# wpeebles/gangealing

Hardware: NVIDIA H100
Metric: gangealing_train_images_per_sec_256 (higher is better)
Workload: dtype f32

## Files before the change

### gangealing_b200/_lib.py

```python
import ctypes
import os

import torch

_HERE = os.path.dirname(os.path.abspath(__file__))
LIB_PATH = os.path.join(_HERE, "libgg_b200.so")

GG_F32, GG_F16, GG_BF16 = 0, 1, 2
PAD_MODES = {"zeros": 0, "border": 1, "reflection": 2}

_c = ctypes
_P, _I, _L, _F = _c.c_void_p, _c.c_int, _c.c_int64, _c.c_float

SIGNATURES = {
    "gg_version": (_I, []),
    "gg_last_error": (_c.c_char_p, []),
    "gg_sm_count": (_I, []),
    "gg_fused_bias_act": (_I, [_P, _P, _P, _P, _I, _I, _I, _F, _F, _L, _L, _L, _P]),
    "gg_noise_bias_act": (_I, [_P, _P, _P, _P, _P, _P, _I, _F, _F, _L, _L, _L, _P]),
    "gg_channel_scale_workspace": (_L, [_L, _L]),
    "gg_channel_scale": (_I, [_P, _P, _P, _P, _P, _P, _I, _L, _L, _P]),
    "gg_bias_act_backward_workspace": (_L, [_L, _L, _L]),
    "gg_bias_act_backward": (_I, [_P, _P, _P, _P, _P, _I, _F, _F, _L, _L, _L, _P]),
    "gg_upfirdn2d": (_I, [_P, _P, _P, _I, _L] + [_I] * 12 + [_P]),
    "gg_blur_noise_bias_act": (_I, [_P] * 7 + [_I, _L, _L] + [_I] * 9 + [_F, _F, _P]),
    "gg_mipmap_pyramid_elems": (_L, [_L, _I, _I, _I]),
    "gg_mipmap_build": (_I, [_P, _P, _I, _L, _I, _I, _I, _P]),
    "gg_mipmap_build_backward": (_I, [_P, _P, _L, _I, _I, _I, _P]),
    "gg_mipmap_warp_forward": (_I, [_P] * 5 + [_I, _L] + [_I] * 6 + [_F, _F, _I, _P]),
    "gg_warp_sample_indices": (_I, [_P, _P, _L, _I, _I, _I, _I, _F, _F, _I, _P]),
    "gg_stn_sample_forward": (_I, [_P] * 11 + [_I, _I, _L] + [_I] * 9 + [_F, _F, _I, _P]),
    "gg_mipmap_warp_lerp_forward": (_I, [_P] * 5 + [_L, _P, _P, _I, _I, _L] + [_I] * 6 + [_F, _F, _I, _P]),
    "gg_mipmap_warp_lerp_mean": (_I, [_P] * 4 + [_L, _P, _P, _I, _I, _L] + [_I] * 6 + [_F, _F, _I, _I, _P]),
    "gg_track_points_lerp": (_I, [_P] * 6 + [_I, _L, _L, _I, _I, _I, _P]),
    "gg_modconv_wsq": (_I, [_P, _P, _I, _I, _I, _P]),
    "gg_modconv_demod": (_I, [_P, _P, _P, _F, _F, _I, _I, _I, _P]),
    "gg_modconv_demod_batched": (_I, [_I, _P, _P, _P, _P, _P, _P, _F, _I, _P]),
    "gg_modconv_modulate": (_I, [_P, _P, _P, _P, _F, _I, _I, _I, _I, _I, _P]),
    "gg_noise_bias_act_nhwc": (_I, [_P] * 6 + [_I, _F, _F, _L, _I, _L, _P]),
    "gg_nhwc_rowwise_workspace": (_L, [_L, _I, _L]),
    "gg_channel_scale_nhwc": (_I, [_P] * 6 + [_I, _L, _I, _L, _P]),
    "gg_bias_act_backward_nhwc": (_I, [_P] * 5 + [_I, _F, _F, _L, _I, _L, _P]),
    "gg_blur_nhwc_workspace": (_L, [_I, _L] + [_I] * 9),
    "gg_blur_nhwc": (_I, [_P] * 12 + [_I, _L] + [_I] * 12 + [_F, _F, _P]),
    "gg_styled_tail_nhwc": (_I, [_P] * 12 + [_I, _I, _F, _F, _L, _I, _L, _P]),
    "gg_styled_tail_backward_workspace": (_L, [_I, _L, _I, _L]),
    "gg_styled_tail_backward_nhwc": (_I, [_P] * 12 + [_I, _F, _F, _L, _I, _L, _L, _P]),
    "gg_tent_downsample_forward": (_I, [_P] * 4 + [_L, _I, _I, _I, _I, _P]),
    "gg_tent_downsample_backward": (_I, [_P] * 4 + [_L, _I, _I, _I, _I, _P]),
    "gg_feature_distance_workspace": (_L, [_L, _I, _L]),
    "gg_feature_distance_forward": (_I, [_P] * 5 + [_I, _L, _I, _L, _F, _P]),
    "gg_feature_distance_backward": (_I, [_P] * 6 + [_I, _L, _I, _L, _F, _P]),
    "gg_bias_relu_pool_nhwc_forward": (_I, [_P, _P, _P, _P, _I, _L, _I, _I, _I, _P]),
    "gg_bias_relu_pool_nhwc_backward": (_I, [_P, _P, _P, _P, _I, _L, _I, _I, _I, _P]),
    "gg_to_rgb_nhwc_workspace": (_L, [_L, _I, _L]),
    "gg_to_rgb_nhwc_forward": (_I, [_P] * 5 + [_L, _I, _L, _P]),
    "gg_to_rgb_nhwc_backward": (_I, [_P] * 6 + [_L, _I, _L, _P]),
    "gg_nn_argmin_workspace": (_L, [_L, _L]),
    "gg_nn_argmin": (_I, [_P, _P, _P, _P, _L, _L, _I, _P]),
    "gg_splat2d_lookup_forward": (_I, [_P] * 8 + [_L, _L, _I, _I, _I, _I, _I, _F, _F, _I, _P]),
    "gg_scale_cast_multi": (_I, [_P, _P, _P, _I, _I, _P]),
    "gg_adam_ema_step": (_I, [_P, _P, _P, _I, _I, _P, _c.c_double, _c.c_double, _c.c_double, _c.c_double, _P]),
    "gg_tv_loss_workspace": (_L, [_L, _I, _I]),
    "gg_tv_loss_forward": (_I, [_P, _P, _P, _L, _I, _I, _P]),
    "gg_tv_loss_backward": (_I, [_P, _P, _P, _L, _I, _I, _P]),
    "gg_splat2d_workspace": (_L, [_L, _I, _I, _I]),
    "gg_splat2d_forward": (_I, [_P] * 6 + [_L, _L, _I, _I, _I, _I, _P]),
    "gg_flow_compose_forward": (_I, [_P] * 7 + [_L, _I, _I, _I, _P]),
    "gg_flow_compose_backward": (_I, [_P] * 10 + [_L, _I, _I, _I, _P]),
    "gg_mipmap_warp_backward": (_I, [_P] * 7 + [_I, _L] + [_I] * 6 + [_F, _F, _I, _P]),
    "gg_laplacian_blend_workspace": (_L, [_L, _I, _I, _I, _I, _I]),
    "gg_laplacian_blend_forward": (_I, [_P] * 6 + [_L, _I, _I, _I, _I, _I, _P]),
    "gg_laplacian_blend_backward": (_I, [_P] * 9 + [_L, _I, _I, _I, _I, _I, _P]),
    "gg_tv_per_sample": (_I, [_P, _P, _L, _I, _I, _P]),
    "gg_pck_transfer_workspace": (_L, [_L, _L, _I]),
    "gg_pck_transfer": (_I, [_P] * 14 + [_L, _L, _I, _I, _I, _I, _I, _P]),
    "gg_batch_gram": (_I, [_P, _P, _P, _P, _L, _I, _P]),
}

_dll = None
CALLS = 0


def load():
    global _dll
    if _dll is None:
        if not os.path.exists(LIB_PATH):
            raise RuntimeError(
                "libgg_b200.so is missing (%s): build it with `python -m gangealing_b200.build` "
                "(there is no CPU/PyTorch fallback for these ops)" % LIB_PATH)
        dll = ctypes.CDLL(LIB_PATH)
        for name, (res, args) in SIGNATURES.items():
            fn = getattr(dll, name)
            fn.restype = res
            fn.argtypes = args
        _dll = dll
    return _dll


def check(rc, what):
    global CALLS
    CALLS += 1
    if rc != 0:
        msg = load().gg_last_error().decode("utf-8", "replace")
        raise RuntimeError("%s failed (%d): %s" % (what, rc, msg))


def dtype_code(t):
    d = t.dtype
    if d == torch.float32:
        return GG_F32
    if d == torch.float16:
        return GG_F16
    if d == torch.bfloat16:
        return GG_BF16
    raise RuntimeError("gangealing_b200: dtype %s is not supported (float32/float16/bfloat16)" % d)


def require_cuda(*tensors):
    for t in tensors:
        if t is None:
            continue
        if not t.is_cuda:
            raise RuntimeError("gangealing_b200 ops run on CUDA tensors only (got a %s tensor); "
                               "the CPU restatement lives in oracle/ and is test infrastructure" % t.device.type)
        if t.device.index != torch.cuda.current_device():
            raise RuntimeError("gangealing_b200: tensor lives on %s but the current device is cuda:%d; wrap the call in "
                               "`with torch.cuda.device(tensor.device):`" % (t.device, torch.cuda.current_device()))


def ptr(t):
    return None if t is None else t.data_ptr()


def is_nhwc(t):
    return (t.dim() == 4 and t.dtype in (torch.float32, torch.bfloat16) and t.shape[1] > 1 and t.shape[2] * t.shape[3] > 1
            and t.is_contiguous(memory_format=torch.channels_last) and not t.is_contiguous())


def nhwc_vec(t):
    return 8 if t.dtype == torch.bfloat16 else 4


def aligned16(t):
    return t.data_ptr() % 16 == 0


def dense_f32(t):
    if t.dtype != torch.float32 or not t.is_contiguous():
        t = t.float().contiguous()
    return t if aligned16(t) else t.clone()


def tensor_cache(t):
    stamp = (t._version, t.data_ptr(), t.device, t.dtype)
    ent = getattr(t, "_gg_cache", None)
    if ent is None or ent[0] != stamp:
        ent = (stamp, {})
        try:
            t._gg_cache = ent
        except Exception:
            pass
    return ent[1]


def filter_is_separable(kernel):
    memo = tensor_cache(kernel)
    v = memo.get("separable")
    if v is None:
        k = kernel.detach().float().cpu()
        big = k.abs().max()
        if big == 0:
            v = True
        else:
            i0, j0 = divmod(int(k.abs().argmax()), k.shape[1])
            v = bool((k - torch.outer(k[:, j0], k[i0, :]) / k[i0, j0]).abs().max() <= 1e-6 * big)
        memo["separable"] = v
    return v


def flipped_filter(kernel):
    memo = tensor_cache(kernel)
    f = memo.get("flipped")
    if f is None:
        f = torch.flip(kernel.detach(), [0, 1])
        fm = tensor_cache(f)
        fm["flipped"] = kernel.detach()
        if "separable" in memo:
            fm["separable"] = memo["separable"]
        memo["flipped"] = f
    return f


def invalidate(t):
    try:
        t._gg_cache = None
    except Exception:
        pass


def stream():
    return torch.cuda.current_stream().cuda_stream


def sm_count():
    return load().gg_sm_count()


def ship_table(slot, payload):
    capturing = torch.cuda.is_current_stream_capturing()
    ev = slot.get("event")
    if ev is not None and not capturing:
        ev.synchronize()
    slot["host"].copy_(payload)
    slot["dev"].copy_(slot["host"], non_blocking=True)
    if capturing:
        slot["event"] = None
    else:
        ev = torch.cuda.Event()
        ev.record()
        slot["event"] = ev
```

### gangealing_b200/csrc/common.cuh

```cuda
#pragma once
#include <cuda_bf16.h>
#include <cuda_fp16.h>
#include <cuda_runtime.h>
#include <stdint.h>

#include <cstdarg>
#include <cstdio>

#include "../../include/gg_b200.h"

namespace gg {

inline char* err_buf() {
  static thread_local char buf[512] = {0};
  return buf;
}
inline int fail(int code, const char* fmt, ...) {
  va_list ap;
  va_start(ap, fmt);
  vsnprintf(err_buf(), 512, fmt, ap);
  va_end(ap);
  return code;
}
inline int cuda_fail(cudaError_t e, const char* what) {
  return fail(GG_ERR_CUDA, "%s: %s", what, cudaGetErrorString(e));
}
#define GG_CHECK_LAUNCH(what)                               \
  do {                                                      \
    cudaError_t e__ = cudaPeekAtLastError();                \
    if (e__ != cudaSuccess) {                               \
      (void)cudaGetLastError();                             \
      return ::gg::cuda_fail(e__, what);                    \
    }                                                       \
  } while (0)

#define GG_DISPATCH_CASE_(code_, type_, ...) \
  case code_: { using T_ = type_; __VA_ARGS__; break; }
#define GG_DISPATCH_T(dtype_, who_, ...)                                                                             \
  switch (dtype_) {                                                                                                  \
    GG_DISPATCH_CASE_(GG_F32, float, __VA_ARGS__)                                                                    \
    GG_DISPATCH_CASE_(GG_BF16, __nv_bfloat16, __VA_ARGS__)                                                           \
    default: return ::gg::fail(GG_ERR_UNSUPPORTED, "%s: dtype %d not supported (fp32 or bf16)", who_, dtype_);       \
  }
#define GG_DISPATCH_T16(dtype_, who_, ...)                                                                           \
  switch (dtype_) {                                                                                                  \
    GG_DISPATCH_CASE_(GG_F32, float, __VA_ARGS__)                                                                    \
    GG_DISPATCH_CASE_(GG_F16, __half, __VA_ARGS__)                                                                   \
    GG_DISPATCH_CASE_(GG_BF16, __nv_bfloat16, __VA_ARGS__)                                                           \
    default: return ::gg::fail(GG_ERR_UNSUPPORTED, "%s: dtype %d not supported (fp32, fp16 or bf16)", who_, dtype_); \
  }

int sm_count();

inline bool aligned16(const void* p) { return (reinterpret_cast<uintptr_t>(p) & 15u) == 0; }

struct DeviceOnce {
  unsigned long long mask[2] = {0ull, 0ull};
  int dev = 0;
  bool needed() {
    if (cudaGetDevice(&dev) != cudaSuccess || dev < 0 || dev >= 128) return true;
    return ((__atomic_load_n(&mask[dev >> 6], __ATOMIC_ACQUIRE) >> (dev & 63)) & 1ull) == 0ull;
  }
  void done() {
    if (dev >= 0 && dev < 128) __atomic_fetch_or(&mask[dev >> 6], 1ull << (dev & 63), __ATOMIC_RELEASE);
  }
};

template <typename T> struct Cvt;
template <> struct Cvt<float> {
  static __device__ __forceinline__ float to_f(float v) { return v; }
  static __device__ __forceinline__ float from_f(float v) { return v; }
};
template <> struct Cvt<__half> {
  static __device__ __forceinline__ float to_f(__half v) { return __half2float(v); }
  static __device__ __forceinline__ __half from_f(float v) { return __float2half_rn(v); }
};
template <> struct Cvt<__nv_bfloat16> {
  static __device__ __forceinline__ float to_f(__nv_bfloat16 v) { return __bfloat162float(v); }
  static __device__ __forceinline__ __nv_bfloat16 from_f(float v) { return __float2bfloat16_rn(v); }
};

template <typename T> struct alignas(16) Vec16 {
  static constexpr int N = 16 / sizeof(T);
  T v[N];
};

template <typename T>
__device__ __forceinline__ Vec16<T> ld_vec_stream(const T* p) {
  Vec16<T> r;
  uint4 u;
  asm volatile("ld.global.nc.L1::no_allocate.v4.u32 {%0,%1,%2,%3}, [%4];"
               : "=r"(u.x), "=r"(u.y), "=r"(u.z), "=r"(u.w)
               : "l"(p));
  *reinterpret_cast<uint4*>(&r) = u;
  return r;
}
template <typename T>
__device__ __forceinline__ void st_vec_stream(T* p, const Vec16<T>& r) {
  const uint4 u = *reinterpret_cast<const uint4*>(&r);
  asm volatile("st.global.L1::no_allocate.v4.u32 [%0], {%1,%2,%3,%4};" ::"l"(p), "r"(u.x), "r"(u.y),
               "r"(u.z), "r"(u.w)
               : "memory");
}

template <typename T> struct ChanVec;
template <> struct ChanVec<float> {
  static constexpr int V = 4;
  static __device__ __forceinline__ void unpack(const uint4& u, float (&f)[4]) {
    f[0] = __uint_as_float(u.x); f[1] = __uint_as_float(u.y); f[2] = __uint_as_float(u.z); f[3] = __uint_as_float(u.w);
  }
  static __device__ __forceinline__ uint4 pack(const float (&f)[4]) {
    return make_uint4(__float_as_uint(f[0]), __float_as_uint(f[1]), __float_as_uint(f[2]), __float_as_uint(f[3]));
  }
};
template <> struct ChanVec<__nv_bfloat16> {
  static constexpr int V = 8;
  static __device__ __forceinline__ void unpack(const uint4& u, float (&f)[8]) {
    f[0] = __uint_as_float(u.x << 16); f[1] = __uint_as_float(u.x & 0xffff0000u);
    f[2] = __uint_as_float(u.y << 16); f[3] = __uint_as_float(u.y & 0xffff0000u);
    f[4] = __uint_as_float(u.z << 16); f[5] = __uint_as_float(u.z & 0xffff0000u);
    f[6] = __uint_as_float(u.w << 16); f[7] = __uint_as_float(u.w & 0xffff0000u);
  }
  static __device__ __forceinline__ uint32_t pack2(float lo, float hi) {
    const __nv_bfloat162 h = __floats2bfloat162_rn(lo, hi);
    return *reinterpret_cast<const uint32_t*>(&h);
  }
  static __device__ __forceinline__ uint4 pack(const float (&f)[8]) {
    return make_uint4(pack2(f[0], f[1]), pack2(f[2], f[3]), pack2(f[4], f[5]), pack2(f[6], f[7]));
  }
};
__device__ __forceinline__ uint4 ldg_stream16(const void* p) {
  uint4 u;
  asm volatile("ld.global.nc.L1::no_allocate.v4.u32 {%0,%1,%2,%3}, [%4];" : "=r"(u.x), "=r"(u.y), "=r"(u.z), "=r"(u.w) : "l"(p));
  return u;
}
__device__ __forceinline__ void stg_stream16(void* p, const uint4& u) {
  asm volatile("st.global.L1::no_allocate.v4.u32 [%0], {%1,%2,%3,%4};" ::"l"(p), "r"(u.x), "r"(u.y), "r"(u.z), "r"(u.w) : "memory");
}

__device__ __forceinline__ float warp_sum(float v) {
#pragma unroll
  for (int o = 16; o > 0; o >>= 1) v += __shfl_xor_sync(0xffffffffu, v, o);
  return v;
}

__device__ __forceinline__ uint32_t smem_u32(const void* p) {
  return static_cast<uint32_t>(__cvta_generic_to_shared(p));
}
__device__ __forceinline__ void mbar_init(uint64_t* bar, uint32_t count) {
  asm volatile("mbarrier.init.shared::cta.b64 [%0], %1;" ::"r"(smem_u32(bar)), "r"(count));
}
__device__ __forceinline__ void mbar_fence_init() {
  asm volatile("fence.mbarrier_init.release.cluster;" ::: "memory");
}
__device__ __forceinline__ void mbar_expect_tx(uint64_t* bar, uint32_t bytes) {
  asm volatile("mbarrier.arrive.expect_tx.shared::cta.b64 _, [%0], %1;" ::"r"(smem_u32(bar)),
               "r"(bytes)
               : "memory");
}
__device__ __forceinline__ void mbar_wait(uint64_t* bar, uint32_t parity) {
  uint32_t done;
  uint32_t spins = 0;
  do {
    if (++spins == (1u << 28)) __trap();
    asm volatile(
        "{\n\t"
        ".reg .pred p;\n\t"
        "mbarrier.try_wait.parity.shared::cta.b64 p, [%1], %2;\n\t"
        "selp.u32 %0, 1, 0, p;\n\t"
        "}"
        : "=r"(done)
        : "r"(smem_u32(bar)), "r"(parity)
        : "memory");
  } while (!done);
}
__device__ __forceinline__ void tma_bulk_g2s(void* dst_smem, const void* src_gmem, uint32_t bytes,
                                             uint64_t* bar) {
  asm volatile(
      "cp.async.bulk.shared::cluster.global.mbarrier::complete_tx::bytes [%0], [%1], %2, [%3];" ::"r"(
          smem_u32(dst_smem)),
      "l"(src_gmem), "r"(bytes), "r"(smem_u32(bar))
      : "memory");
}

}
```

### gangealing_b200/csrc/nhwc.cu

```cuda
#include <cuda.h>

#include "common.cuh"
#include "nhwc_reduce.cuh"

namespace gg {
namespace {

constexpr int kT = 256;

template <typename T>
__global__ void __launch_bounds__(kT)
noise_bias_act_nhwc_kernel(T* __restrict__ out, const T* __restrict__ x, const float* __restrict__ noise,
                           const float* __restrict__ noise_weight, const float* __restrict__ bias,
                           const float* __restrict__ row_scale, float alpha, float gain, int64_t n_vec, int cv,
                           int64_t hw) {
  constexpr int V = ChanVec<T>::V;
  const float nw = noise ? (noise_weight ? __ldg(noise_weight) : 1.f) : 0.f;
  const int64_t base = (static_cast<int64_t>(blockIdx.x) * 4) * kT + threadIdx.x;
  uint4 xv[4];
#pragma unroll
  for (int u = 0; u < 4; ++u) {
    const int64_t v = base + static_cast<int64_t>(u) * kT;
    if (v < n_vec) xv[u] = ldg_stream16(x + v * V);
  }
#pragma unroll
  for (int u = 0; u < 4; ++u) {
    const int64_t v = base + static_cast<int64_t>(u) * kT;
    if (v < n_vec) {
      int64_t pix, n = 0;
      int cq;
      if (n_vec <= 0xffffffffLL) {
        const unsigned v32 = static_cast<unsigned>(v), p32 = v32 / static_cast<unsigned>(cv);
        cq = static_cast<int>(v32 - p32 * static_cast<unsigned>(cv));
        pix = p32;
        if (row_scale) n = p32 / static_cast<unsigned>(hw);
      } else {
        pix = v / cv;
        cq = static_cast<int>(v - pix * cv);
        if (row_scale) n = pix / hw;
      }
      const float nz = noise ? nw * __ldg(noise + pix) : 0.f;
      float xf[V], o[V];
      ChanVec<T>::unpack(xv[u], xf);
#pragma unroll
      for (int q = 0; q < V / 4; ++q) {
        const float4 b = bias ? __ldg(reinterpret_cast<const float4*>(bias) + cq * (V / 4) + q) : make_float4(0.f, 0.f, 0.f, 0.f);
        const float4 r = row_scale ? __ldg(reinterpret_cast<const float4*>(row_scale + n * cv * V) + cq * (V / 4) + q)
                                   : make_float4(1.f, 1.f, 1.f, 1.f);
        const float bb[4] = {b.x, b.y, b.z, b.w}, rr[4] = {r.x, r.y, r.z, r.w};
#pragma unroll
        for (int k = 0; k < 4; ++k) {
          const float t = fmaf(xf[4 * q + k], rr[k], bb[k]) + nz;
          o[4 * q + k] = (t > 0.f ? t : t * alpha) * gain;
        }
      }
      stg_stream16(out + v * V, ChanVec<T>::pack(o));
    }
  }
}

template <typename T, int MODE>
__global__ void __launch_bounds__(kT)
rowwise_nhwc_kernel(T* __restrict__ out, float* __restrict__ partial, const T* __restrict__ x,
                    const T* __restrict__ y, const float* __restrict__ s, float alpha, float gain, int cv,
                    int64_t hw, int chunk, int chunks_per_sample) {
  constexpr int V = ChanVec<T>::V;
  extern __shared__ float red[];
  const int64_t n = blockIdx.x / chunks_per_sample;
  const int ck = blockIdx.x - n * chunks_per_sample;
  const int64_t p0 = static_cast<int64_t>(ck) * chunk, p1 = min(p0 + chunk, hw);
  const int lanes_p = kT / cv > 0 ? kT / cv : 1;
  float acc[V];
#pragma unroll
  for (int k = 0; k < V; ++k) acc[k] = 0.f;
  const int cq = threadIdx.x % cv;
  const int pl = threadIdx.x / cv;
  if (pl < lanes_p) {
    float sv[V];
#pragma unroll
    for (int k = 0; k < V; ++k) sv[k] = (MODE == 0) ? __ldg(s + n * cv * V + cq * V + k) : 1.f;
    const bool has_y = (MODE == 1) || y != nullptr;
    auto body = [&](const uint4 xr, const uint4 yr, int64_t off) {
      float xf[V], yf[V], o[V];
      ChanVec<T>::unpack(xr, xf);
      ChanVec<T>::unpack(yr, yf);
#pragma unroll
      for (int k = 0; k < V; ++k) {
        if (MODE == 0) {
          o[k] = xf[k] * sv[k];
          if (has_y) acc[k] = fmaf(xf[k], yf[k], acc[k]);
        } else {
          o[k] = (yf[k] > 0.f ? xf[k] : xf[k] * alpha) * gain;
          acc[k] += o[k];
        }
      }
      *reinterpret_cast<uint4*>(out + off) = ChanVec<T>::pack(o);
    };
    const uint4 zero = make_uint4(0u, 0u, 0u, 0u);
    int64_t p = p0 + pl;
    for (; p + 3 * lanes_p < p1; p += 4 * lanes_p) {
      uint4 xv[4], yv[4];
      int64_t off[4];
#pragma unroll
      for (int u = 0; u < 4; ++u) {
        off[u] = ((n * hw + p + u * lanes_p) * cv + cq) * V;
        xv[u] = ldg_stream16(x + off[u]);
      }
#pragma unroll
      for (int u = 0; u < 4; ++u) yv[u] = has_y ? ldg_stream16(y + off[u]) : zero;
#pragma unroll
      for (int u = 0; u < 4; ++u) body(xv[u], yv[u], off[u]);
    }
    for (; p < p1; p += lanes_p) {
      const int64_t off = ((n * hw + p) * cv + cq) * V;
      const uint4 xv = ldg_stream16(x + off);
      const uint4 yv = has_y ? ldg_stream16(y + off) : zero;
      body(xv, yv, off);
    }
  }
  if (partial) {
    const int C = cv * V;
    if (pl < lanes_p) {
#pragma unroll
      for (int q = 0; q < V / 4; ++q)
        reinterpret_cast<float4*>(red + pl * C + cq * V)[q] = make_float4(acc[4 * q], acc[4 * q + 1], acc[4 * q + 2], acc[4 * q + 3]);
    }
    __syncthreads();
    for (int c = threadIdx.x; c < C; c += kT) {
      float t = 0.f;
      for (int l = 0; l < lanes_p; ++l) t += red[l * C + c];
      partial[static_cast<int64_t>(blockIdx.x) * C + c] = t;
    }
  }
}

__global__ void __launch_bounds__(kT)
to_rgb_nhwc_fwd_kernel(float* __restrict__ out, const float* __restrict__ x, const float* __restrict__ wm,
                       const float* __restrict__ bias, const float* __restrict__ skip, int c4, int64_t hw, int chunk,
                       int chunks_per_sample) {
  extern __shared__ __align__(16) float wsm[];
  const int64_t n = blockIdx.x / chunks_per_sample;
  const int ck = blockIdx.x - n * chunks_per_sample;
  const int64_t p0 = static_cast<int64_t>(ck) * chunk, p1 = min(p0 + chunk, hw);
  {
    const float4* src = reinterpret_cast<const float4*>(wm + n * 3 * c4 * 4);
    float4* dst = reinterpret_cast<float4*>(wsm);
    for (int i = threadIdx.x; i < 3 * c4; i += kT) dst[i] = __ldg(src + i);
  }
  __syncthreads();
  const float4* w4 = reinterpret_cast<const float4*>(wsm);
  const int l = threadIdx.x & 7, grp = threadIdx.x >> 3;
  const bool vec_ok = (hw & 3) == 0;
  const unsigned gmask = 0xffu << (threadIdx.x & 24);
  for (int64_t pb = p0 + grp * 4; pb < p1; pb += (kT / 8) * 4) {
    float acc[4][3];
#pragma unroll
    for (int u = 0; u < 4; ++u) acc[u][0] = acc[u][1] = acc[u][2] = 0.f;
    const float4* xp[4];
#pragma unroll
    for (int u = 0; u < 4; ++u) {
      const int64_t pu = min(pb + u, p1 - 1);
      xp[u] = reinterpret_cast<const float4*>(x + (n * hw + pu) * c4 * 4);
    }
    for (int q = l; q < c4; q += 8) {
      float4 xv[4];
#pragma unroll
      for (int u = 0; u < 4; ++u) xv[u] = __ldcs(xp[u] + q);
      const float4 w0 = w4[q], w1 = w4[c4 + q], w2 = w4[2 * c4 + q];
#pragma unroll
      for (int u = 0; u < 4; ++u) {
        acc[u][0] = fmaf(xv[u].x, w0.x, fmaf(xv[u].y, w0.y, fmaf(xv[u].z, w0.z, fmaf(xv[u].w, w0.w, acc[u][0]))));
        acc[u][1] = fmaf(xv[u].x, w1.x, fmaf(xv[u].y, w1.y, fmaf(xv[u].z, w1.z, fmaf(xv[u].w, w1.w, acc[u][1]))));
        acc[u][2] = fmaf(xv[u].x, w2.x, fmaf(xv[u].y, w2.y, fmaf(xv[u].z, w2.z, fmaf(xv[u].w, w2.w, acc[u][2]))));
      }
    }
#pragma unroll
    for (int m = 4; m >= 1; m >>= 1)
#pragma unroll
      for (int u = 0; u < 4; ++u)
#pragma unroll
        for (int o = 0; o < 3; ++o) acc[u][o] += __shfl_xor_sync(gmask, acc[u][o], m);
    if (l < 3) {
      const int o = l;
      float r[4];
#pragma unroll
      for (int u = 0; u < 4; ++u) r[u] = (o == 0 ? acc[u][0] : o == 1 ? acc[u][1] : acc[u][2]) + (bias ? __ldg(bias + o) : 0.f);
      const int64_t off = (n * 3 + o) * hw + pb;
      if (vec_ok && pb + 3 < p1) {
        if (skip) {
          const float4 sk = __ldg(reinterpret_cast<const float4*>(skip + off));
          r[0] += sk.x; r[1] += sk.y; r[2] += sk.z; r[3] += sk.w;
        }
        *reinterpret_cast<float4*>(out + off) = make_float4(r[0], r[1], r[2], r[3]);
      } else {
#pragma unroll
        for (int u = 0; u < 4; ++u)
          if (pb + u < p1) out[off + u] = r[u] + (skip ? __ldg(skip + off + u) : 0.f);
      }
    }
  }
}

__global__ void __launch_bounds__(kT)
to_rgb_nhwc_bwd_kernel(float* __restrict__ gx, float* __restrict__ partial, const float* __restrict__ g,
                       const float* __restrict__ x, const float* __restrict__ wm, int c4, int64_t hw, int chunk,
                       int chunks_per_sample) {
  extern __shared__ float red[];
  const int64_t n = blockIdx.x / chunks_per_sample;
  const int ck = blockIdx.x - n * chunks_per_sample;
  const int64_t p0 = static_cast<int64_t>(ck) * chunk, p1 = min(p0 + chunk, hw);
  const int lanes_p = kT / c4 > 0 ? kT / c4 : 1;
  const int cq = threadIdx.x % c4, pl = threadIdx.x / c4;
  float4 a0 = make_float4(0.f, 0.f, 0.f, 0.f), a1 = a0, a2 = a0;
  if (pl < lanes_p) {
    const float4* wp = reinterpret_cast<const float4*>(wm + n * 3 * c4 * 4);
    const float4 w0 = __ldg(wp + cq), w1 = __ldg(wp + c4 + cq), w2 = __ldg(wp + 2 * c4 + cq);
    const float* g0 = g + n * 3 * hw;
    auto body = [&](int64_t p, const float4 xv, float s0, float s1, float s2) {
      float4 o;
      o.x = fmaf(w2.x, s2, fmaf(w1.x, s1, w0.x * s0)); o.y = fmaf(w2.y, s2, fmaf(w1.y, s1, w0.y * s0));
      o.z = fmaf(w2.z, s2, fmaf(w1.z, s1, w0.z * s0)); o.w = fmaf(w2.w, s2, fmaf(w1.w, s1, w0.w * s0));
      if (gx) *reinterpret_cast<float4*>(gx + ((n * hw + p) * c4 + cq) * 4) = o;
      a0.x = fmaf(s0, xv.x, a0.x); a0.y = fmaf(s0, xv.y, a0.y); a0.z = fmaf(s0, xv.z, a0.z); a0.w = fmaf(s0, xv.w, a0.w);
      a1.x = fmaf(s1, xv.x, a1.x); a1.y = fmaf(s1, xv.y, a1.y); a1.z = fmaf(s1, xv.z, a1.z); a1.w = fmaf(s1, xv.w, a1.w);
      a2.x = fmaf(s2, xv.x, a2.x); a2.y = fmaf(s2, xv.y, a2.y); a2.z = fmaf(s2, xv.z, a2.z); a2.w = fmaf(s2, xv.w, a2.w);
    };
    const float4 zero = make_float4(0.f, 0.f, 0.f, 0.f);
    int64_t p = p0 + pl;
    for (; p + 3 * lanes_p < p1; p += 4 * lanes_p) {
      float4 xv[4];
      float s[4][3];
#pragma unroll
      for (int u = 0; u < 4; ++u) {
        const int64_t pu = p + u * lanes_p;
        xv[u] = partial ? __ldcs(reinterpret_cast<const float4*>(x + ((n * hw + pu) * c4 + cq) * 4)) : zero;
        s[u][0] = __ldg(g0 + pu); s[u][1] = __ldg(g0 + hw + pu); s[u][2] = __ldg(g0 + 2 * hw + pu);
      }
#pragma unroll
      for (int u = 0; u < 4; ++u) body(p + u * lanes_p, xv[u], s[u][0], s[u][1], s[u][2]);
    }
    for (; p < p1; p += lanes_p) {
      const float4 xv = partial ? __ldcs(reinterpret_cast<const float4*>(x + ((n * hw + p) * c4 + cq) * 4)) : zero;
      body(p, xv, __ldg(g0 + p), __ldg(g0 + hw + p), __ldg(g0 + 2 * hw + p));
    }
  }
  if (partial) {
    float4* r4 = reinterpret_cast<float4*>(red);
    if (pl < lanes_p) {
      r4[(pl * 3 + 0) * c4 + cq] = a0; r4[(pl * 3 + 1) * c4 + cq] = a1; r4[(pl * 3 + 2) * c4 + cq] = a2;
    }
    __syncthreads();
    for (int i = threadIdx.x; i < 3 * c4; i += kT) {
      float4 t = make_float4(0.f, 0.f, 0.f, 0.f);
      for (int q = 0; q < lanes_p; ++q) {
        const float4 v = r4[q * 3 * c4 + i];
        t.x += v.x; t.y += v.y; t.z += v.z; t.w += v.w;
      }
      reinterpret_cast<float4*>(partial + static_cast<int64_t>(blockIdx.x) * 3 * c4 * 4)[i] = t;
    }
  }
}

template <typename T> struct BlurGeom {
  static constexpr int V = ChanVec<T>::V;
  static constexpr int CB = 8 * V;
  static constexpr int COLS = (V == 4) ? 2 : 1;
  static constexpr int BX = 32 * COLS;
  static constexpr int TW = BX + 3;
  static constexpr int STAGE_ELEMS = 4 * TW * CB;
};
constexpr int kRY = 4;
constexpr int kNS = 3;

struct BlurNhwcParams {
  int n, c, in_h, in_w, out_h, out_w;
  int pad_x0, pad_y0;
  int seg_rows;
  int act;
  float alpha, gain;
};

__device__ __forceinline__ void tma_load_4d(void* smem_dst, const CUtensorMap* tmap, int c0, int x0, int y0, int n0,
                                            uint64_t* bar) {
  asm volatile(
      "cp.async.bulk.tensor.4d.shared::cluster.global.tile.mbarrier::complete_tx::bytes [%0], [%1, {%2, %3, %4, %5}], [%6];"
      ::"r"(smem_u32(smem_dst)), "l"(tmap), "r"(c0), "r"(x0), "r"(y0), "r"(n0), "r"(smem_u32(bar))
      : "memory");
}

template <typename T, int MODE, bool SEP, bool FAST = false>
__global__ void __launch_bounds__(kT, 2)
blur_nhwc_kernel(T* __restrict__ out, T* __restrict__ out2, const __grid_constant__ CUtensorMap tmap,
                 const float* __restrict__ filt, int kh, int kw, const float* __restrict__ noise,
                 const float* __restrict__ noise_weight, const float* __restrict__ bias,
                 const float* __restrict__ row_scale, const float* __restrict__ scale2, const T* __restrict__ mul,
                 float* __restrict__ partial, BlurNhwcParams p) {
  using G = BlurGeom<T>;
  constexpr int V = G::V, CB = G::CB, COLS = G::COLS, BX = G::BX, TW = G::TW;
  constexpr bool FUSED = MODE == 1;
  extern __shared__ __align__(128) unsigned char tiles_raw[];
  T* tiles = reinterpret_cast<T*>(tiles_raw);
  __shared__ uint64_t full_bar[kNS];
  const int tid = threadIdx.x;
  const int cq = tid & 7;
  const int xg = tid >> 3;
  const int chunks = p.c / CB;
  const int bx = blockIdx.x / chunks, cc = blockIdx.x - bx * chunks;
  const int n = blockIdx.z;
  const int oy0 = blockIdx.y * p.seg_rows;
  const int rows_out = min(p.seg_rows, p.out_h - oy0);
  const int x_out0 = bx * BX;
  const int c0 = cc * CB;
  const int iy0 = oy0 - p.pad_y0, ix0 = x_out0 - p.pad_x0;
  const int rows_in = rows_out + 3;
  const int n_stage_iters = (rows_in + kRY - 1) / kRY;
  constexpr uint32_t kStageBytes = G::STAGE_ELEMS * sizeof(T);

  if (tid == 0) {
#pragma unroll
    for (int s = 0; s < kNS; ++s) mbar_init(&full_bar[s], 1);
    mbar_fence_init();
  }
  __syncthreads();
  if (tid == 0) {
#pragma unroll
    for (int s = 0; s < kNS - 1; ++s)
      if (s < n_stage_iters) {
        mbar_expect_tx(&full_bar[s], kStageBytes);
        tma_load_4d(tiles + s * G::STAGE_ELEMS, &tmap, c0, ix0, iy0 + s * kRY, n, &full_bar[s]);
      }
  }

  float kf[4][4];
#pragma unroll
  for (int a = 0; a < 4; ++a)
#pragma unroll
    for (int b = 0; b < 4; ++b)
      kf[a][b] = (a < kh && b < kw) ? __ldg(filt + (kh - 1 - a) * kw + (kw - 1 - b)) : 0.f;
  float ku[4], kv[4];
  {
    int a0 = 0, b0 = 0;
    float big = 0.f;
#pragma unroll
    for (int a = 0; a < 4; ++a)
#pragma unroll
      for (int b = 0; b < 4; ++b)
        if (fabsf(kf[a][b]) > big) { big = fabsf(kf[a][b]); a0 = a; b0 = b; }
    float piv = 1.f;
#pragma unroll
    for (int a = 0; a < 4; ++a)
#pragma unroll
      for (int b = 0; b < 4; ++b)
        if (a == a0 && b == b0) piv = kf[a][b];
    const float inv = big > 0.f ? 1.f / piv : 0.f;
#pragma unroll
    for (int a = 0; a < 4; ++a) {
      float col = 0.f;
#pragma unroll
      for (int b = 0; b < 4; ++b) if (b == b0) col = kf[a][b];
      ku[a] = col * inv;
    }
#pragma unroll
    for (int b = 0; b < 4; ++b) {
      float row = 0.f;
#pragma unroll
      for (int a = 0; a < 4; ++a) if (a == a0) row = kf[a][b];
      kv[b] = row;
    }
  }

  float bq[V], rq[V], sq[V], dacc[V];
#pragma unroll
  for (int k = 0; k < V; ++k) { bq[k] = 0.f; rq[k] = 1.f; sq[k] = 1.f; dacc[k] = 0.f; }
  float nw = 0.f;
  const int64_t nc0 = static_cast<int64_t>(n) * p.c + c0 + cq * V;
  if (MODE != 0) {
    if (row_scale) {
#pragma unroll
      for (int k = 0; k < V; ++k) rq[k] = __ldg(row_scale + nc0 + k);
    }
  }
  if (FUSED) {
    if (bias) {
#pragma unroll
      for (int k = 0; k < V; ++k) bq[k] = __ldg(bias + c0 + cq * V + k);
    }
    if (scale2) {
#pragma unroll
      for (int k = 0; k < V; ++k) sq[k] = __ldg(scale2 + nc0 + k);
    }
    nw = noise ? (noise_weight ? __ldg(noise_weight) : 1.f) : 0.f;
  }
  constexpr bool fast = FUSED && FAST;
  const float neg = (p.act == 3) ? p.alpha : 1.f;
  if (fast) {
#pragma unroll
    for (int k = 0; k < V; ++k) { rq[k] *= p.gain; bq[k] *= p.gain; }
    nw *= p.gain;
  }
  const int xo = x_out0 + COLS * xg;
  const int64_t row_stride = static_cast<int64_t>(p.out_w) * p.c;
  const int64_t obase = ((static_cast<int64_t>(n) * p.out_h + oy0) * p.out_w + xo) * p.c + c0 + cq * V;
  int64_t ocur = obase - 3 * row_stride;
  bool okc[COLS];
#pragma unroll
  for (int j = 0; j < COLS; ++j) okc[j] = xo + j < p.out_w;
  float nzn[kRY][COLS];
#pragma unroll
  for (int rr = 0; rr < kRY; ++rr)
#pragma unroll
    for (int j = 0; j < COLS; ++j) nzn[rr][j] = 0.f;
  const float* noise_base = noise ? noise + (static_cast<int64_t>(n) * p.out_h + oy0) * p.out_w + xo : nullptr;
  auto fetch_noise = [&](int it_) {
#pragma unroll
    for (int rr = 0; rr < kRY; ++rr) {
      const int ro = it_ * kRY + rr - 3;
#pragma unroll
      for (int j = 0; j < COLS; ++j) nzn[rr][j] = 0.f;
      if (ro >= 0 && ro < rows_out) {
        const float* np_ = noise_base + static_cast<int64_t>(ro) * p.out_w;
#pragma unroll
        for (int j = 0; j < COLS; ++j)
          if (okc[j]) nzn[rr][j] = __ldg(np_ + j);
      }
    }
  };
  if (FUSED && noise) fetch_noise(0);

  uint4 mcur[COLS], mnext[COLS];
#pragma unroll
  for (int j = 0; j < COLS; ++j) mcur[j] = mnext[j] = make_uint4(0u, 0u, 0u, 0u);
  auto fetch_mul = [&](int ro_) {
    if (ro_ >= 0 && ro_ < rows_out) {
      const int64_t mo = obase + ro_ * row_stride;
#pragma unroll
      for (int j = 0; j < COLS; ++j)
        if (okc[j]) mnext[j] = __ldg(reinterpret_cast<const uint4*>(mul + mo + static_cast<int64_t>(j) * p.c));
    }
  };
  if (MODE == 2 && mul) { fetch_mul(-3 + 3); }

  float hwin[SEP ? 4 : 1][COLS][V];
  float rwin[SEP ? 1 : 4][COLS + 3][V];
  int r_in = 0;
  for (int it = 0; it < n_stage_iters; ++it) {
    const int stage = it % kNS;
    if (tid == 0) {
      const int nxt = it + kNS - 1;
      if (nxt < n_stage_iters) {
        const int ns = nxt % kNS;
        asm volatile("fence.proxy.async.shared::cta;" ::: "memory");
        mbar_expect_tx(&full_bar[ns], kStageBytes);
        tma_load_4d(tiles + ns * G::STAGE_ELEMS, &tmap, c0, ix0, iy0 + nxt * kRY, n, &full_bar[ns]);
      }
    }
    float nzc[kRY][COLS];
#pragma unroll
    for (int rr = 0; rr < kRY; ++rr)
#pragma unroll
      for (int j = 0; j < COLS; ++j) nzc[rr][j] = nzn[rr][j];
    if (FUSED && noise && it + 1 < n_stage_iters) fetch_noise(it + 1);
    if (MODE == 2 && mul && it + 1 < n_stage_iters) {
#pragma unroll
      for (int rr = 0; rr < kRY; ++rr) {
        const int ro = (it + 1) * kRY + rr - 3;
        if (ro >= 0 && ro < rows_out) {
          const T* mp = mul + obase + ro * row_stride;
#pragma unroll
          for (int j = 0; j < COLS; ++j)
            if (okc[j]) asm volatile("prefetch.global.L2 [%0];" ::"l"(mp + static_cast<int64_t>(j) * p.c));
        }
      }
    }
    mbar_wait(&full_bar[stage], static_cast<uint32_t>((it / kNS) & 1));
    const T* st = tiles + stage * G::STAGE_ELEMS;
#pragma unroll
    for (int rr = 0; rr < kRY; ++rr, ++r_in, ocur += row_stride) {
      if (MODE == 2 && mul) {
#pragma unroll
        for (int j = 0; j < COLS; ++j) mcur[j] = mnext[j];
        fetch_mul(r_in - 3 + 1);
      }
      const uint4* rowp = reinterpret_cast<const uint4*>(st + (rr * TW + COLS * xg) * CB) + cq;
      float q[COLS + 3][V];
#pragma unroll
      for (int i = 0; i < COLS + 3; ++i) ChanVec<T>::unpack(rowp[i * 8], q[i]);
      if constexpr (SEP) {
#pragma unroll
        for (int j = 0; j < COLS; ++j)
#pragma unroll
          for (int k = 0; k < V; ++k) {
            float h = __fmul_rn(kv[0], q[j][k]);
            h = __fmaf_rn(kv[1], q[j + 1][k], h);
            h = __fmaf_rn(kv[2], q[j + 2][k], h);
            h = __fmaf_rn(kv[3], q[j + 3][k], h);
            hwin[rr][j][k] = h;
          }
      } else {
#pragma unroll
        for (int i = 0; i < COLS + 3; ++i)
#pragma unroll
          for (int k = 0; k < V; ++k) rwin[rr][i][k] = q[i][k];
      }
      const int ro = r_in - 3;
      if (ro >= 0 && ro < rows_out) {
#pragma unroll
        for (int j = 0; j < COLS; ++j) {
          float a4[V];
          if constexpr (SEP) {
#pragma unroll
            for (int k = 0; k < V; ++k) {
              float a = __fmul_rn(ku[0], hwin[(rr + 1) & 3][j][k]);
              a = __fmaf_rn(ku[1], hwin[(rr + 2) & 3][j][k], a);
              a = __fmaf_rn(ku[2], hwin[(rr + 3) & 3][j][k], a);
              a = __fmaf_rn(ku[3], hwin[rr][j][k], a);
              a4[k] = a;
            }
          } else {
#pragma unroll
            for (int k = 0; k < V; ++k) a4[k] = 0.f;
#pragma unroll
            for (int a = 0; a < 4; ++a)
#pragma unroll
              for (int b = 0; b < 4; ++b)
#pragma unroll
                for (int k = 0; k < V; ++k) a4[k] = fmaf(kf[a][b], rwin[(rr + 1 + a) & 3][j + b][k], a4[k]);
          }
          const int64_t ooff = ocur + j * p.c;
          if (FUSED) {
            const float nzj = nw * nzc[rr][j];
            float o2[V];
#pragma unroll
            for (int k = 0; k < V; ++k) {
              float t = __fmaf_rn(a4[k], rq[k], __fadd_rn(bq[k], nzj));
              const float tn = __fmul_rn(t, neg);
              if (fast) t = fmaxf(t, tn);
              else t = (t > 0.f ? t : tn) * p.gain;
              a4[k] = t;
              o2[k] = __fmul_rn(t, sq[k]);
            }
            if (okc[j]) {
              if (out) *reinterpret_cast<uint4*>(out + ooff) = ChanVec<T>::pack(a4);
              if (out2) *reinterpret_cast<uint4*>(out2 + ooff) = ChanVec<T>::pack(o2);
            }
          } else if (MODE == 2) {
            if (okc[j]) {
              if (mul) {
                float mf[V];
                ChanVec<T>::unpack(mcur[j], mf);
#pragma unroll
                for (int k = 0; k < V; ++k) dacc[k] = fmaf(a4[k], mf[k], dacc[k]);
              }
#pragma unroll
              for (int k = 0; k < V; ++k) a4[k] *= rq[k];
              *reinterpret_cast<uint4*>(out + ooff) = ChanVec<T>::pack(a4);
            }
          } else {
            if (okc[j]) *reinterpret_cast<uint4*>(out + ooff) = ChanVec<T>::pack(a4);
          }
        }
      }
    }
    __syncthreads();
  }
  if (MODE == 2 && partial) {
    float* red = reinterpret_cast<float*>(tiles_raw);
#pragma unroll
    for (int k = 0; k < V; ++k) red[xg * CB + cq * V + k] = dacc[k];
    __syncthreads();
    if (tid < CB) {
      float t = 0.f;
#pragma unroll 8
      for (int g = 0; g < 32; ++g) t += red[g * CB + tid];
      const int64_t K = static_cast<int64_t>(gridDim.x / chunks) * gridDim.y;
      const int64_t kidx = static_cast<int64_t>(bx) * gridDim.y + blockIdx.y;
      partial[(static_cast<int64_t>(n) * K + kidx) * p.c + c0 + tid] = t;
    }
  }
}

typedef CUresult (*EncodeTiledFn)(CUtensorMap*, CUtensorMapDataType, cuuint32_t, void*, const cuuint64_t*, const cuuint64_t*,
                                  const cuuint32_t*, const cuuint32_t*, CUtensorMapInterleave, CUtensorMapSwizzle,
                                  CUtensorMapL2promotion, CUtensorMapFloatOOBfill);

inline EncodeTiledFn encode_fn() {
  static EncodeTiledFn fn = nullptr;
  if (!fn) {
    void* p = nullptr;
    cudaDriverEntryPointQueryResult q;
    if (cudaGetDriverEntryPoint("cuTensorMapEncodeTiled", &p, cudaEnableDefault, &q) == cudaSuccess &&
        q == cudaDriverEntryPointSuccess)
      fn = reinterpret_cast<EncodeTiledFn>(p);
  }
  return fn;
}

inline int grid1(int64_t total, int per_cta) {
  int64_t g = (total + per_cta - 1) / per_cta;
  return static_cast<int>(g > 0 ? g : 1);
}

}
}

using namespace gg;

extern "C" {

static inline int vec_of(int dtype) { return dtype == GG_BF16 ? 8 : 4; }

int gg_noise_bias_act_nhwc(void* out, const void* x, const float* noise, const float* noise_weight, const float* bias,
                           const float* row_scale, int dtype, float alpha, float scale, int64_t N, int C, int64_t HW,
                           void* stream) {
  if (N < 0 || C < 0 || HW < 0) return fail(GG_ERR_BAD_ARG, "noise_bias_act_nhwc: negative size");
  if (dtype != GG_F32 && dtype != GG_BF16) return fail(GG_ERR_UNSUPPORTED, "noise_bias_act_nhwc: dtype %d not supported", dtype);
  const int64_t numel = N * HW * C;
  if (numel == 0) return GG_OK;
  const int V = vec_of(dtype);
  if (C % V != 0) return fail(GG_ERR_UNSUPPORTED, "noise_bias_act_nhwc: C must be a multiple of %d", V);
  if (!out || !x) return fail(GG_ERR_BAD_ARG, "noise_bias_act_nhwc: null tensor");
  if (!aligned16(bias) || !aligned16(row_scale))
    return fail(GG_ERR_BAD_ARG, "noise_bias_act_nhwc: bias and row_scale must be 16-byte aligned");
  const int64_t n_vec = numel / V;
  const int64_t grid = (n_vec + 4 * kT - 1) / (4 * kT);
  if (grid > 0x7fffffffLL) return fail(GG_ERR_BAD_ARG, "noise_bias_act_nhwc: tensor too large");
  GG_DISPATCH_T(dtype, "noise_bias_act_nhwc",
                (noise_bias_act_nhwc_kernel<T_><<<static_cast<unsigned>(grid), kT, 0, static_cast<cudaStream_t>(stream)>>>(
                    static_cast<T_*>(out), static_cast<const T_*>(x), noise, noise_weight, bias, row_scale, alpha, scale,
                    n_vec, C / V, HW)));
  GG_CHECK_LAUNCH("noise_bias_act_nhwc launch");
  return GG_OK;
}

static int64_t rowwise_chunk(int64_t N, int cv, int64_t HW) {
  const int lanes_p = kT / cv > 0 ? kT / cv : 1;
  const int64_t target = 8LL * sm_count();
  int64_t k = (target + N - 1) / N;
  const int64_t kmax = (HW + 4 * lanes_p - 1) / (4 * lanes_p);
  if (k > kmax) k = kmax;
  if (k < 1) k = 1;
  return (HW + k - 1) / k;
}

int64_t gg_nhwc_rowwise_workspace(int64_t N, int C, int64_t HW) {
  if (N <= 0 || C <= 0 || HW <= 0 || C % 4 != 0) return 0;
  const int64_t chunk = rowwise_chunk(N, C / 4, HW);
  const int64_t chunk8 = (C % 8 == 0) ? rowwise_chunk(N, C / 8, HW) : chunk;
  const int64_t k = (HW + (chunk < chunk8 ? chunk : chunk8) - 1) / (chunk < chunk8 ? chunk : chunk8);
  return N * k * C * static_cast<int64_t>(sizeof(float));
}

static int launch_rowwise(int mode, void* out, float* dst, void* workspace, const void* x, const void* y, const float* s,
                          int dtype, float alpha, float gain, int64_t N, int C, int64_t HW, bool per_sample, void* stream) {
  if (N < 0 || C < 0 || HW < 0) return fail(GG_ERR_BAD_ARG, "nhwc rowwise: negative size");
  if (dtype != GG_F32 && dtype != GG_BF16) return fail(GG_ERR_UNSUPPORTED, "nhwc rowwise: dtype %d not supported", dtype);
  if (N * HW * C == 0) {
    const int64_t sums = (per_sample ? N : 1) * C;
    if (dst && sums > 0) {
      cudaError_t e = cudaMemsetAsync(dst, 0, sums * sizeof(float), static_cast<cudaStream_t>(stream));
      if (e != cudaSuccess) return cuda_fail(e, "nhwc rowwise memset");
    }
    return GG_OK;
  }
  const int V = vec_of(dtype);
  if (C % V != 0 || C / V > kT) return fail(GG_ERR_UNSUPPORTED, "nhwc rowwise: C must be a multiple of %d and <= %d", V, V * kT);
  if (!out || !x) return fail(GG_ERR_BAD_ARG, "nhwc rowwise: null tensor");
  if (dst && !workspace) return fail(GG_ERR_BAD_ARG, "nhwc rowwise: reduction needs a workspace");
  const int cv = C / V;
  const int64_t chunk64 = rowwise_chunk(N, cv, HW);
  if (chunk64 > 0x7fffffffLL) return fail(GG_ERR_BAD_ARG, "nhwc rowwise: plane too large");
  const int chunk = static_cast<int>(chunk64);
  const int K = static_cast<int>((HW + chunk - 1) / chunk);
  const int64_t grid = N * K;
  if (grid > 0x7fffffffLL) return fail(GG_ERR_BAD_ARG, "nhwc rowwise: too many CTAs");
  const int lanes_p = kT / cv > 0 ? kT / cv : 1;
  const size_t smem = static_cast<size_t>(lanes_p) * C * sizeof(float);
  float* partial = dst ? static_cast<float*>(workspace) : nullptr;
  auto st = static_cast<cudaStream_t>(stream);
  const unsigned g = static_cast<unsigned>(grid);
  if (mode == 0) {
    GG_DISPATCH_T(dtype, "nhwc rowwise",
                  (rowwise_nhwc_kernel<T_, 0><<<g, kT, smem, st>>>(static_cast<T_*>(out), partial, static_cast<const T_*>(x),
                                                                 dst ? static_cast<const T_*>(y) : nullptr, s, alpha, gain,
                                                                 cv, HW, chunk, K)));
  } else {
    GG_DISPATCH_T(dtype, "nhwc rowwise",
                  (rowwise_nhwc_kernel<T_, 1><<<g, kT, smem, st>>>(static_cast<T_*>(out), partial, static_cast<const T_*>(x),
                                                                 static_cast<const T_*>(y), s, alpha, gain, cv, HW, chunk, K)));
  }
  GG_CHECK_LAUNCH("nhwc rowwise launch");
  if (dst) {
    const int64_t rows = per_sample ? N : 1;
    const int kk = per_sample ? K : static_cast<int>(N * K);
    nhwc_finish_kernel<<<static_cast<unsigned>(rows * ((C + 31) / 32)), dim3(32, 32), 0, st>>>(dst, partial, rows, kk, C);
    GG_CHECK_LAUNCH("nhwc finish launch");
  }
  return GG_OK;
}

int gg_channel_scale_nhwc(void* out, float* row_dot, void* workspace, const void* x, const void* y, const float* s,
                          int dtype, int64_t N, int C, int64_t HW, void* stream) {
  if (!s) return fail(GG_ERR_BAD_ARG, "channel_scale_nhwc: null scale");
  if (row_dot && !y) return fail(GG_ERR_BAD_ARG, "channel_scale_nhwc: row_dot needs y");
  return launch_rowwise(0, out, row_dot, workspace, x, y, s, dtype, 0.f, 1.f, N, C, HW, true, stream);
}

int gg_bias_act_backward_nhwc(void* gx, float* grad_bias, void* workspace, const void* g, const void* out_saved,
                              int dtype, float alpha, float scale, int64_t N, int C, int64_t HW, void* stream) {
  if (!out_saved) return fail(GG_ERR_BAD_ARG, "bias_act_backward_nhwc: null saved output");
  return launch_rowwise(1, gx, grad_bias, workspace, g, out_saved, nullptr, dtype, alpha, scale, N, C, HW, false, stream);
}

int64_t gg_to_rgb_nhwc_workspace(int64_t N, int C, int64_t HW) { return 3 * gg_nhwc_rowwise_workspace(N, C, HW); }

int gg_to_rgb_nhwc_forward(float* out, const float* x, const float* wm, const float* bias, const float* skip, int64_t N,
                           int C, int64_t HW, void* stream) {
  if (N < 0 || C < 0 || HW < 0) return fail(GG_ERR_BAD_ARG, "to_rgb_nhwc: negative size");
  if (N * HW == 0) return GG_OK;
  if (C < 32 || C % 32 != 0 || C > 1024) return fail(GG_ERR_UNSUPPORTED, "to_rgb_nhwc: C must be a multiple of 32, <= 1024");
  if (!out || !x || !wm) return fail(GG_ERR_BAD_ARG, "to_rgb_nhwc: null tensor");
  if (!aligned16(wm) || (HW % 4 == 0 && (!aligned16(skip) || !aligned16(out))))
    return fail(GG_ERR_BAD_ARG, "to_rgb_nhwc: wm (and skip, out when HW %% 4 == 0) must be 16-byte aligned");
  const int64_t target = 8LL * sm_count();
  int64_t k = (target + N - 1) / N;
  const int64_t kmax = (HW + 127) / 128;
  if (k > kmax) k = kmax;
  if (k < 1) k = 1;
  int64_t chunk = ((HW + k - 1) / k + 127) / 128 * 128;
  if (chunk > 0x7fffff00LL) return fail(GG_ERR_BAD_ARG, "to_rgb_nhwc: plane too large");
  const int K = static_cast<int>((HW + chunk - 1) / chunk);
  const int64_t grid = N * K;
  if (grid > 0x7fffffffLL) return fail(GG_ERR_BAD_ARG, "to_rgb_nhwc: too many CTAs");
  to_rgb_nhwc_fwd_kernel<<<static_cast<unsigned>(grid), kT, static_cast<size_t>(3) * C * sizeof(float),
                           static_cast<cudaStream_t>(stream)>>>(out, x, wm, bias, skip, C / 4, HW, static_cast<int>(chunk), K);
  GG_CHECK_LAUNCH("to_rgb_nhwc forward launch");
  return GG_OK;
}

int gg_to_rgb_nhwc_backward(float* gx, float* gwm, void* workspace, const float* g, const float* x, const float* wm,
                            int64_t N, int C, int64_t HW, void* stream) {
  if (N < 0 || C < 0 || HW < 0) return fail(GG_ERR_BAD_ARG, "to_rgb_nhwc backward: negative size");
  if (N * HW == 0 || C == 0) {
    if (gwm && N * C > 0) {
      cudaError_t e = cudaMemsetAsync(gwm, 0, N * 3 * C * sizeof(float), static_cast<cudaStream_t>(stream));
      if (e != cudaSuccess) return cuda_fail(e, "to_rgb_nhwc backward memset");
    }
    return GG_OK;
  }
  if (C % 4 != 0 || C > 1024) return fail(GG_ERR_UNSUPPORTED, "to_rgb_nhwc backward: C must be a multiple of 4, <= 1024");
  if (!g || !wm || (!gx && !gwm)) return fail(GG_ERR_BAD_ARG, "to_rgb_nhwc backward: null tensor");
  if (gwm && (!x || !workspace)) return fail(GG_ERR_BAD_ARG, "to_rgb_nhwc backward: gwm needs x and a workspace");
  if (!aligned16(wm)) return fail(GG_ERR_BAD_ARG, "to_rgb_nhwc backward: wm must be 16-byte aligned");
  const int c4 = C / 4;
  const int64_t chunk64 = rowwise_chunk(N, c4, HW);
  if (chunk64 > 0x7fffffffLL) return fail(GG_ERR_BAD_ARG, "to_rgb_nhwc backward: plane too large");
  const int chunk = static_cast<int>(chunk64);
  const int K = static_cast<int>((HW + chunk - 1) / chunk);
  const int64_t grid = N * K;
  if (grid > 0x7fffffffLL) return fail(GG_ERR_BAD_ARG, "to_rgb_nhwc backward: too many CTAs");
  const int lanes_p = kT / c4 > 0 ? kT / c4 : 1;
  const size_t smem = static_cast<size_t>(lanes_p) * 3 * C * sizeof(float);
  auto st = static_cast<cudaStream_t>(stream);
  float* partial = gwm ? static_cast<float*>(workspace) : nullptr;
  to_rgb_nhwc_bwd_kernel<<<static_cast<unsigned>(grid), kT, smem, st>>>(gx, partial, g, x, wm, c4, HW, chunk, K);
  GG_CHECK_LAUNCH("to_rgb_nhwc backward launch");
  if (gwm) {
    nhwc_finish_kernel<<<static_cast<unsigned>(N * ((3 * C + 31) / 32)), dim3(32, 32), 0, st>>>(gwm, partial, N, K, 3 * C);
    GG_CHECK_LAUNCH("to_rgb_nhwc finish launch");
  }
  return GG_OK;
}

struct BlurPlan {
  int out_h, out_w, xblocks, chunks, segs, seg_rows;
};
static int blur_plan(BlurPlan* pl, int dtype, int64_t N, int C, int in_h, int in_w, int kernel_h, int kernel_w, int pad_x0,
                     int pad_x1, int pad_y0, int pad_y1) {
  const int V = vec_of(dtype);
  const int CB = 8 * V, BX = (V == 4) ? 64 : 32;
  if (C % CB != 0) return fail(GG_ERR_UNSUPPORTED, "blur_nhwc: C must be a multiple of %d", CB);
  pl->out_h = in_h + pad_y0 + pad_y1 - kernel_h + 1;
  pl->out_w = in_w + pad_x0 + pad_x1 - kernel_w + 1;
  if (pl->out_h < 1 || pl->out_w < 1) return fail(GG_ERR_BAD_ARG, "blur_nhwc: empty output");
  pl->xblocks = (pl->out_w + BX - 1) / BX;
  pl->chunks = C / CB;
  const int64_t base_ctas = static_cast<int64_t>(pl->xblocks) * pl->chunks * (N > 0 ? N : 1);
  int segs = static_cast<int>((2LL * 2 * sm_count() + base_ctas - 1) / base_ctas);
  int seg_rows = (pl->out_h + segs - 1) / segs;
  if (seg_rows < 16) seg_rows = pl->out_h < 16 ? pl->out_h : 16;
  seg_rows = (seg_rows + 3) / 4 * 4;
  pl->seg_rows = seg_rows;
  pl->segs = (pl->out_h + seg_rows - 1) / seg_rows;
  return GG_OK;
}

int64_t gg_blur_nhwc_workspace(int dtype, int64_t N, int C, int in_h, int in_w, int kernel_h, int kernel_w, int pad_x0,
                               int pad_x1, int pad_y0, int pad_y1) {
  BlurPlan pl;
  if (N <= 0 || C <= 0 || (dtype != GG_F32 && dtype != GG_BF16)) return 0;
  if (blur_plan(&pl, dtype, N, C, in_h, in_w, kernel_h, kernel_w, pad_x0, pad_x1, pad_y0, pad_y1) != GG_OK) return 0;
  return N * static_cast<int64_t>(pl.xblocks) * pl.segs * C * static_cast<int64_t>(sizeof(float));
}

}

template <typename T>
static int launch_blur(void* out, void* out2, const void* in, const float* kernel, const float* noise,
                       const float* noise_weight, const float* bias, const float* row_scale, const float* scale2,
                       const void* mul, float* row_dot, void* workspace, int64_t N, int C, int in_h, int in_w, int kernel_h,
                       int kernel_w, int separable, int pad_x0, int pad_x1, int pad_y0, int pad_y1, int mode, int act,
                       float alpha, float scale, void* stream, int dtype) {
  using G = BlurGeom<T>;
  BlurPlan pl;
  int rc = blur_plan(&pl, dtype, N, C, in_h, in_w, kernel_h, kernel_w, pad_x0, pad_x1, pad_y0, pad_y1);
  if (rc != GG_OK) return rc;
  EncodeTiledFn enc = encode_fn();
  if (!enc) return fail(GG_ERR_CUDA, "blur_nhwc: cuTensorMapEncodeTiled is not available from this driver");
  struct MapKey { const void* ptr; int64_t n; int c, h, w, es; };
  struct MapEnt { MapKey key; CUtensorMap map; bool valid; };
  static thread_local MapEnt cache[16] = {};
  static thread_local unsigned cache_next = 0;
  const MapKey key = {in, N, C, in_h, in_w, static_cast<int>(sizeof(T))};
  const CUtensorMap* cached = nullptr;
  for (int i = 0; i < 16 && !cached; ++i)
    if (cache[i].valid && cache[i].key.ptr == key.ptr && cache[i].key.n == key.n && cache[i].key.c == key.c &&
        cache[i].key.h == key.h && cache[i].key.w == key.w && cache[i].key.es == key.es)
      cached = &cache[i].map;
  CUtensorMap tmap;
  if (cached) tmap = *cached;
  const cuuint64_t es = sizeof(T);
  const cuuint64_t gdim[4] = {static_cast<cuuint64_t>(C), static_cast<cuuint64_t>(in_w), static_cast<cuuint64_t>(in_h),
                              static_cast<cuuint64_t>(N)};
  const cuuint64_t gstr[3] = {static_cast<cuuint64_t>(C) * es, static_cast<cuuint64_t>(in_w) * C * es,
                              static_cast<cuuint64_t>(in_h) * in_w * C * es};
  const cuuint32_t box[4] = {G::CB, G::TW, kRY, 1};
  const cuuint32_t estr[4] = {1, 1, 1, 1};
  if (!cached) {
    const CUresult r = enc(&tmap, sizeof(T) == 4 ? CU_TENSOR_MAP_DATA_TYPE_FLOAT32 : CU_TENSOR_MAP_DATA_TYPE_BFLOAT16, 4,
                           const_cast<void*>(in), gdim, gstr, box, estr, CU_TENSOR_MAP_INTERLEAVE_NONE,
                           CU_TENSOR_MAP_SWIZZLE_NONE, CU_TENSOR_MAP_L2_PROMOTION_L2_128B, CU_TENSOR_MAP_FLOAT_OOB_FILL_NONE);
    if (r != CUDA_SUCCESS) return fail(GG_ERR_CUDA, "blur_nhwc: cuTensorMapEncodeTiled failed (%d)", static_cast<int>(r));
    MapEnt& e = cache[cache_next++ % 16];
    e.key = key; e.map = tmap; e.valid = true;
  }
  BlurNhwcParams p;
  p.n = static_cast<int>(N); p.c = C; p.in_h = in_h; p.in_w = in_w; p.out_h = pl.out_h; p.out_w = pl.out_w;
  p.pad_x0 = pad_x0; p.pad_y0 = pad_y0;
  p.act = act; p.alpha = alpha; p.gain = scale;
  p.seg_rows = pl.seg_rows;
  const dim3 grid(static_cast<unsigned>(pl.xblocks * pl.chunks), static_cast<unsigned>(pl.segs), static_cast<unsigned>(N));
  const size_t smem = static_cast<size_t>(kNS) * G::STAGE_ELEMS * sizeof(T);
  static DeviceOnce configured;
  if (configured.needed()) {
    cudaError_t e = cudaSuccess;
    const void* kernels[8] = {reinterpret_cast<const void*>(blur_nhwc_kernel<T, 0, true>),
                              reinterpret_cast<const void*>(blur_nhwc_kernel<T, 0, false>),
                              reinterpret_cast<const void*>(blur_nhwc_kernel<T, 1, true, false>),
                              reinterpret_cast<const void*>(blur_nhwc_kernel<T, 1, false, false>),
                              reinterpret_cast<const void*>(blur_nhwc_kernel<T, 1, true, true>),
                              reinterpret_cast<const void*>(blur_nhwc_kernel<T, 1, false, true>),
                              reinterpret_cast<const void*>(blur_nhwc_kernel<T, 2, true>),
                              reinterpret_cast<const void*>(blur_nhwc_kernel<T, 2, false>)};
    for (int i = 0; i < 8 && e == cudaSuccess; ++i)
      e = cudaFuncSetAttribute(kernels[i], cudaFuncAttributeMaxDynamicSharedMemorySize, static_cast<int>(smem));
    if (e != cudaSuccess) return cuda_fail(e, "blur_nhwc smem opt-in");
    configured.done();
  }
  auto st = static_cast<cudaStream_t>(stream);
  float* partial = (mode == 2 && row_dot) ? static_cast<float*>(workspace) : nullptr;
  const bool fast = scale > 0.f && ((act == 3 && alpha >= 0.f && alpha <= 1.f) || act == 1);
#define GG_BLUR(M_, S_, F_)                                                                                          \
  blur_nhwc_kernel<T, M_, S_, F_><<<grid, kT, smem, st>>>(static_cast<T*>(out), static_cast<T*>(out2), tmap, kernel, kernel_h, \
                                                         kernel_w, noise, noise_weight, bias, row_scale, scale2,     \
                                                         static_cast<const T*>(mul), partial, p)
  if (mode == 1) {
    if (fast) { if (separable) GG_BLUR(1, true, true); else GG_BLUR(1, false, true); }
    else { if (separable) GG_BLUR(1, true, false); else GG_BLUR(1, false, false); }
  }
  else if (mode == 2) { if (separable) GG_BLUR(2, true, false); else GG_BLUR(2, false, false); }
  else { if (separable) GG_BLUR(0, true, false); else GG_BLUR(0, false, false); }
#undef GG_BLUR
  GG_CHECK_LAUNCH("blur_nhwc launch");
  if (partial) {
    const int K = pl.xblocks * pl.segs;
    nhwc_finish_kernel<<<static_cast<unsigned>(N * ((C + 31) / 32)), dim3(32, 32), 0, st>>>(row_dot, partial, N, K, C);
    GG_CHECK_LAUNCH("blur_nhwc finish launch");
  }
  return GG_OK;
}

extern "C" {

int gg_blur_nhwc(void* out, void* out2, const void* in, const float* kernel, const float* noise, const float* noise_weight,
                 const float* bias, const float* row_scale, const float* scale2, const void* mul, float* row_dot,
                 void* workspace, int dtype, int64_t N, int C, int in_h, int in_w, int kernel_h, int kernel_w, int separable,
                 int pad_x0, int pad_x1, int pad_y0, int pad_y1, int mode, int act, float alpha, float scale, void* stream) {
  if (N < 0 || C < 0 || in_h < 1 || in_w < 1) return fail(GG_ERR_BAD_ARG, "blur_nhwc: bad shape");
  if (kernel_h < 1 || kernel_w < 1 || kernel_h > 4 || kernel_w > 4) return fail(GG_ERR_UNSUPPORTED, "blur_nhwc: filter must be <= 4x4");
  if (mode < 0 || mode > 2) return fail(GG_ERR_BAD_ARG, "blur_nhwc: mode must be 0 (blur), 1 (fused tail) or 2 (adjoint epilogue)");
  if (act != 1 && act != 3) return fail(GG_ERR_UNSUPPORTED, "blur_nhwc: act must be 1 or 3");
  if (dtype != GG_F32 && dtype != GG_BF16) return fail(GG_ERR_UNSUPPORTED, "blur_nhwc: dtype %d not supported (fp32 or bf16)", dtype);
  if (N == 0 || C == 0) return GG_OK;
  if (!in || !kernel) return fail(GG_ERR_BAD_ARG, "blur_nhwc: null tensor");
  if (mode == 1 ? (!out && !out2) : !out) return fail(GG_ERR_BAD_ARG, "blur_nhwc: null output");
  if (mode != 1 && out2) return fail(GG_ERR_BAD_ARG, "blur_nhwc: out2 belongs to the fused tail (mode 1)");
  if (mode == 2 && row_dot && (!mul || !workspace)) return fail(GG_ERR_BAD_ARG, "blur_nhwc: row_dot needs `mul` and a workspace");
  if (N > 65535) return fail(GG_ERR_UNSUPPORTED, "blur_nhwc: batch > 65535");
  if (mode == 0) { noise = nullptr; noise_weight = nullptr; bias = nullptr; row_scale = nullptr; scale2 = nullptr; }
  GG_DISPATCH_T(dtype, "blur_nhwc",
                return launch_blur<T_>(out, out2, in, kernel, noise, noise_weight, bias, row_scale, scale2, mul, row_dot,
                                       workspace, N, C, in_h, in_w, kernel_h, kernel_w, separable, pad_x0, pad_x1, pad_y0,
                                       pad_y1, mode, act, alpha, scale, stream, dtype));
  return GG_OK;
}

}
```

### gangealing_b200/csrc/styled.cu

```cuda
#include "common.cuh"
#include "nhwc_reduce.cuh"

namespace gg {
namespace {

constexpr int kT = 256;
constexpr int kGroup = 8;
constexpr int kPix = 4;

struct TailFwdParams {
  const void* raw; void* out; void* xs; float* rgb; const float* skip;
  const float* noise; const float* noise_weight; const float* bias; const float* demod; const float* s_next;
  const float* wm; const float* rgb_bias;
  float alpha, gain;
  int act;
  int C;
  int64_t hw;
  int chunk, chunks_per_sample;
};

template <typename T, bool FAST>
__global__ void __launch_bounds__(kT, 2)
styled_tail_nhwc_kernel(const TailFwdParams p) {
  constexpr int V = ChanVec<T>::V;
  constexpr int Q = V / 4;
  extern __shared__ __align__(16) float cst[];
  const int C = p.C;
  const int nvec = C / V, J = nvec / kGroup;
  const int64_t n = blockIdx.x / p.chunks_per_sample;
  const int ck = blockIdx.x - n * p.chunks_per_sample;
  const int64_t p0 = static_cast<int64_t>(ck) * p.chunk, p1 = min(p0 + p.chunk, p.hw);
  constexpr bool fast = FAST;
  const float neg = (p.act == 3) ? p.alpha : 1.f;
  const float gfold = fast ? p.gain : 1.f;
  for (int c = threadIdx.x; c < C; c += kT) {
    const int v = c / V, r = c - v * V, q = r >> 2, e = r & 3;
    const int slot = (q * nvec + v) * 4 + e;
    cst[slot] = (p.demod ? __ldg(p.demod + n * C + c) : 1.f) * gfold;
    cst[C + slot] = (p.bias ? __ldg(p.bias + c) : 0.f) * gfold;
    cst[2 * C + slot] = p.s_next ? __ldg(p.s_next + n * C + c) : 1.f;
    if (p.rgb) {
      cst[3 * C + slot] = __ldg(p.wm + (n * 3 + 0) * C + c);
      cst[4 * C + slot] = __ldg(p.wm + (n * 3 + 1) * C + c);
      cst[5 * C + slot] = __ldg(p.wm + (n * 3 + 2) * C + c);
    }
  }
  const float nw = (p.noise ? (p.noise_weight ? __ldg(p.noise_weight) : 1.f) : 0.f) * gfold;
  __syncthreads();
  const float4* c4 = reinterpret_cast<const float4*>(cst);
  const int c4_plane = C / 4;
  const int l = threadIdx.x & (kGroup - 1), grp = threadIdx.x / kGroup;
  const unsigned gmask = 0xffu << (threadIdx.x & 24);
  const int hw = static_cast<int>(p.hw);
  const T* raw = static_cast<const T*>(p.raw) + n * hw * C;
  T* out = p.out ? static_cast<T*>(p.out) + n * hw * C : nullptr;
  T* xs = p.xs ? static_cast<T*>(p.xs) + n * hw * C : nullptr;
  const float* noise_n = p.noise ? p.noise + n * hw : nullptr;
  const int q0 = static_cast<int>(p0), q1 = static_cast<int>(p1);
  constexpr int kStride = (kT / kGroup) * kPix;
  auto pixel = [&](int pb_, int u) { return min(pb_ + u, q1 - 1); };
  uint4 xn[kPix];
  int pb = q0 + grp * kPix;
  if (pb < q1) {
#pragma unroll
    for (int u = 0; u < kPix; ++u) xn[u] = ldg_stream16(raw + static_cast<unsigned>(pixel(pb, u) * C + l * V));
  }
  for (; pb < q1; pb += kStride) {
    float nz[kPix];
    unsigned po[kPix];
#pragma unroll
    for (int u = 0; u < kPix; ++u) {
      const int px = pixel(pb, u);
      po[u] = static_cast<unsigned>(px) * static_cast<unsigned>(C);
      nz[u] = noise_n ? nw * __ldg(noise_n + px) : 0.f;
    }
    float acc[kPix][3];
#pragma unroll
    for (int u = 0; u < kPix; ++u) acc[u][0] = acc[u][1] = acc[u][2] = 0.f;
    for (int j = 0; j < J; ++j) {
      const int v = l + kGroup * j;
      uint4 xr[kPix];
#pragma unroll
      for (int u = 0; u < kPix; ++u) xr[u] = xn[u];
      {
        const bool wrap = (j + 1 == J);
        const int pbn = wrap ? pb + kStride : pb;
        const int vn = wrap ? l : v + kGroup;
        if (pbn < q1) {
#pragma unroll
          for (int u = 0; u < kPix; ++u) xn[u] = ldg_stream16(raw + static_cast<unsigned>(pixel(pbn, u) * C + vn * V));
        }
      }
      float d[V], b[V], s[V], w0[V], w1[V], w2[V];
#pragma unroll
      for (int q = 0; q < Q; ++q) {
        const float4 dv = c4[q * nvec + v], bv = c4[c4_plane + q * nvec + v], sv = c4[2 * c4_plane + q * nvec + v];
        d[4 * q] = dv.x; d[4 * q + 1] = dv.y; d[4 * q + 2] = dv.z; d[4 * q + 3] = dv.w;
        b[4 * q] = bv.x; b[4 * q + 1] = bv.y; b[4 * q + 2] = bv.z; b[4 * q + 3] = bv.w;
        s[4 * q] = sv.x; s[4 * q + 1] = sv.y; s[4 * q + 2] = sv.z; s[4 * q + 3] = sv.w;
        if (p.rgb) {
          const float4 a0 = c4[3 * c4_plane + q * nvec + v], a1 = c4[4 * c4_plane + q * nvec + v], a2 = c4[5 * c4_plane + q * nvec + v];
          w0[4 * q] = a0.x; w0[4 * q + 1] = a0.y; w0[4 * q + 2] = a0.z; w0[4 * q + 3] = a0.w;
          w1[4 * q] = a1.x; w1[4 * q + 1] = a1.y; w1[4 * q + 2] = a1.z; w1[4 * q + 3] = a1.w;
          w2[4 * q] = a2.x; w2[4 * q + 1] = a2.y; w2[4 * q + 2] = a2.z; w2[4 * q + 3] = a2.w;
        }
      }
#pragma unroll
      for (int u = 0; u < kPix; ++u) {
        float x[V], o[V], o2[V];
        ChanVec<T>::unpack(xr[u], x);
#pragma unroll
        for (int k = 0; k < V; ++k) {
          float t = fmaf(x[k], d[k], b[k] + nz[u]);
          t = fast ? fmaxf(t, t * neg) : (t > 0.f ? t : t * neg) * p.gain;
          o[k] = t;
          o2[k] = t * s[k];
        }
        if (p.rgb) {
#pragma unroll
          for (int k = 0; k < V; ++k) {
            acc[u][0] = fmaf(w0[k], o[k], acc[u][0]);
            acc[u][1] = fmaf(w1[k], o[k], acc[u][1]);
            acc[u][2] = fmaf(w2[k], o[k], acc[u][2]);
          }
        }
        if (pb + u < q1) {
          const unsigned off = po[u] + static_cast<unsigned>(v * V);
          if (out) stg_stream16(out + off, ChanVec<T>::pack(o));
          if (xs) stg_stream16(xs + off, ChanVec<T>::pack(o2));
        }
      }
    }
    if (p.rgb) {
#pragma unroll
      for (int m = kGroup / 2; m >= 1; m >>= 1)
#pragma unroll
        for (int u = 0; u < kPix; ++u)
#pragma unroll
          for (int o = 0; o < 3; ++o) acc[u][o] += __shfl_xor_sync(gmask, acc[u][o], m);
      if (l < 3) {
        const int o = l;
        const float rb = p.rgb_bias ? __ldg(p.rgb_bias + o) : 0.f;
        const int64_t off = (n * 3 + o) * p.hw + pb;
#pragma unroll
        for (int u = 0; u < kPix; ++u)
          if (pb + u < q1) {
            const float r = (o == 0 ? acc[u][0] : o == 1 ? acc[u][1] : acc[u][2]) + rb;
            p.rgb[off + u] = r + (p.skip ? __ldg(p.skip + off + u) : 0.f);
          }
      }
    }
  }
}

struct TailBwdParams {
  void* g_raw; float* partial;
  const void* g_xs; const void* out; const void* raw;
  const float* s_next; const float* demod; const float* g_rgb; const float* wm;
  float alpha, gain;
  int C;
  int64_t hw;
  int chunk, chunks_per_sample;
  int r_ds, r_dd, r_gw, n_red;
};

template <typename T>
__global__ void __launch_bounds__(kT, 2)
styled_tail_bwd_nhwc_kernel(const TailBwdParams p) {
  constexpr int V = ChanVec<T>::V;
  constexpr int U = (V == 4) ? 4 : 2;
  extern __shared__ float red[];
  const int C = p.C, cv = C / V;
  const int64_t n = blockIdx.x / p.chunks_per_sample;
  const int ck = blockIdx.x - n * p.chunks_per_sample;
  const int64_t p0 = static_cast<int64_t>(ck) * p.chunk, p1 = min(p0 + p.chunk, p.hw);
  const int lanes_p = kT / cv > 0 ? kT / cv : 1;
  const int cq = threadIdx.x % cv, pl = threadIdx.x / cv;
  float a_ds[V], a_dd[V], a_g0[V], a_g1[V], a_g2[V];
#pragma unroll
  for (int k = 0; k < V; ++k) a_ds[k] = a_dd[k] = a_g0[k] = a_g1[k] = a_g2[k] = 0.f;
  const T* gxs = static_cast<const T*>(p.g_xs);
  const T* outp = static_cast<const T*>(p.out);
  const T* rawp = static_cast<const T*>(p.raw);
  T* graw = static_cast<T*>(p.g_raw);
  if (pl < lanes_p) {
    float sv[V], dv[V], w0[V], w1[V], w2[V];
#pragma unroll
    for (int k = 0; k < V; ++k) {
      const int c = cq * V + k;
      sv[k] = p.s_next ? __ldg(p.s_next + n * C + c) : 1.f;
      dv[k] = p.demod ? __ldg(p.demod + n * C + c) : 1.f;
      w0[k] = p.g_rgb ? __ldg(p.wm + (n * 3 + 0) * C + c) : 0.f;
      w1[k] = p.g_rgb ? __ldg(p.wm + (n * 3 + 1) * C + c) : 0.f;
      w2[k] = p.g_rgb ? __ldg(p.wm + (n * 3 + 2) * C + c) : 0.f;
    }
    const float* g0 = p.g_rgb ? p.g_rgb + n * 3 * p.hw : nullptr;
    const uint4 zero = make_uint4(0u, 0u, 0u, 0u);
    auto body = [&](int64_t off, const uint4 gr, const uint4 orw, const uint4 rr, float s0, float s1, float s2) {
      float g[V], o[V], r[V], gt[V];
      ChanVec<T>::unpack(gr, g);
      ChanVec<T>::unpack(orw, o);
      ChanVec<T>::unpack(rr, r);
#pragma unroll
      for (int k = 0; k < V; ++k) {
        float go = g[k] * sv[k];
        if (p.g_rgb) go = fmaf(w2[k], s2, fmaf(w1[k], s1, fmaf(w0[k], s0, go)));
        const float t = (o[k] > 0.f ? go : go * p.alpha) * p.gain;
        a_ds[k] = fmaf(g[k], o[k], a_ds[k]);
        a_dd[k] = fmaf(t, r[k], a_dd[k]);
        a_g0[k] = fmaf(s0, o[k], a_g0[k]);
        a_g1[k] = fmaf(s1, o[k], a_g1[k]);
        a_g2[k] = fmaf(s2, o[k], a_g2[k]);
        gt[k] = t * dv[k];
      }
      *reinterpret_cast<uint4*>(graw + off) = ChanVec<T>::pack(gt);
    };
    int64_t pp = p0 + pl;
    for (; pp + (U - 1) * lanes_p < p1; pp += U * lanes_p) {
      uint4 gr[U], orw[U], rr[U];
      float s[U][3];
      int64_t off[U];
#pragma unroll
      for (int u = 0; u < U; ++u) {
        const int64_t pu = pp + u * lanes_p;
        off[u] = ((n * p.hw + pu) * cv + cq) * V;
        orw[u] = ldg_stream16(outp + off[u]);
        gr[u] = gxs ? ldg_stream16(gxs + off[u]) : zero;
      }
#pragma unroll
      for (int u = 0; u < U; ++u) {
        const int64_t pu = pp + u * lanes_p;
        rr[u] = rawp ? ldg_stream16(rawp + off[u]) : zero;
        s[u][0] = g0 ? __ldg(g0 + pu) : 0.f;
        s[u][1] = g0 ? __ldg(g0 + p.hw + pu) : 0.f;
        s[u][2] = g0 ? __ldg(g0 + 2 * p.hw + pu) : 0.f;
      }
#pragma unroll
      for (int u = 0; u < U; ++u) body(off[u], gr[u], orw[u], rr[u], s[u][0], s[u][1], s[u][2]);
    }
    for (; pp < p1; pp += lanes_p) {
      const int64_t off = ((n * p.hw + pp) * cv + cq) * V;
      body(off, gxs ? ldg_stream16(gxs + off) : zero, ldg_stream16(outp + off), rawp ? ldg_stream16(rawp + off) : zero,
           g0 ? __ldg(g0 + pp) : 0.f, g0 ? __ldg(g0 + p.hw + pp) : 0.f, g0 ? __ldg(g0 + 2 * p.hw + pp) : 0.f);
    }
  }
  if (p.partial && p.n_red > 0) {
    const int R = p.n_red;
    if (pl < lanes_p) {
      float* row = red + static_cast<int64_t>(pl) * R * C + cq * V;
#pragma unroll
      for (int k = 0; k < V; ++k) {
        if (p.r_ds >= 0) row[p.r_ds * C + k] = a_ds[k];
        if (p.r_dd >= 0) row[p.r_dd * C + k] = a_dd[k];
        if (p.r_gw >= 0) { row[p.r_gw * C + k] = a_g0[k]; row[(p.r_gw + 1) * C + k] = a_g1[k]; row[(p.r_gw + 2) * C + k] = a_g2[k]; }
      }
    }
    __syncthreads();
    for (int i = threadIdx.x; i < R * C; i += kT) {
      float t = 0.f;
      for (int q = 0; q < lanes_p; ++q) t += red[static_cast<int64_t>(q) * R * C + i];
      p.partial[static_cast<int64_t>(blockIdx.x) * R * C + i] = t;
    }
  }
}

int64_t fwd_chunk(int64_t N, int64_t HW) {
  const int64_t trip = (kT / kGroup) * kPix;
  const int64_t target = 8LL * sm_count();
  int64_t k = (target + N - 1) / N;
  const int64_t kmax = (HW + trip - 1) / trip;
  if (k > kmax) k = kmax;
  if (k < 1) k = 1;
  return ((HW + k - 1) / k + trip - 1) / trip * trip;
}

int64_t bwd_chunk(int64_t N, int cv, int64_t HW) {
  const int lanes_p = kT / cv > 0 ? kT / cv : 1;
  const int64_t target = 8LL * sm_count();
  int64_t k = (target + N - 1) / N;
  const int64_t kmax = (HW + 4 * lanes_p - 1) / (4 * lanes_p);
  if (k > kmax) k = kmax;
  if (k < 1) k = 1;
  return (HW + k - 1) / k;
}

}
}

using namespace gg;

extern "C" {

int gg_styled_tail_nhwc(void* out, void* xs, float* rgb, const void* raw, const float* noise, const float* noise_weight,
                        const float* bias, const float* demod, const float* s_next, const float* wm, const float* rgb_bias,
                        const float* skip, int dtype, int act, float alpha, float scale, int64_t N, int C, int64_t HW,
                        void* stream) {
  if (N < 0 || C < 0 || HW < 0) return fail(GG_ERR_BAD_ARG, "styled_tail_nhwc: negative size");
  if (dtype != GG_F32 && dtype != GG_BF16) return fail(GG_ERR_UNSUPPORTED, "styled_tail_nhwc: dtype %d not supported (fp32 or bf16)", dtype);
  if (act != 1 && act != 3) return fail(GG_ERR_UNSUPPORTED, "styled_tail_nhwc: act must be 1 (linear) or 3 (lrelu)");
  if (N * HW * C == 0) return GG_OK;
  const int V = dtype == GG_BF16 ? 8 : 4;
  if (C % (V * kGroup) != 0 || C > 2048) return fail(GG_ERR_UNSUPPORTED, "styled_tail_nhwc: C must be a multiple of %d, <= 2048", V * kGroup);
  if (!raw || (!out && !xs && !rgb)) return fail(GG_ERR_BAD_ARG, "styled_tail_nhwc: null tensor");
  if (xs && !s_next) return fail(GG_ERR_BAD_ARG, "styled_tail_nhwc: xs needs s_next");
  if (rgb && !wm) return fail(GG_ERR_BAD_ARG, "styled_tail_nhwc: rgb needs wm");
  const int64_t chunk = fwd_chunk(N, HW);
  if (chunk > 0x7fffff00LL || HW * C >= 0x7fffffffLL) return fail(GG_ERR_BAD_ARG, "styled_tail_nhwc: plane too large (H*W*C must be < 2^31)");
  const int K = static_cast<int>((HW + chunk - 1) / chunk);
  const int64_t grid = N * K;
  if (grid > 0x7fffffffLL) return fail(GG_ERR_BAD_ARG, "styled_tail_nhwc: too many CTAs");
  TailFwdParams p;
  p.raw = raw; p.out = out; p.xs = xs; p.rgb = rgb; p.skip = rgb ? skip : nullptr;
  p.noise = noise; p.noise_weight = noise_weight; p.bias = bias; p.demod = demod; p.s_next = s_next;
  p.wm = wm; p.rgb_bias = rgb_bias; p.alpha = alpha; p.gain = scale; p.act = act; p.C = C; p.hw = HW;
  p.chunk = static_cast<int>(chunk); p.chunks_per_sample = K;
  const size_t smem = static_cast<size_t>(6) * C * sizeof(float);
  auto st = static_cast<cudaStream_t>(stream);
  const bool fast = p.gain > 0.f && ((p.act == 3 && p.alpha >= 0.f && p.alpha <= 1.f) || p.act == 1);
  const unsigned g = static_cast<unsigned>(grid);
  if (dtype == GG_F32) {
    if (fast) styled_tail_nhwc_kernel<float, true><<<g, kT, smem, st>>>(p);
    else styled_tail_nhwc_kernel<float, false><<<g, kT, smem, st>>>(p);
  } else {
    if (fast) styled_tail_nhwc_kernel<__nv_bfloat16, true><<<g, kT, smem, st>>>(p);
    else styled_tail_nhwc_kernel<__nv_bfloat16, false><<<g, kT, smem, st>>>(p);
  }
  GG_CHECK_LAUNCH("styled_tail_nhwc launch");
  return GG_OK;
}

int64_t gg_styled_tail_backward_workspace(int dtype, int64_t N, int C, int64_t HW) {
  if (N <= 0 || C <= 0 || HW <= 0) return 0;
  const int V = dtype == GG_BF16 ? 8 : 4;
  if (C % V != 0) return 0;
  const int64_t chunk = bwd_chunk(N, C / V, HW);
  return N * ((HW + chunk - 1) / chunk) * 5 * C * static_cast<int64_t>(sizeof(float));
}

int gg_styled_tail_backward_nhwc(void* g_raw, float* d_s_next, float* d_demod, float* d_wm, void* workspace,
                                 const void* g_xs, const float* g_rgb, const void* out_saved, const void* raw,
                                 const float* s_next, const float* demod, const float* wm, int dtype, float alpha,
                                 float scale, int64_t N, int C, int64_t HW, int64_t reduce_pitch, void* stream) {
  if (N < 0 || C < 0 || HW < 0) return fail(GG_ERR_BAD_ARG, "styled_tail_backward_nhwc: negative size");
  if (dtype != GG_F32 && dtype != GG_BF16) return fail(GG_ERR_UNSUPPORTED, "styled_tail_backward_nhwc: dtype %d not supported", dtype);
  if (N * HW * C == 0) return GG_OK;
  const int V = dtype == GG_BF16 ? 8 : 4;
  if (C % V != 0 || C / V > kT) return fail(GG_ERR_UNSUPPORTED, "styled_tail_backward_nhwc: C must be a multiple of %d, <= %d", V, V * kT);
  if (!g_raw || !out_saved || (!g_xs && !g_rgb)) return fail(GG_ERR_BAD_ARG, "styled_tail_backward_nhwc: null tensor");
  if (g_xs && !s_next) return fail(GG_ERR_BAD_ARG, "styled_tail_backward_nhwc: g_xs needs s_next");
  if (g_rgb && !wm) return fail(GG_ERR_BAD_ARG, "styled_tail_backward_nhwc: g_rgb needs wm");
  if (d_s_next && !g_xs) return fail(GG_ERR_BAD_ARG, "styled_tail_backward_nhwc: d_s_next needs g_xs");
  if (d_demod && !raw) return fail(GG_ERR_BAD_ARG, "styled_tail_backward_nhwc: d_demod needs raw");
  if (d_wm && !g_rgb) return fail(GG_ERR_BAD_ARG, "styled_tail_backward_nhwc: d_wm needs g_rgb");
  if ((d_s_next || d_demod || d_wm) && !workspace) return fail(GG_ERR_BAD_ARG, "styled_tail_backward_nhwc: reductions need a workspace");
  const int cv = C / V;
  const int64_t chunk64 = bwd_chunk(N, cv, HW);
  if (chunk64 > 0x7fffffffLL) return fail(GG_ERR_BAD_ARG, "styled_tail_backward_nhwc: plane too large");
  const int K = static_cast<int>((HW + chunk64 - 1) / chunk64);
  const int64_t grid = N * K;
  if (grid > 0x7fffffffLL) return fail(GG_ERR_BAD_ARG, "styled_tail_backward_nhwc: too many CTAs");
  TailBwdParams p;
  p.g_raw = g_raw; p.partial = static_cast<float*>(workspace); p.g_xs = g_xs; p.out = out_saved;
  p.raw = d_demod ? raw : nullptr; p.s_next = s_next; p.demod = demod; p.g_rgb = g_rgb; p.wm = wm;
  p.alpha = alpha; p.gain = scale; p.C = C; p.hw = HW; p.chunk = static_cast<int>(chunk64); p.chunks_per_sample = K;
  int r = 0;
  p.r_ds = d_s_next ? r++ : -1;
  p.r_dd = d_demod ? r++ : -1;
  p.r_gw = d_wm ? r : -1;
  if (d_wm) r += 3;
  p.n_red = r;
  const int lanes_p = kT / cv > 0 ? kT / cv : 1;
  const size_t smem = static_cast<size_t>(lanes_p) * (r > 0 ? r : 1) * C * sizeof(float);
  auto st = static_cast<cudaStream_t>(stream);
  if (smem > 48 * 1024) {
    static DeviceOnce configured;
    if (configured.needed()) {
      cudaError_t e = cudaFuncSetAttribute(styled_tail_bwd_nhwc_kernel<float>, cudaFuncAttributeMaxDynamicSharedMemorySize, 100 * 1024);
      if (e == cudaSuccess)
        e = cudaFuncSetAttribute(styled_tail_bwd_nhwc_kernel<__nv_bfloat16>, cudaFuncAttributeMaxDynamicSharedMemorySize, 100 * 1024);
      if (e != cudaSuccess) return cuda_fail(e, "styled_tail_backward_nhwc smem opt-in");
      configured.done();
    }
    if (smem > 100 * 1024) return fail(GG_ERR_UNSUPPORTED, "styled_tail_backward_nhwc: C too large for the reduction stage");
  }
  if (dtype == GG_F32) styled_tail_bwd_nhwc_kernel<float><<<static_cast<unsigned>(grid), kT, smem, st>>>(p);
  else styled_tail_bwd_nhwc_kernel<__nv_bfloat16><<<static_cast<unsigned>(grid), kT, smem, st>>>(p);
  GG_CHECK_LAUNCH("styled_tail_backward_nhwc launch");
  if (r > 0) {
    float* first = d_s_next ? d_s_next : (d_demod ? d_demod : d_wm);
    const bool packed = (!d_s_next || d_s_next == first + static_cast<int64_t>(p.r_ds) * C) &&
                        (!d_demod || d_demod == first + static_cast<int64_t>(p.r_dd) * C) &&
                        (!d_wm || d_wm == first + static_cast<int64_t>(p.r_gw) * C) && reduce_pitch == r * C;
    if (packed) {
      nhwc_finish_kernel<<<static_cast<unsigned>(N * ((r * C + 31) / 32)), dim3(32, 32), 0, st>>>(
          first, static_cast<const float*>(workspace), N, K, r * C, r * C);
    } else {
      auto finish_row = [&](float* dst, int row, int rows_n) {
        nhwc_finish_kernel<<<static_cast<unsigned>(N * ((rows_n * C + 31) / 32)), dim3(32, 32), 0, st>>>(
            dst, static_cast<const float*>(workspace) + static_cast<int64_t>(row) * C, N, K, rows_n * C, r * C);
      };
      if (reduce_pitch != C && reduce_pitch != 0 && reduce_pitch != r * C)
        return fail(GG_ERR_BAD_ARG, "styled_tail_backward_nhwc: reduce_pitch must be C (separate dense outputs) or r*C (packed block)");
      if (d_s_next) finish_row(d_s_next, p.r_ds, 1);
      if (d_demod) finish_row(d_demod, p.r_dd, 1);
      if (d_wm) finish_row(d_wm, p.r_gw, 3);
    }
    GG_CHECK_LAUNCH("styled_tail_backward_nhwc finish launch");
  }
  return GG_OK;
}

}
```

### gangealing_b200/op/nhwc.py

```python
import torch

from .. import _lib

CL = torch.channels_last

TIMING = None


def elementwise_ok(t):
    return _lib.is_nhwc(t) and t.shape[1] % _lib.nhwc_vec(t) == 0 and _lib.aligned16(t)


def rowwise_ok(t):
    return elementwise_ok(t) and t.shape[1] // _lib.nhwc_vec(t) <= 256


def blur_ok(t, kh, kw, up=(1, 1), down=(1, 1)):
    return (_lib.is_nhwc(t) and t.shape[1] % (8 * _lib.nhwc_vec(t)) == 0 and kh <= 4 and kw <= 4
            and up == (1, 1) and down == (1, 1) and _lib.aligned16(t))


def _f32(t, numel=None):
    if t is None:
        return None
    t = _lib.dense_f32(t.detach())
    if numel is not None and t.numel() != numel:
        raise RuntimeError("channels-last op: expected %d fp32 values, got %d" % (numel, t.numel()))
    return t


def noise_plane(noise, n, h, w):
    if noise is None:
        return None
    noise = noise.detach()
    if noise.numel() != n * h * w:
        noise = noise.expand(n, 1, h, w)
    return noise.float().contiguous()


def blur(x, kernel, pad, mode=0, noise=None, noise_weight=None, bias=None, row_scale=None, scale2=None, want_out=True,
         want_out2=False, mul=None, want_dot=False, negative_slope=0.2, gain=1.0, act=3):
    n, c, in_h, in_w = x.shape
    taps = kernel.detach()
    if taps.dtype != torch.float32 or not taps.is_contiguous():
        taps = taps.float().contiguous()
    kh, kw = taps.shape
    out_h = in_h + pad[2] + pad[3] - kh + 1
    out_w = in_w + pad[0] + pad[1] - kw + 1
    if out_h < 1 or out_w < 1:
        raise RuntimeError("blur: empty output (%d x %d)" % (out_h, out_w))
    lib = _lib.load()
    code = _lib.dtype_code(x)

    def empty():
        return torch.empty((n, c, out_h, out_w), dtype=x.dtype, device=x.device, memory_format=CL)
    out = empty() if (want_out or mode != 1) else None
    out2 = empty() if (mode == 1 and want_out2) else None
    nz = noise_plane(noise, n, out_h, out_w) if mode == 1 else None
    dot = ws = None
    if mode == 2 and want_dot:
        if (mul is None or mul.shape != (n, c, out_h, out_w) or mul.dtype != x.dtype or not mul.is_contiguous(memory_format=CL)
                or not _lib.aligned16(mul)):
            raise RuntimeError("blur (adjoint epilogue): `mul` must be a 16-byte-aligned channels-last tensor of the output's "
                               "shape and dtype")
        dot = torch.empty((n, c), dtype=torch.float32, device=x.device)
        nbytes = lib.gg_blur_nhwc_workspace(code, n, c, in_h, in_w, kh, kw, pad[0], pad[1], pad[2], pad[3])
        ws = torch.empty(max(1, nbytes // 4), dtype=torch.float32, device=x.device)
    timed = TIMING is not None and mode == 1
    if timed:
        ev0, ev1 = torch.cuda.Event(enable_timing=True), torch.cuda.Event(enable_timing=True)
        ev0.record()
    nw, b, rs, s2 = _f32(noise_weight, 1), _f32(bias, c), _f32(row_scale, n * c), _f32(scale2, n * c)
    rc = lib.gg_blur_nhwc(_lib.ptr(out), _lib.ptr(out2), x.data_ptr(), taps.data_ptr(), _lib.ptr(nz),
                          _lib.ptr(nw), _lib.ptr(b), _lib.ptr(rs),
                          _lib.ptr(s2), _lib.ptr(mul if dot is not None else None), _lib.ptr(dot), _lib.ptr(ws),
                          code, n, c, in_h, in_w, kh, kw, 1 if _lib.filter_is_separable(kernel) else 0, pad[0], pad[1],
                          pad[2], pad[3], mode, act, negative_slope, gain, _lib.stream())
    _lib.check(rc, "gg_blur_nhwc")
    if timed:
        ev1.record()
        es = x.element_size()
        writes = (out is not None) + (out2 is not None)
        TIMING.append((ev0, ev1, es * n * c * (in_h * in_w + writes * out_h * out_w) + (4 * n * out_h * out_w if nz is not None else 0)
                       + 4 * ((2 + (scale2 is not None)) * c + 1 + kh * kw)))
    return out, out2, dot


def noise_bias_act(x, noise, noise_weight, bias, row_scale, negative_slope, gain):
    n, c, h, w = x.shape
    out = torch.empty_like(x)
    nz, nw, b, rs = noise_plane(noise, n, h, w), _f32(noise_weight, 1), _f32(bias, c), _f32(row_scale, n * c)
    rc = _lib.load().gg_noise_bias_act_nhwc(out.data_ptr(), x.data_ptr(), _lib.ptr(nz), _lib.ptr(nw), _lib.ptr(b),
                                            _lib.ptr(rs), _lib.dtype_code(x), negative_slope, gain, n, c, h * w,
                                            _lib.stream())
    _lib.check(rc, "gg_noise_bias_act_nhwc")
    return out


def bias_act_backward(g, out_saved, negative_slope, gain, want_bias_grad):
    n, c, h, w = out_saved.shape
    lib = _lib.load()
    gx = torch.empty_like(out_saved)
    grad_bias = ws = None
    if want_bias_grad:
        grad_bias = torch.empty(c, dtype=torch.float32, device=g.device)
        ws = torch.empty(max(1, lib.gg_nhwc_rowwise_workspace(n, c, h * w) // 4), dtype=torch.float32, device=g.device)
    rc = lib.gg_bias_act_backward_nhwc(gx.data_ptr(), _lib.ptr(grad_bias), _lib.ptr(ws), g.data_ptr(), out_saved.data_ptr(),
                                       _lib.dtype_code(out_saved), negative_slope, gain, n, c, h * w, _lib.stream())
    _lib.check(rc, "gg_bias_act_backward_nhwc")
    return gx, grad_bias


def channel_scale(x, s, y=None):
    n, c, h, w = x.shape
    lib = _lib.load()
    out = torch.empty_like(x)
    dot = ws = None
    if y is not None:
        dot = torch.empty((n, c), dtype=torch.float32, device=x.device)
        ws = torch.empty(max(1, lib.gg_nhwc_rowwise_workspace(n, c, h * w) // 4), dtype=torch.float32, device=x.device)
    sc = _f32(s, n * c)
    rc = lib.gg_channel_scale_nhwc(out.data_ptr(), _lib.ptr(dot), _lib.ptr(ws), x.data_ptr(), _lib.ptr(y), sc.data_ptr(),
                                   _lib.dtype_code(x), n, c, h * w, _lib.stream())
    _lib.check(rc, "gg_channel_scale_nhwc")
    return out, dot


def styled_tail(raw, noise, noise_weight, bias, demod, s_next, wm, rgb_bias, skip, want_out, negative_slope, gain, act=3):
    n, c, h, w = raw.shape
    out = torch.empty_like(raw) if want_out else None
    xs = torch.empty_like(raw) if s_next is not None else None
    rgb = torch.empty((n, 3, h, w), dtype=torch.float32, device=raw.device) if wm is not None else None
    sk = None
    if skip is not None and rgb is not None:
        sk = skip.detach()
        if sk.dtype != torch.float32 or not sk.is_contiguous():
            sk = sk.float().contiguous()
        if sk.shape != rgb.shape:
            raise RuntimeError("styled_tail: skip must be (N, 3, H, W)")
    consts = [noise_plane(noise, n, h, w), _f32(noise_weight, 1), _f32(bias, c), _f32(demod, n * c), _f32(s_next, n * c),
              _f32(wm, n * 3 * c), _f32(rgb_bias, 3)]
    rc = _lib.load().gg_styled_tail_nhwc(_lib.ptr(out), _lib.ptr(xs), _lib.ptr(rgb), raw.data_ptr(),
                                         *[_lib.ptr(t) for t in consts], _lib.ptr(sk),
                                         _lib.dtype_code(raw), act, negative_slope, gain, n, c, h * w, _lib.stream())
    _lib.check(rc, "gg_styled_tail_nhwc")
    return out, xs, rgb


def styled_tail_backward(g_xs, g_rgb, out_saved, raw, s_next, demod, wm, want_ds, want_dd, want_dwm, negative_slope, gain):
    n, c, h, w = out_saved.shape
    lib = _lib.load()
    dev = out_saved.device
    g_raw = torch.empty_like(out_saved)
    want_ds = want_ds and g_xs is not None
    want_dd = want_dd and raw is not None
    want_dwm = want_dwm and g_rgb is not None
    rows = int(want_ds) + int(want_dd) + 3 * int(want_dwm)
    block = torch.empty((n, rows, c), dtype=torch.float32, device=dev) if rows else None
    r = 0
    d_s = d_d = d_w = None
    if want_ds:
        d_s = block[:, r]; r += 1
    if want_dd:
        d_d = block[:, r]; r += 1
    if want_dwm:
        d_w = block[:, r:r + 3]
    code = _lib.dtype_code(out_saved)
    ws = None
    if rows:
        ws = torch.empty(max(1, lib.gg_styled_tail_backward_workspace(code, n, c, h * w) // 4), dtype=torch.float32, device=dev)
    consts = [_f32(s_next, n * c), _f32(demod, n * c), _f32(wm, n * 3 * c)]
    rc = lib.gg_styled_tail_backward_nhwc(g_raw.data_ptr(), _lib.ptr(d_s), _lib.ptr(d_d), _lib.ptr(d_w), _lib.ptr(ws),
                                          _lib.ptr(g_xs), _lib.ptr(g_rgb), out_saved.data_ptr(),
                                          _lib.ptr(raw if want_dd else None),
                                          *[_lib.ptr(t) for t in consts],
                                          code, negative_slope, gain, n, c, h * w, rows * c, _lib.stream())
    _lib.check(rc, "gg_styled_tail_backward_nhwc")
    return g_raw, d_s, d_d, d_w
```

### gangealing_b200/op/style_path.py

```python
import ctypes

import torch
from torch.autograd import Function
from torch.autograd.function import once_differentiable

from .. import _lib
from .modconv import _derived


class _Plan:

    def __init__(self, convs, rgbs, conv_idx, rgb_idx):
        mods = [(("conv", i), m.conv.modulation, conv_idx[i]) for i, m in enumerate(convs)] + \
               [(("rgb", i), m.conv.modulation, rgb_idx[i]) for i, m in enumerate(rgbs)]
        groups = {}
        for key, lin, li in mods:
            groups.setdefault(lin.weight.shape[0], []).append((key, lin, li))
        self.groups = []
        for c, members in sorted(groups.items(), reverse=True):
            w = torch.stack([(lin.weight.detach() * lin.scale).t().contiguous() for _, lin, _ in members])
            b = torch.stack([(lin.bias.detach() * lin.lr_mul) for _, lin, _ in members]).unsqueeze(1)
            idx = torch.tensor([li for _, _, li in members], device=w.device)
            self.groups.append((w, b, idx, [key for key, _, _ in members]))
        self.stamp = tuple((lin.weight._version, lin.weight.data_ptr(), lin.bias._version) for _, lin, _ in mods)

    def valid(self, convs, rgbs):
        mods = [m.conv.modulation for m in convs] + [m.conv.modulation for m in rgbs]
        return self.stamp == tuple((lin.weight._version, lin.weight.data_ptr(), lin.bias._version) for lin in mods)


def all_styles(generator, latent, convs, rgbs, conv_idx, rgb_idx):
    plan = getattr(generator, "_gg_style_plan", None)
    if plan is None or not plan.valid(convs, rgbs):
        plan = _Plan(convs, rgbs, conv_idx, rgb_idx)
        generator._gg_style_plan = plan
    out = {}
    for w, b, idx, keys in plan.groups:
        lat = latent.index_select(1, idx).transpose(0, 1)
        s = torch.baddbmm(b, lat, w)
        for j, key in enumerate(keys):
            out[key] = s[j]
    return [out[("conv", i)] for i in range(len(convs))], [out[("rgb", i)] for i in range(len(rgbs))]


class _DemodAll(Function):

    @staticmethod
    def forward(ctx, meta, *styles):
        weights, scales, eps = meta
        lib = _lib.load()
        n = len(styles)
        b = styles[0].shape[0]
        if b > 256:
            raise RuntimeError("batched demodulation: batch %d > 256" % b)
        ss, wsqs, outs = [], [], []
        for w, s in zip(weights, styles):
            s = s.detach()
            if s.dtype != torch.float32 or not s.is_contiguous():
                s = s.float().contiguous()
            ss.append(s)
            wsqs.append(_derived(w, False)[1])
            outs.append(torch.empty((b, w.shape[1]), dtype=torch.float32, device=s.device))
        P, F, I = ctypes.c_void_p * n, ctypes.c_float * n, ctypes.c_int * n
        rc = lib.gg_modconv_demod_batched(n, P(*[o.data_ptr() for o in outs]), P(*[w.data_ptr() for w in wsqs]),
                                          P(*[s.data_ptr() for s in ss]), F(*[float(x) for x in scales]),
                                          I(*[w.shape[1] for w in weights]), I(*[w.shape[2] for w in weights]), float(eps), b,
                                          _lib.stream())
        _lib.check(rc, "gg_modconv_demod_batched")
        ctx.save_for_backward(*ss, *outs, *wsqs)
        ctx.cfg = (n, tuple(float(x) for x in scales), tuple(s.dtype for s in styles))
        return tuple(outs)

    @staticmethod
    @once_differentiable
    def backward(ctx, *gds):
        n, scales, dtypes = ctx.cfg
        saved = ctx.saved_tensors
        ss, ds, wsqs = saved[:n], saved[n:2 * n], saved[2 * n:]
        grads = [None] * n
        groups = {}
        for l in range(n):
            if gds[l] is not None and ctx.needs_input_grad[1 + l]:
                groups.setdefault(tuple(wsqs[l].shape), []).append(l)
        for _, members in groups.items():
            t = torch.stack([gds[l].float() * ds[l].pow(3) * (-(scales[l] ** 2)) for l in members])
            w = torch.stack([wsqs[l] for l in members])
            gs = torch.bmm(t, w)
            for j, l in enumerate(members):
                grads[l] = (gs[j] * ss[l]).to(dtypes[l])
        return (None,) + tuple(grads)


def all_demod(weights, styles, scales, eps=1e-8):
    for w in weights:
        if w.requires_grad:
            raise RuntimeError("batched demodulation serves frozen filter banks only")
    _lib.require_cuda(*weights, *styles)
    return list(_DemodAll.apply((tuple(weights), tuple(scales), eps), *styles))
```

### gangealing_b200/op/styled_fused.py

```python
import torch
from torch.autograd import Function
from torch.autograd.function import once_differentiable

from .. import _lib
from . import conv2d_gradfix, nhwc, style_path
from .modconv import channel_scale, shared_conv_weight
from .upfirdn2d import grad_pad, upfirdn2d

CL = torch.channels_last


class _FusedTail(Function):

    @staticmethod
    def forward(ctx, raw, demod, s_next, wm, skip, noise, noise_weight, bias, rgb_bias, kernel, pad, negative_slope, gain):
        _lib.require_cuda(raw, demod, s_next, wm, skip, noise)
        needs = ctx.needs_input_grad
        save = needs[0] or needs[1] or needs[2] or needs[3]
        if kernel is None:
            out, xs, rgb = nhwc.styled_tail(raw, noise, noise_weight, bias, demod, s_next, wm, rgb_bias, skip, save,
                                            negative_slope, gain)
        else:
            if wm is not None:
                raise RuntimeError("fused tail: the blur (up-sampling) layers carry no to-RGB branch")
            pad4 = (pad[0], pad[1], pad[0], pad[1])
            out, xs, _ = nhwc.blur(raw, kernel, pad4, mode=1, noise=noise, noise_weight=noise_weight, bias=bias,
                                   row_scale=demod, scale2=s_next, want_out=save or s_next is None,
                                   want_out2=s_next is not None, negative_slope=negative_slope, gain=gain)
            rgb = None
        ctx.cfg = (kernel is not None, pad, negative_slope, gain, tuple(raw.shape))
        if save:
            ctx.save_for_backward(raw if (needs[1] and demod is not None) else None, out,
                                  demod.detach() if demod is not None else None,
                                  s_next.detach() if s_next is not None else None,
                                  wm.detach() if wm is not None else None, kernel)
        if skip is not None and rgb is None:
            raise RuntimeError("fused tail: skip without a to-RGB branch")
        return xs, rgb

    @staticmethod
    @once_differentiable
    def backward(ctx, g_xs, g_rgb):
        raw, out, demod, s_next, wm, kernel = ctx.saved_tensors
        is_blur, pad, negative_slope, gain, raw_shape = ctx.cfg
        need_raw, need_d, need_s, need_w, need_skip = ctx.needs_input_grad[:5]
        if g_xs is not None:
            g_xs = g_xs.contiguous(memory_format=CL)
            if g_xs.dtype != out.dtype:
                g_xs = g_xs.to(out.dtype)
        if g_rgb is not None:
            g_rgb = g_rgb.float().contiguous()
        g_raw = d_s = d_d = d_w = None
        if g_xs is None and g_rgb is None:
            return (None,) * 13
        if not is_blur:
            g_raw, d_s, d_d, d_w = nhwc.styled_tail_backward(
                g_xs, g_rgb, out, raw, s_next, demod, wm, need_s, need_d and demod is not None, need_w,
                negative_slope, gain)
        else:
            g_t, d_s, _, _ = nhwc.styled_tail_backward(g_xs, None, out, None, s_next, None, None, need_s, False, False,
                                                       negative_slope, gain)
            kh, kw = kernel.shape
            pad4 = (pad[0], pad[1], pad[0], pad[1])
            gp = grad_pad(raw_shape[2], raw_shape[3], out.shape[2], out.shape[3], kh, kw, (1, 1), (1, 1), pad4)
            want_dot = need_d and demod is not None
            g_raw, _, d_d = nhwc.blur(g_t, _lib.flipped_filter(kernel), gp, mode=2, row_scale=demod, mul=raw if want_dot else None,
                                      want_dot=want_dot)
            if tuple(g_raw.shape) != raw_shape:
                raise RuntimeError("fused tail backward: adjoint produced %s, expected %s" % (tuple(g_raw.shape), raw_shape))
        return (g_raw if need_raw else None, d_d if need_d else None, d_s if need_s else None, d_w if need_w else None,
                g_rgb if need_skip else None, None, None, None, None, None, None, None, None)


def fused_tail(raw, demod, s_next, wm, skip, noise, noise_weight, bias, rgb_bias, kernel=None, pad=None, negative_slope=0.2,
               gain=2 ** 0.5):
    return _FusedTail.apply(raw, demod, s_next, wm, skip, noise, noise_weight, bias, rgb_bias, kernel, pad, negative_slope, gain)


def fusable(generator, latent, act_dtype):
    if not latent.is_cuda or getattr(generator, "num_fp16_res", 0) != 0 and not generator.run_fp32:
        return False
    vec = 8 if act_dtype == torch.bfloat16 else 4
    layers = [generator.conv1] + list(generator.convs)
    for layer in layers:
        conv = layer.conv
        if conv.normalize or conv.downsample or not conv.demodulate or conv.out_channel % (8 * vec) or conv.in_channel % vec:
            return False
        if conv.kernel_size != 3 or layer.activate.scale <= 0:
            return False
    for m in list(generator.to_rgbs) + [generator.to_rgb1]:
        if m.conv.normalize or m.conv.demodulate or m.conv.out_channel != 3:
            return False
    return not any(p.requires_grad for p in generator.parameters())


def synthesis(generator, latent, noise, act_dtype=torch.float32):
    layers = [generator.conv1] + list(generator.convs)
    rgbs = [generator.to_rgb1] + list(generator.to_rgbs)
    b = latent.shape[0]
    styles, rgb_styles = style_path.all_styles(generator, latent, layers, rgbs, list(range(len(layers))),
                                               [2 * r + 1 for r in range(len(rgbs))])
    demods = style_path.all_demod([layer.conv.weight for layer in layers], styles, [layer.conv.scale for layer in layers],
                                  layers[0].conv.eps)
    x0 = generator.input(latent).to(act_dtype).contiguous(memory_format=CL)
    xs = channel_scale(x0, styles[0])
    rgb = None
    for i, layer in enumerate(layers):
        conv, act = layer.conv, layer.activate
        w = shared_conv_weight(conv.weight, conv.scale, transposed=conv.upsample, channels_last=True, dtype=act_dtype)
        if conv.upsample:
            raw = conv2d_gradfix.conv_transpose2d(xs, w, padding=0, stride=2)
            blur = conv.blur
            out_h = raw.shape[2] + blur.pad[0] + blur.pad[1] - blur.kernel.shape[0] + 1
            out_w = raw.shape[3] + blur.pad[0] + blur.pad[1] - blur.kernel.shape[1] + 1
        else:
            raw = conv2d_gradfix.conv2d(xs, w, padding=conv.padding)
            blur = None
            out_h, out_w = raw.shape[2], raw.shape[3]
        nz = noise[i]
        if nz is None:
            nz = type(layer.noise).sample(b, out_h, out_w, styles[0])
        demod = demods[i]
        s_next = styles[i + 1] if i + 1 < len(layers) else None
        wm = rgb_bias = skip = None
        if not conv.upsample:
            to_rgb = rgbs[i // 2]
            rconv = to_rgb.conv
            s_rgb = rgb_styles[i // 2]
            wm = (rconv.scale * rconv.weight[0, :, :, 0, 0]).unsqueeze(0) * s_rgb.unsqueeze(1)
            rgb_bias = to_rgb.bias
            if rgb is not None:
                skip = upfirdn2d(rgb, to_rgb.upsample.kernel, up=to_rgb.upsample.up, down=1, pad=to_rgb.upsample.pad)
        xs, new_rgb = fused_tail(raw, demod, s_next, wm, skip, nz, layer.noise.weight, act.bias, rgb_bias,
                                 kernel=blur.kernel if blur is not None else None, pad=blur.pad if blur is not None else None,
                                 negative_slope=act.negative_slope, gain=act.scale)
        if new_rgb is not None:
            rgb = new_rgb
    return rgb
```

### gangealing_b200/stylegan2/networks.py

```python
import math
import random

import torch
from torch import nn
from torch.nn import functional as F

from ..opset import cuda_ops


def make_kernel(k):
    k = torch.tensor(k, dtype=torch.float32)
    if k.ndim == 1:
        k = k[None, :] * k[:, None]
    return k / k.sum()


class PixelNorm(nn.Module):
    def forward(self, input):
        return input * torch.rsqrt(torch.mean(input ** 2, dim=1, keepdim=True) + 1e-8)


class _FirModule(nn.Module):

    def __init__(self, kernel, up, down, pad, ops):
        super().__init__()
        self.register_buffer("kernel", kernel)
        self.up, self.down, self.pad = up, down, pad
        self.ops = ops if ops is not None else cuda_ops()

    def forward(self, input):
        return self.ops.upfirdn2d(input, self.kernel, up=self.up, down=self.down, pad=self.pad)


class Upsample(_FirModule):
    def __init__(self, kernel, factor=2, ops=None):
        k = make_kernel(kernel) * (factor ** 2)
        p = k.shape[0] - factor
        super().__init__(k, factor, 1, ((p + 1) // 2 + factor - 1, p // 2), ops)
        self.factor = factor


class Downsample(_FirModule):
    def __init__(self, kernel, factor=2, ops=None):
        k = make_kernel(kernel)
        p = k.shape[0] - factor
        super().__init__(k, 1, factor, ((p + 1) // 2, p // 2), ops)
        self.factor = factor


class Blur(_FirModule):
    def __init__(self, kernel, pad, upsample_factor=1, ops=None):
        k = make_kernel(kernel)
        if upsample_factor > 1:
            k = k * (upsample_factor ** 2)
        super().__init__(k, 1, 1, pad, ops)


class EqualConv2d(nn.Module):
    def __init__(self, in_channel, out_channel, kernel_size, stride=1, padding=0, bias=True, ops=None):
        super().__init__()
        self.weight = nn.Parameter(torch.randn(out_channel, in_channel, kernel_size, kernel_size))
        self.scale = 1 / math.sqrt(in_channel * kernel_size ** 2)
        self.stride, self.padding = stride, padding
        self.bias = nn.Parameter(torch.zeros(out_channel)) if bias else None
        self.ops = ops if ops is not None else cuda_ops()

    scaler = None

    def forward(self, input, gain=1.0):
        w = self.scaler.get(self, input.dtype, gain) if self.scaler is not None and input.is_cuda else None
        if w is None:
            w = self.weight * (self.scale * gain)
        b = self.bias
        if w.dtype != input.dtype:
            w = w.to(input.dtype)
        if b is not None and b.dtype != input.dtype:
            b = b.to(input.dtype)
        return self.ops.conv2d(input, w, bias=b, stride=self.stride, padding=self.padding)

    def __repr__(self):
        return (f"{self.__class__.__name__}({self.weight.shape[1]}, {self.weight.shape[0]},"
                f" {self.weight.shape[2]}, stride={self.stride}, padding={self.padding})")


class EqualLinear(nn.Module):
    def __init__(self, in_dim, out_dim, bias=True, bias_init=0, lr_mul=1, activation=None, ops=None):
        super().__init__()
        self.weight = nn.Parameter(torch.randn(out_dim, in_dim).div_(lr_mul))
        self.bias = nn.Parameter(torch.zeros(out_dim).fill_(bias_init)) if bias else None
        self.activation = activation
        self.scale = (1 / math.sqrt(in_dim)) * lr_mul
        self.lr_mul = lr_mul
        self.ops = ops if ops is not None else cuda_ops()

    scaler = None

    def forward(self, input):
        w = self.scaler.get(self, input.dtype) if self.scaler is not None and input.is_cuda else None
        if w is None:
            w = self.weight * self.scale
        if self.activation:
            out = F.linear(input, w)
            return self.ops.fused_leaky_relu(out, self.bias * self.lr_mul)
        return F.linear(input, w, bias=self.bias * self.lr_mul)

    def __repr__(self):
        return f"{self.__class__.__name__}({self.weight.shape[1]}, {self.weight.shape[0]})"


class ScaledLeakyReLU(nn.Module):
    def __init__(self, negative_slope=0.2):
        super().__init__()
        self.negative_slope = negative_slope

    def forward(self, input):
        return F.leaky_relu(input, negative_slope=self.negative_slope) * math.sqrt(2)


class FusedLeakyReLU(nn.Module):

    def __init__(self, channel, negative_slope=0.2, scale=2 ** 0.5, ops=None):
        super().__init__()
        self.bias = nn.Parameter(torch.zeros(channel))
        self.negative_slope, self.scale = negative_slope, scale
        self.ops = ops if ops is not None else cuda_ops()

    def forward(self, input):
        bias = self.bias if input.dtype == torch.bfloat16 else self.bias.type(input.dtype)
        return self.ops.fused_leaky_relu(input, bias, self.negative_slope, self.scale)


class ModulatedConv2d(nn.Module):

    def __init__(self, in_channel, out_channel, kernel_size, style_dim, demodulate=True, upsample=False,
                 downsample=False, blur_kernel=[1, 3, 3, 1], normalize=False, ops=None):
        super().__init__()
        self.eps = 1e-8
        self.kernel_size, self.in_channel, self.out_channel = kernel_size, in_channel, out_channel
        self.upsample, self.downsample, self.normalize = upsample, downsample, normalize
        self.ops = ops if ops is not None else cuda_ops()
        if upsample:
            factor = 2
            p = (len(blur_kernel) - factor) - (kernel_size - 1)
            self.blur = Blur(blur_kernel, pad=((p + 1) // 2 + factor - 1, p // 2 + 1), upsample_factor=factor, ops=ops)
        if downsample:
            factor = 2
            p = (len(blur_kernel) - factor) + (kernel_size - 1)
            self.blur = Blur(blur_kernel, pad=((p + 1) // 2, p // 2), ops=ops)
        self.scale = 1 / math.sqrt(in_channel * kernel_size ** 2)
        self.padding = kernel_size // 2
        self.weight = nn.Parameter(torch.randn(1, out_channel, in_channel, kernel_size, kernel_size))
        self.modulation = EqualLinear(style_dim, in_channel, bias_init=1, ops=ops)
        self.demodulate = demodulate

    def __repr__(self):
        return (f"{self.__class__.__name__}({self.in_channel}, {self.out_channel}, {self.kernel_size}, "
                f"upsample={self.upsample}, downsample={self.downsample})")

    def conv_raw(self, input, style):
        style = self.modulation(style)
        plain = not (self.normalize or (input.dtype == torch.float16 and self.demodulate)) and not self.downsample
        if plain:
            return self.ops.modulated_conv2d(input, self.weight, style, self.scale, self.demodulate, self.upsample,
                                             self.padding, self.eps)
        return self._reference_formulation(input, style), None

    def forward(self, input, style, fuse_blur=True):
        raw, demod = self.conv_raw(input, style)
        if demod is not None:
            raw = self.ops.channel_scale(raw, demod)
        if self.upsample and fuse_blur:
            return self.blur(raw)
        return raw

    def _reference_formulation(self, input, style):
        batch, in_channel, height, width = input.shape
        weight = self.weight
        scale = self.scale
        if self.normalize or (input.dtype == torch.float16 and self.demodulate):
            style = style / torch.max(torch.abs(style))
            fan = torch.tensor(in_channel * weight.size(3) * weight.size(4), dtype=torch.float32)
            weight = scale * weight * torch.sqrt(1.0 / fan) / torch.amax(torch.abs(scale * weight), dim=(2, 3, 4), keepdims=True)
            scale = 1.0
        w = self.ops.modulated_weight(weight, style, scale, self.demodulate, transposed=self.upsample, eps=self.eps)
        w = w.type(input.dtype)
        x = input.reshape(1, batch * in_channel, height, width)
        if self.upsample:
            out = self.ops.conv_transpose2d(x, w, padding=0, stride=2, groups=batch)
        elif self.downsample:
            xb = self.blur(input)
            out = self.ops.conv2d(xb.reshape(1, batch * in_channel, xb.shape[2], xb.shape[3]), w, padding=0, stride=2,
                                  groups=batch)
        else:
            out = self.ops.conv2d(x, w, padding=self.padding, groups=batch)
        return out.view(batch, self.out_channel, out.shape[2], out.shape[3])


class NoiseInjection(nn.Module):
    def __init__(self):
        super().__init__()
        self.weight = nn.Parameter(torch.zeros(1))

    @staticmethod
    def sample(batch, height, width, like):
        return like.new_empty(batch, 1, height, width).normal_()

    def forward(self, image, noise=None):
        if noise is None:
            noise = self.sample(image.shape[0], image.shape[2], image.shape[3], image)
        return image + self.weight.type(image.dtype) * noise.type(image.dtype)


class ConstantInput(nn.Module):
    def __init__(self, channel, size=4):
        super().__init__()
        self.input = nn.Parameter(torch.randn(1, channel, size, size))
        self.size = size

    def forward(self, input):
        return self.input.repeat(input.shape[0], 1, 1, 1)


class StyledConv(nn.Module):

    def __init__(self, in_channel, out_channel, kernel_size, style_dim, upsample=False, blur_kernel=[1, 3, 3, 1],
                 demodulate=True, normalize=False, ops=None):
        super().__init__()
        self.conv = ModulatedConv2d(in_channel, out_channel, kernel_size, style_dim, upsample=upsample,
                                    blur_kernel=blur_kernel, demodulate=demodulate, normalize=normalize, ops=ops)
        self.noise = NoiseInjection()
        self.activate = FusedLeakyReLU(out_channel, ops=ops)
        self.ops = ops if ops is not None else cuda_ops()

    def forward(self, input, style, noise=None):
        act = self.activate
        raw, demod = self.conv.conv_raw(input, style)
        if self.conv.upsample:
            blur = self.conv.blur
            out_h = raw.shape[2] + blur.pad[0] + blur.pad[1] - blur.kernel.shape[0] + 1
            out_w = raw.shape[3] + blur.pad[0] + blur.pad[1] - blur.kernel.shape[1] + 1
            if noise is None:
                noise = NoiseInjection.sample(raw.shape[0], out_h, out_w, raw)
            return self.ops.blur_noise_bias_act(raw, blur.kernel, blur.pad, noise, self.noise.weight, act.bias,
                                                act.negative_slope, act.scale, row_scale=demod)
        if noise is None:
            noise = NoiseInjection.sample(raw.shape[0], raw.shape[2], raw.shape[3], raw)
        return self.ops.noise_bias_act(raw, noise, self.noise.weight, act.bias, act.negative_slope, act.scale,
                                       row_scale=demod)


class ToRGB(nn.Module):
    def __init__(self, in_channel, style_dim, upsample=True, blur_kernel=[1, 3, 3, 1], normalize=False, ops=None):
        super().__init__()
        if upsample:
            self.upsample = Upsample(blur_kernel, ops=ops)
        self.conv = ModulatedConv2d(in_channel, 3, 1, style_dim, demodulate=False, normalize=normalize, ops=ops)
        self.bias = nn.Parameter(torch.zeros(1, 3, 1, 1))

    def forward(self, input, style, skip=None):
        conv = self.conv
        up = self.upsample(skip) if skip is not None else None
        if not (conv.normalize or conv.downsample or conv.upsample or conv.demodulate):
            out, _ = conv.ops.modulated_conv2d(input, conv.weight, conv.modulation(style), conv.scale, False, False,
                                               conv.padding, conv.eps, bias=self.bias, skip=up)
            return out
        out = conv(input, style) + self.bias.type(input.dtype)
        if up is not None:
            out = out.float() + up
        return out


class ConvLayer(nn.Sequential):

    def __init__(self, in_channel, out_channel, kernel_size, downsample=False, blur_kernel=[1, 3, 3, 1], bias=True,
                 activate=True, ops=None):
        layers = []
        if downsample:
            factor = 2
            p = (len(blur_kernel) - factor) + (kernel_size - 1)
            layers.append(Blur(blur_kernel, pad=((p + 1) // 2, p // 2), ops=ops))
            stride, self.padding = 2, 0
        else:
            stride, self.padding = 1, kernel_size // 2
        layers.append(EqualConv2d(in_channel, out_channel, kernel_size, padding=self.padding, stride=stride,
                                  bias=bias and not activate, ops=ops))
        if activate:
            layers.append(FusedLeakyReLU(out_channel, ops=ops) if bias else ScaledLeakyReLU(0.2))
        super().__init__(*layers)


class ResBlock(nn.Module):
    def __init__(self, in_channel, out_channel, blur_kernel=[1, 3, 3, 1], downsample=True, ops=None):
        super().__init__()
        self.conv1 = ConvLayer(in_channel, in_channel, 3, ops=ops)
        self.conv2 = ConvLayer(in_channel, out_channel, 3, downsample=downsample, ops=ops)
        self.skip = ConvLayer(in_channel, out_channel, 1, downsample=downsample, activate=False, bias=False, ops=ops)

    def forward(self, input):
        act, skip_conv = self.conv2[-1], self.skip[-1]
        if (input.is_cuda and isinstance(act, FusedLeakyReLU) and getattr(act.ops, "name", None) == "sm_90a"
                and isinstance(skip_conv, EqualConv2d) and skip_conv.bias is None):
            inv = 1.0 / math.sqrt(2)
            main = self.conv1(input)
            for layer in list(self.conv2)[:-1]:
                main = layer(main)
            bias = act.bias if main.dtype == torch.bfloat16 else act.bias.type(main.dtype)
            main = act.ops.fused_leaky_relu(main, bias, act.negative_slope, act.scale * inv)
            side = input
            for layer in list(self.skip)[:-1]:
                side = layer(side)
            return main + skip_conv(side, gain=inv)
        return (self.conv2(self.conv1(input)) + self.skip(input)) / math.sqrt(2)


def channel_table(channel_multiplier):
    return {4: 512, 8: 512, 16: 512, 32: 512, 64: 256 * channel_multiplier, 128: 128 * channel_multiplier,
            256: 64 * channel_multiplier, 512: 32 * channel_multiplier, 1024: 16 * channel_multiplier}


class Generator(nn.Module):

    def __init__(self, size, style_dim, n_mlp, channel_multiplier=2, blur_kernel=[1, 3, 3, 1], lr_mlp=0.01,
                 num_fp16_res=0, run_fp32=True, ops=None):
        super().__init__()
        self.size, self.style_dim = size, style_dim
        self.style = nn.Sequential(PixelNorm(), *[EqualLinear(style_dim, style_dim, lr_mul=lr_mlp, activation="fused_lrelu", ops=ops)
                                                  for _ in range(n_mlp)])
        self.channels = channel_table(channel_multiplier)
        self.input = ConstantInput(self.channels[4])
        self.conv1 = StyledConv(self.channels[4], self.channels[4], 3, style_dim, blur_kernel=blur_kernel, ops=ops)
        self.to_rgb1 = ToRGB(self.channels[4], style_dim, upsample=False, ops=ops)
        self.log_size = int(math.log(size, 2))
        self.num_layers = (self.log_size - 2) * 2 + 1
        self.convs, self.upsamples, self.to_rgbs = nn.ModuleList(), nn.ModuleList(), nn.ModuleList()
        self.noises = nn.Module()
        for layer_idx in range(self.num_layers):
            res = (layer_idx + 5) // 2
            self.noises.register_buffer(f"noise_{layer_idx}", torch.randn(1, 1, 2 ** res, 2 ** res))
        in_channel = self.channels[4]
        for i in range(3, self.log_size + 1):
            mixed = i > self.log_size - num_fp16_res
            out_channel = self.channels[2 ** i]
            self.convs.append(StyledConv(in_channel, out_channel, 3, style_dim, upsample=True, blur_kernel=blur_kernel,
                                         normalize=mixed, ops=ops))
            self.convs.append(StyledConv(out_channel, out_channel, 3, style_dim, blur_kernel=blur_kernel,
                                         normalize=mixed, ops=ops))
            self.to_rgbs.append(ToRGB(out_channel, style_dim, normalize=False, ops=ops))
            in_channel = out_channel
        self.n_latent = self.log_size * 2 - 2
        self.num_fp16_res, self.run_fp32 = num_fp16_res, run_fp32
        self.channels_last = False
        self.act_dtype = torch.float32
        self.fuse_synthesis = True

    def ops_are_native(self):
        return getattr(self.conv1.ops, "name", None) == "sm_90a"

    def make_noise(self, batch_size=1):
        device = self.input.input.device
        noises = [torch.randn(batch_size, 1, 4, 4, device=device)]
        for i in range(3, self.log_size + 1):
            noises += [torch.randn(batch_size, 1, 2 ** i, 2 ** i, device=device) for _ in range(2)]
        return noises

    def batch_latent(self, n_latent):
        return self.style(torch.randn(n_latent, self.style_dim, device=self.input.input.device))

    def mean_latent(self, n_latent):
        return self.batch_latent(n_latent).mean(dim=0, keepdim=True)

    def get_latent(self, input):
        return self.style(input)

    def forward(self, styles, mapping_only=False, return_latents=False, inject_index=None, truncation=1,
                truncation_latent=None, input_is_latent=False, noise=None, randomize_noise=True):
        if not input_is_latent:
            styles = [self.style(s) for s in styles]
            if mapping_only:
                return styles
        if noise is None:
            noise = [None] * self.num_layers if randomize_noise else \
                [getattr(self.noises, f"noise_{i}") for i in range(self.num_layers)]
        if truncation < 1:
            styles = [truncation_latent + truncation * (styles[0] - truncation_latent), styles[0]]
        if len(styles) < 2 or inject_index == self.n_latent:
            inject_index = self.n_latent
            latent = styles[0].unsqueeze(1).repeat(1, inject_index, 1) if styles[0].ndim < 3 else styles[0]
        else:
            if inject_index is None:
                inject_index = random.randint(1, self.n_latent - 1)
            latent = torch.cat([styles[0].unsqueeze(1).repeat(1, inject_index, 1),
                                styles[1].unsqueeze(1).repeat(1, self.n_latent - inject_index, 1)], 1)

        if self.channels_last and self.fuse_synthesis and self.ops_are_native():
            from ..op import styled_fused
            if styled_fused.fusable(self, latent, self.act_dtype):
                image = styled_fused.synthesis(self, latent, noise, self.act_dtype)
                return (image, latent) if return_latents else (image, None)
        x0 = self.input(latent)
        if self.channels_last:
            x0 = x0.contiguous(memory_format=torch.channels_last)
        out = self.conv1(x0, latent[:, 0], noise=noise[0])
        skip = self.to_rgb1(out, latent[:, 1])
        i = 1
        for j, (up, conv, n_up, n_conv, to_rgb) in enumerate(
                zip(self.convs[::2], self.convs[1::2], noise[1::2], noise[2::2], self.to_rgbs), 3):
            half = j > self.log_size - self.num_fp16_res and not self.run_fp32
            out = out.type(torch.float16 if half else torch.float32)
            out = up(out, latent[:, i], noise=n_up)
            out = conv(out, latent[:, i + 1], noise=n_conv)
            skip = to_rgb(out, latent[:, i + 2], skip)
            i += 2
        return (skip, latent) if return_latents else (skip, None)
```

### gangealing_b200/training/latent_learner.py

```python
import numpy as np
import torch
import torch.nn as nn

from . import distributed as gdist


def gen_batches(n, batch_size, min_batch_size=0):
    offsets, start = [0], 0
    for _ in range(n // batch_size):
        end = start + batch_size
        if end + min_batch_size > n:
            continue
        offsets.append(end)
        start = end
    if start < n:
        offsets.append(n)
    return offsets


class PCA:

    def __init__(self, n_components, w_batch, ops=None):
        self.n_components = int(n_components)
        self.ops = ops
        self.n_samples_seen_ = 0
        self._V = self._s = self._mu = None
        self._fit(w_batch, gen_batches(w_batch.size(0), 5 * w_batch.size(1), self.n_components))

    @property
    def pca(self):
        return self

    def update(self, w_batch):
        self._fit(w_batch, [0, w_batch.size(0)])

    def encode(self, x):
        mean = torch.from_numpy(self.mean_).to(x.device)
        comps = torch.from_numpy(self.components_).to(x.device)
        return (x.detach().to(torch.float64) - mean) @ comps.T

    def _fit(self, w, offsets):
        k = self.n_components
        if w.dim() != 2 or not 1 <= k <= w.size(1):
            raise ValueError("PCA: n_components=%d must be between 1 and the %s latents' width" % (k, tuple(w.shape)))
        sizes = [b - a for a, b in zip(offsets[:-1], offsets[1:])]
        if not sizes or min(sizes) < k:
            raise ValueError("PCA: n_components=%d must be less or equal to the batch number of samples %d"
                             % (k, min(sizes) if sizes else 0))
        ops = self.ops
        if ops is None:
            from ..opset import cuda_ops
            ops = cuda_ops()
        gram, mean = ops.batch_gram(w.detach().float(), offsets)
        V, s, mu, seen = self._V, self._s, self._mu, self.n_samples_seen_
        for b, nb in enumerate(sizes):
            if seen == 0:
                A, mu = gram[b], mean[b]
            else:
                delta = mu - mean[b]
                A = (V.T * s.square()) @ V + gram[b] + (seen * nb / (seen + nb)) * torch.outer(delta, delta)
                mu = (seen * mu + nb * mean[b]) / (seen + nb)
            lam, E = torch.linalg.eigh(A)
            V = E[:, -k:].flip(1).T.contiguous()
            s = lam[-k:].flip(0).clamp_min(0).sqrt()
            seen += nb
        self._V, self._s, self._mu, self.n_samples_seen_ = V, s, mu, seen
        signs = V.gather(1, V.abs().argmax(1, keepdim=True)).sign()
        self.components_ = (V * signs).cpu().numpy()
        self.singular_values_ = s.cpu().numpy()
        self.mean_ = mu.cpu().numpy()


class DirectionInterpolator(nn.Module):
    def __init__(self, pca_path, n_comps, inject_index, n_latent, num_heads=1, initializer=None, dim_latent=512):
        super().__init__()
        if pca_path is not None:
            with np.load(pca_path) as data:
                self.register_buffer("lat_mean", torch.from_numpy(data["lat_mean"]))
                self.register_buffer("directions", torch.from_numpy(data["lat_comp"].squeeze(axis=1))[:n_comps])
        else:
            self.register_buffer("directions", torch.randn(n_comps, dim_latent))
            self.register_buffer("lat_mean", torch.randn(1, dim_latent))
        if initializer is None:
            initializer = torch.zeros(num_heads, n_comps)
        self.coefficients = nn.Parameter(initializer.detach().clone())
        self.n_latent, self.inject_index, self.num_heads = n_latent, inject_index, num_heads

    def forward(self, styled_latent, psi=None, lat_mean=None, pca=None, unfold=False):
        if pca is not None:
            return self.assign_buffers(pca)
        return self.interpolate(styled_latent, psi, lat_mean, unfold)

    def interpolate(self, styled_latent, psi, lat_mean=None, unfold=False):
        assert len(styled_latent) == 1
        w = styled_latent[0]
        n = w.size(0)
        mean = self.lat_mean if lat_mean is None else lat_mean
        target = (mean + self.coefficients @ self.directions).repeat(n, 1)
        w = w.repeat_interleave(self.num_heads, dim=0)
        truncated = target.lerp(w, psi).unsqueeze(1).repeat(1, self.inject_index, 1)
        fixed = w.unsqueeze(1).repeat(1, self.n_latent - self.inject_index, 1)
        out = torch.cat([truncated, fixed], dim=1)
        if unfold:
            out = out.reshape(n, self.num_heads, self.n_latent, out.size(-1))
        return [out]

    @torch.no_grad()
    def assign_buffers(self, pca):
        dev = self.directions.device
        self.register_buffer("directions", torch.from_numpy(pca.pca.components_).float().to(dev))
        self.register_buffer("lat_mean", torch.from_numpy(pca.pca.mean_[None]).float().to(dev))

    @torch.no_grad()
    def assign_coefficients(self, initializer):
        self.coefficients.copy_(initializer)


@torch.no_grad()
def kmeans_plusplus(num_heads, num_latent, G, loss_fn, inject_index=6, batch_size=100):
    num_w_per_gpu = num_latent // gdist.get_world_size()
    batch_w = G.batch_latent(num_w_per_gpu)
    dev = batch_w.device
    mean_w = gdist.all_gather(batch_w.mean(dim=0, keepdim=True)).mean(dim=0, keepdim=True)
    batch_fakes = None
    for i in range(0, num_w_per_gpu, batch_size):
        batch_w_in = batch_w[i:i + batch_size]
        fakes, _ = G([batch_w_in, mean_w.expand_as(batch_w_in)], input_is_latent=True, randomize_noise=True,
                     inject_index=inject_index)
        if batch_fakes is None:
            batch_fakes = fakes.new_empty((num_w_per_gpu,) + tuple(fakes.shape[1:]))
        batch_fakes[i:i + batch_size] = fakes
    batch_w = gdist.all_gather(batch_w)
    initial_w_idx = torch.randint(low=0, high=num_latent, size=(1,), device=dev)
    initial_w_idx = gdist.rank0_to_all(initial_w_idx).item()
    dists = []
    centroid_idx = [initial_w_idx]
    for _ in range(num_heads - 1):
        G_w, _ = G([batch_w[centroid_idx[-1]].unsqueeze(0), mean_w], input_is_latent=True, randomize_noise=True,
                   inject_index=inject_index)
        dist = []
        for i in range(0, num_w_per_gpu, batch_size):
            dist.append(loss_fn(G_w.expand_as(batch_fakes[i:i + batch_size]), batch_fakes[i:i + batch_size]).squeeze())
        dist = gdist.all_gather(torch.cat(dist, 0))
        dists.append(dist)
        closest = torch.stack(dists).min(dim=0).values
        logits_sqr = closest ** 2
        logits = logits_sqr / logits_sqr.sum()
        next_idx = gdist.rank0_to_all(torch.multinomial(logits, num_samples=1)).item()
        centroid_idx.append(next_idx)
    print("Centroids: %s" % centroid_idx)
    return batch_w[centroid_idx]
```

### gangealing_b200/training/losses.py

```python
import torch

from ..stn.transformer import total_variation_loss


def flow_identity_loss(delta_flow):
    return delta_flow.pow(2).mean()


def sample_gan_supervised_pairs(generator, ll, resize_fake2stn, psi, batch, dim_latent, freeze_ll, device, z=None):
    with torch.set_grad_enabled(not freeze_ll):
        if z is None:
            z = torch.randn(batch, dim_latent, device=device)
        unaligned_in, w_noise = generator([z], noise=None, return_latents=True)
        w_aligned = ll([w_noise[:, 0, :]], psi=psi)
        aligned_target, _ = generator(w_aligned, input_is_latent=True, noise=None)
        aligned_target = resize_fake2stn(aligned_target)
    return unaligned_in, aligned_target


def gangealing_loss(generator, stn, ll, loss_fn, resize_fake2stn, psi, batch, dim_latent, freeze_ll, device,
                    sample_from_full_res=False, z=None, **stn_kwargs):
    unaligned_in, aligned_target = sample_gan_supervised_pairs(generator, ll, resize_fake2stn, psi, batch, dim_latent,
                                                               freeze_ll, device, z=z)
    source = unaligned_in if sample_from_full_res else None
    aligned_pred, delta_flow = stn(resize_fake2stn(unaligned_in), return_flow=True, input_img_for_sampling=source,
                                   **stn_kwargs)
    return loss_fn(aligned_pred, aligned_target).mean(), delta_flow


def assign_fake_images_to_clusters(generator, stn, ll, loss_fn, resize_fake2stn, psi, batch, dim_latent, freeze_ll,
                                   num_heads, flips, device, sample_from_full_res=True, z=None, **stn_kwargs):
    unaligned_in, aligned_target = sample_gan_supervised_pairs(generator, ll, resize_fake2stn, psi, batch, dim_latent,
                                                               freeze_ll, device, z)
    if flips:
        unaligned_in = torch.cat([unaligned_in, unaligned_in.flip(3,)], 0)
        aligned_target = aligned_target.repeat(2, 1, 1, 1)
        loss_size = (2, batch, num_heads)
    else:
        loss_size = (batch, num_heads)
    source = unaligned_in if sample_from_full_res else None
    resized = resize_fake2stn(unaligned_in)
    aligned_pred, delta_flow = stn(resized, return_flow=True, input_img_for_sampling=source, **stn_kwargs)
    perceptual = loss_fn(aligned_pred, aligned_target).view(*loss_size)
    collapsed = perceptual.permute(1, 0, 2).reshape(batch, 2 * num_heads) if flips else perceptual
    return collapsed.min(dim=1), aligned_pred, delta_flow, unaligned_in, resized, collapsed


def gangealing_cluster_loss(generator, stn, ll, loss_fn, resize_fake2stn, psi, batch, dim_latent, freeze_ll, num_heads,
                            flips, device, sample_from_full_res=True, z=None, **stn_kwargs):
    assignments, _, delta_flow, _, _, _ = assign_fake_images_to_clusters(
        generator, stn, ll, loss_fn, resize_fake2stn, psi, batch, dim_latent, freeze_ll, num_heads, flips, device,
        sample_from_full_res, z=z, **stn_kwargs)
    hw2 = delta_flow.size()[1:]
    if flips:
        delta_flow = delta_flow.view(2, batch, num_heads, *hw2).permute(1, 0, 2, 3, 4, 5).reshape(batch, 2 * num_heads, *hw2)
    else:
        delta_flow = delta_flow.view(batch, num_heads, *hw2)
    return assignments.values.mean(), delta_flow[torch.arange(batch, device=delta_flow.device), assignments.indices]
```

### include/gg_b200.h

```cpp
#ifndef GG_B200_H_
#define GG_B200_H_

#include <stdint.h>

#ifdef __cplusplus
extern "C" {
#endif

#define GG_API __attribute__((visibility("default")))

enum { GG_F32 = 0, GG_F16 = 1, GG_BF16 = 2, GG_F64 = 3 };

enum {
  GG_OK = 0,
  GG_ERR_BAD_ARG = -1,
  GG_ERR_UNSUPPORTED = -2,
  GG_ERR_CUDA = -3
};

enum { GG_PAD_ZEROS = 0, GG_PAD_BORDER = 1, GG_PAD_REFLECTION = 2 };

GG_API int gg_version(void);
GG_API const char* gg_last_error(void);
GG_API int gg_sm_count(void);

GG_API int gg_fused_bias_act(void* out, const void* x, const void* bias, const void* ref, int dtype,
                             int act, int grad, float alpha, float scale, int64_t size_x,
                             int64_t step_b, int64_t size_b, void* stream);

GG_API int gg_noise_bias_act(void* out, const void* x, const void* noise, const float* noise_weight,
                             const float* bias, const float* row_scale, int dtype, float alpha, float scale,
                             int64_t N, int64_t C, int64_t HW, void* stream);

GG_API int64_t gg_channel_scale_workspace(int64_t rows, int64_t HW);
GG_API int gg_channel_scale(void* out, float* row_dot, void* workspace, const void* x, const void* y,
                            const float* s, int dtype, int64_t rows, int64_t HW, void* stream);

GG_API int64_t gg_bias_act_backward_workspace(int64_t N, int64_t C, int64_t HW);
GG_API int gg_bias_act_backward(void* gx, float* grad_bias, void* workspace, const void* g,
                                const void* out, int dtype, float alpha, float scale, int64_t N,
                                int64_t C, int64_t HW, void* stream);

GG_API int gg_upfirdn2d(void* out, const void* in, const float* kernel, int dtype, int64_t major,
                        int in_h, int in_w, int kernel_h, int kernel_w, int up_x, int up_y,
                        int down_x, int down_y, int pad_x0, int pad_x1, int pad_y0, int pad_y1,
                        void* stream);

GG_API int gg_blur_noise_bias_act(void* out, const void* in, const float* kernel, const void* noise,
                                  const float* noise_weight, const float* bias,
                                  const float* row_scale, int dtype, int64_t N, int64_t C, int in_h,
                                  int in_w, int kernel_h, int kernel_w, int pad_x0, int pad_x1,
                                  int pad_y0, int pad_y1, int act, float alpha, float scale,
                                  void* stream);

GG_API int64_t gg_mipmap_pyramid_elems(int64_t planes, int hs, int ws, int extra_levels);
GG_API int gg_mipmap_build(float* pyramid, const void* src, int dtype, int64_t planes, int hs, int ws,
                           int extra_levels, void* stream);
GG_API int gg_mipmap_build_backward(float* grad_src, float* grad_pyramid, int64_t planes, int hs, int ws,
                                    int extra_levels, void* stream);
GG_API int gg_mipmap_warp_forward(void* out, float* levels_out, const void* src, const float* pyramid,
                                  const float* grid, int dtype, int64_t N, int C, int hs, int ws, int ho,
                                  int wo, int extra_levels, float max_level, float min_level,
                                  int padding_mode, void* stream);
GG_API int gg_mipmap_warp_backward(float* grad_src, float* grad_pyramid, float* grad_grid,
                                   const void* grad_out, const void* src, const float* pyramid,
                                   const float* grid, int dtype, int64_t N, int C, int hs, int ws, int ho,
                                   int wo, int extra_levels, float max_level, float min_level,
                                   int padding_mode, void* stream);
GG_API int gg_warp_sample_indices(int32_t* indices, const float* grid, int64_t N, int hs, int ws, int ho, int wo,
                                  float max_level, float min_level, int padding_mode, void* stream);
GG_API int gg_mipmap_warp_lerp_forward(void* out, float* grid_out, const void* src, const float* pyramid, const float* base,
                                       int64_t base_stride, const float* target, const float* alphas, int T, int dtype,
                                       int64_t N, int C, int hs, int ws, int ho, int wo, int extra_levels, float max_level,
                                       float min_level, int padding_mode, void* stream);
GG_API int gg_mipmap_warp_lerp_mean(float* acc, const void* src, const float* pyramid, const float* base, int64_t base_stride,
                                    const float* target, const float* alphas, int T, int dtype, int64_t N, int C, int hs,
                                    int ws, int ho, int wo, int extra_levels, float max_level, float min_level,
                                    int padding_mode, int accumulate, void* stream);

GG_API int gg_flow_compose_forward(float* delta_flow, float* flow, const float* low_flow, const float* mask,
                                   const float* identity_flow, const float* base_warp, const float* alpha,
                                   int64_t N, int H, int W, int S, void* stream);
GG_API int gg_flow_compose_backward(float* grad_mask, float* grad_low_flow, float* grad_base_warp,
                                    const float* grad_delta, const float* grad_flow, const float* low_flow,
                                    const float* mask, const float* identity_flow, const float* base_warp,
                                    const float* alpha, int64_t N, int H, int W, int S, void* stream);

GG_API int64_t gg_splat2d_workspace(int64_t N, int C, int H, int W);
GG_API int gg_splat2d_forward(float* out, void* workspace, const float* input, const float* coordinates,
                              const float* values, const float* sigma, int64_t N, int64_t P, int C, int H,
                              int W, int soft_normalize, void* stream);

GG_API int gg_stn_sample_forward(void* out, float* grid_out, float* delta_out, float* levels_out, const void* src,
                                 const float* pyramid, const float* theta, const float* low, const float* mask,
                                 const float* identity, const float* alpha, int mode, int dtype, int64_t N, int C,
                                 int hs, int ws, int ho, int wo, int lh, int lw, int s, int extra_levels,
                                 float max_level, float min_level, int padding_mode, void* stream);

GG_API int gg_modconv_wsq(float* wsq, const float* weight, int O, int I, int kk, void* stream);
GG_API int gg_modconv_demod(float* demod, const float* wsq, const float* style, float scale, float eps, int B,
                            int O, int I, void* stream);
GG_API int gg_modconv_demod_batched(int layers, float* const* demod, const float* const* wsq, const float* const* style,
                                    const float* scale, const int* O, const int* I, float eps, int B, void* stream);
GG_API int gg_modconv_modulate(float* out, const float* weight, const float* style, const float* demod,
                               float scale, int B, int O, int I, int kk, int transposed, void* stream);

GG_API int gg_noise_bias_act_nhwc(void* out, const void* x, const float* noise, const float* noise_weight,
                                  const float* bias, const float* row_scale, int dtype, float alpha, float scale,
                                  int64_t N, int C, int64_t HW, void* stream);
GG_API int64_t gg_nhwc_rowwise_workspace(int64_t N, int C, int64_t HW);
GG_API int gg_channel_scale_nhwc(void* out, float* row_dot, void* workspace, const void* x, const void* y,
                                 const float* s, int dtype, int64_t N, int C, int64_t HW, void* stream);
GG_API int gg_bias_act_backward_nhwc(void* gx, float* grad_bias, void* workspace, const void* g,
                                     const void* out_saved, int dtype, float alpha, float scale, int64_t N, int C,
                                     int64_t HW, void* stream);
GG_API int64_t gg_blur_nhwc_workspace(int dtype, int64_t N, int C, int in_h, int in_w, int kernel_h, int kernel_w,
                                      int pad_x0, int pad_x1, int pad_y0, int pad_y1);
GG_API int gg_blur_nhwc(void* out, void* out2, const void* in, const float* kernel, const float* noise,
                        const float* noise_weight, const float* bias, const float* row_scale, const float* scale2,
                        const void* mul, float* row_dot, void* workspace, int dtype, int64_t N, int C, int in_h,
                        int in_w, int kernel_h, int kernel_w, int separable, int pad_x0, int pad_x1, int pad_y0,
                        int pad_y1, int mode, int act, float alpha, float scale, void* stream);

GG_API int gg_styled_tail_nhwc(void* out, void* xs, float* rgb, const void* raw, const float* noise,
                               const float* noise_weight, const float* bias, const float* demod, const float* s_next,
                               const float* wm, const float* rgb_bias, const float* skip, int dtype, int act,
                               float alpha, float scale, int64_t N, int C, int64_t HW, void* stream);
GG_API int64_t gg_styled_tail_backward_workspace(int dtype, int64_t N, int C, int64_t HW);
GG_API int gg_styled_tail_backward_nhwc(void* g_raw, float* d_s_next, float* d_demod, float* d_wm, void* workspace,
                                        const void* g_xs, const float* g_rgb, const void* out_saved, const void* raw,
                                        const float* s_next, const float* demod, const float* wm, int dtype,
                                        float alpha, float scale, int64_t N, int C, int64_t HW, int64_t reduce_pitch,
                                        void* stream);

GG_API int64_t gg_to_rgb_nhwc_workspace(int64_t N, int C, int64_t HW);
GG_API int gg_to_rgb_nhwc_forward(float* out, const float* x, const float* wm, const float* bias, const float* skip,
                                  int64_t N, int C, int64_t HW, void* stream);
GG_API int gg_to_rgb_nhwc_backward(float* gx, float* gwm, void* workspace, const float* g, const float* x,
                                   const float* wm, int64_t N, int C, int64_t HW, void* stream);


GG_API int64_t gg_feature_distance_workspace(int64_t N, int C, int64_t HW);
GG_API int gg_feature_distance_forward(float* out, void* workspace, const void* f0, const void* f1,
                                       const float* weight, int dtype, int64_t N, int C, int64_t HW, float eps,
                                       void* stream);
GG_API int gg_feature_distance_backward(void* g0, void* g1, const float* grad_out, const void* f0, const void* f1,
                                        const float* weight, int dtype, int64_t N, int C, int64_t HW, float eps,
                                        void* stream);

GG_API int gg_bias_relu_pool_nhwc_forward(void* y, void* pooled, const void* raw, const float* bias, int dtype, int64_t N,
                                          int C, int H, int W, void* stream);
GG_API int gg_bias_relu_pool_nhwc_backward(void* grad_raw, const void* grad_y, const void* grad_pooled, const void* y,
                                           int dtype, int64_t N, int C, int H, int W, void* stream);

GG_API int gg_tent_downsample_forward(float* out, const float* in, const float* taps_h, const float* taps_v, int64_t N,
                                      int C, int in_h, int in_w, int stride, void* stream);
GG_API int gg_tent_downsample_backward(float* grad_in, const float* grad_out, const float* taps_h, const float* taps_v,
                                       int64_t N, int C, int in_h, int in_w, int stride, void* stream);

GG_API int64_t gg_nn_argmin_workspace(int64_t N, int64_t P);
GG_API int gg_nn_argmin(int64_t* index, void* workspace, const float* grid, const float* points, int64_t N, int64_t P, int HW,
                        void* stream);
GG_API int gg_track_points_lerp(int64_t* track, int64_t* centers, const float* base, const float* target, const float* alphas,
                                const float* points, int T, int64_t N, int64_t P, int H, int W, int patch, void* stream);
GG_API int gg_splat2d_lookup_forward(float* out, float* points_out, void* workspace, const float* input, const float* grid,
                                     const float* query, const float* values, const float* sigma, int64_t N, int64_t P,
                                     int C, int H, int W, int grid_h, int grid_w, float unnorm_k, float unnorm_m,
                                     int soft_normalize, void* stream);

GG_API int gg_tv_per_sample(float* out, const float* flow, int64_t N, int H, int W, void* stream);
GG_API int64_t gg_pck_transfer_workspace(int64_t B, int64_t P, int F);
GG_API int gg_pck_transfer(int64_t* counts, float* est_points, int64_t* nn_index, void* workspace, const float* points,
                           const float* gt_points, const float* visible, const float* thresh, const float* alphas,
                           const float* matrix_src, const float* matrix_dst, const float* delta_src, const float* identity,
                           const float* grid_dst, int64_t B, int64_t P, int A, int S, int F, int grid_h, int grid_w,
                           void* stream);

GG_API int64_t gg_laplacian_blend_workspace(int64_t N, int C, int H, int W, int levels, int backward);
GG_API int gg_laplacian_blend_forward(float* out, void* workspace, const float* img0, const float* img1, const float* mask,
                                      const float* taps, int64_t N, int C, int H, int W, int levels, int width, void* stream);
GG_API int gg_laplacian_blend_backward(float* grad_img0, float* grad_img1, float* grad_mask, void* workspace,
                                       const float* grad_out, const float* img0, const float* img1, const float* mask,
                                       const float* taps, int64_t N, int C, int H, int W, int levels, int width,
                                       void* stream);

GG_API int gg_adam_ema_step(const void* table, const int* block_tensor, const int* block_chunk, int blocks, int chunk,
                            float* state, double beta1, double beta2, double eps, double ema_decay, void* stream);
GG_API int64_t gg_tv_loss_workspace(int64_t N, int H, int W);
GG_API int gg_tv_loss_forward(float* out, void* workspace, const float* flow, int64_t N, int H, int W, void* stream);
GG_API int gg_tv_loss_backward(float* grad_flow, const float* grad_out, const float* flow, int64_t N, int H, int W,
                               void* stream);

GG_API int gg_scale_cast_multi(const void* table, const int* block_tensor, const int* block_chunk, int blocks, int chunk,
                               void* stream);

GG_API int gg_batch_gram(double* gram, double* mean, const float* w, const int64_t* batch_offsets, int64_t B, int D,
                         void* stream);

#ifdef __cplusplus
}
#endif
#endif
```

Baseline: 468.1.

## Save leaky-ReLU sign bitmask instead of full activations for styled backward

Adds mask variants of the blur and styled-tail kernels. When the saved output is only needed for the leaky-ReLU derivative, they store one sign bit per channel, packed with warp shuffles, instead of the full activation tensor, and the backward kernel reads those bits. The training loss also passes latents in split form with per-row grad flags, so rows without gradient can skip style and demod gradient work. This cuts activation write and read traffic, at the cost of extra shuffle work, new kernel variants and plumbing through the generator.

Measured after the change: 498.7, median of 6. 6.5% higher.

```diff
diff --git a/gangealing_b200/_lib.py b/gangealing_b200/_lib.py
--- a/gangealing_b200/_lib.py
+++ b/gangealing_b200/_lib.py
@@ -43,7 +43,10 @@
     "gg_bias_act_backward_nhwc": (_I, [_P] * 5 + [_I, _F, _F, _L, _I, _L, _P]),
     "gg_blur_nhwc_workspace": (_L, [_I, _L] + [_I] * 9),
     "gg_blur_nhwc": (_I, [_P] * 12 + [_I, _L] + [_I] * 12 + [_F, _F, _P]),
+    "gg_blur_nhwc_mask": (_I, [_P] * 9 + [_I, _L] + [_I] * 11 + [_F, _F, _P]),
     "gg_styled_tail_nhwc": (_I, [_P] * 12 + [_I, _I, _F, _F, _L, _I, _L, _P]),
+    "gg_styled_tail_mask_nhwc": (_I, [_P] * 12 + [_I, _I, _F, _F, _L, _I, _L, _P]),
+    "gg_styled_tail_backward_mask_nhwc": (_I, [_P] * 7 + [_I, _F, _F, _L, _I, _L, _P]),
     "gg_styled_tail_backward_workspace": (_L, [_I, _L, _I, _L]),
     "gg_styled_tail_backward_nhwc": (_I, [_P] * 12 + [_I, _F, _F, _L, _I, _L, _L, _P]),
     "gg_tent_downsample_forward": (_I, [_P] * 4 + [_L, _I, _I, _I, _I, _P]),
diff --git a/gangealing_b200/csrc/common.cuh b/gangealing_b200/csrc/common.cuh
--- a/gangealing_b200/csrc/common.cuh
+++ b/gangealing_b200/csrc/common.cuh
@@ -136,6 +136,29 @@
 }
 __device__ __forceinline__ void stg_stream16(void* p, const uint4& u) {
   asm volatile("st.global.L1::no_allocate.v4.u32 [%0], {%1,%2,%3,%4};" ::"l"(p), "r"(u.x), "r"(u.y), "r"(u.z), "r"(u.w) : "memory");
+}
+
+template <typename T> struct SignFloor { static constexpr float v = 0.f; };
+template <> struct SignFloor<__nv_bfloat16> { static constexpr float v = 0x1p-134f; };
+
+template <typename T, int V>
+__device__ __forceinline__ uint32_t sign_bits(const float (&o)[V]) {
+  uint32_t m = 0u;
+#pragma unroll
+  for (int k = 0; k < V; ++k) m |= (o[k] > SignFloor<T>::v ? 1u : 0u) << k;
+  return m;
+}
+template <int V>
+__device__ __forceinline__ uint32_t sign_word(uint32_t bits, int cq, unsigned lanes) {
+  constexpr int L = 32 / V;
+  uint32_t w = bits << (V * (cq & (L - 1)));
+#pragma unroll
+  for (int m = L / 2; m >= 1; m >>= 1) w |= __shfl_xor_sync(lanes, w, m);
+  return w;
+}
+template <int V>
+__device__ __forceinline__ uint32_t sign_load(const uint32_t* px, int cq) {
+  return __ldg(px + (cq * V >> 5)) >> (cq * V & 31);
 }
 
 __device__ __forceinline__ float warp_sum(float v) {
diff --git a/gangealing_b200/csrc/nhwc.cu b/gangealing_b200/csrc/nhwc.cu
--- a/gangealing_b200/csrc/nhwc.cu
+++ b/gangealing_b200/csrc/nhwc.cu
@@ -297,7 +297,8 @@
                  float* __restrict__ partial, BlurNhwcParams p) {
   using G = BlurGeom<T>;
   constexpr int V = G::V, CB = G::CB, COLS = G::COLS, BX = G::BX, TW = G::TW;
-  constexpr bool FUSED = MODE == 1;
+  constexpr bool FUSED = MODE == 1 || MODE == 3;
+  constexpr bool MASK = MODE == 3;
   extern __shared__ __align__(128) unsigned char tiles_raw[];
   T* tiles = reinterpret_cast<T*>(tiles_raw);
   __shared__ uint64_t full_bar[kNS];
@@ -539,8 +540,14 @@
               a4[k] = t;
               o2[k] = __fmul_rn(t, sq[k]);
             }
+            uint32_t word = 0u;
+            if (MASK) word = sign_word<V>(sign_bits<T>(a4), cq, 0xffffffffu);
             if (okc[j]) {
-              if (out) *reinterpret_cast<uint4*>(out + ooff) = ChanVec<T>::pack(a4);
+              if (MASK) {
+                if ((cq * V & 31) == 0) reinterpret_cast<uint32_t*>(out)[ooff >> 5] = word;
+              } else if (out) {
+                *reinterpret_cast<uint4*>(out + ooff) = ChanVec<T>::pack(a4);
+              }
               if (out2) *reinterpret_cast<uint4*>(out2 + ooff) = ChanVec<T>::pack(o2);
             }
           } else if (MODE == 2) {
@@ -809,7 +816,7 @@
                        const float* noise_weight, const float* bias, const float* row_scale, const float* scale2,
                        const void* mul, float* row_dot, void* workspace, int64_t N, int C, int in_h, int in_w, int kernel_h,
                        int kernel_w, int separable, int pad_x0, int pad_x1, int pad_y0, int pad_y1, int mode, int act,
-                       float alpha, float scale, void* stream, int dtype) {
+                       float alpha, float scale, void* stream, int dtype, bool out_is_mask) {
   using G = BlurGeom<T>;
   BlurPlan pl;
   int rc = blur_plan(&pl, dtype, N, C, in_h, in_w, kernel_h, kernel_w, pad_x0, pad_x1, pad_y0, pad_y1);
@@ -853,15 +860,19 @@
   static DeviceOnce configured;
   if (configured.needed()) {
     cudaError_t e = cudaSuccess;
-    const void* kernels[8] = {reinterpret_cast<const void*>(blur_nhwc_kernel<T, 0, true>),
+    const void* kernels[12] = {reinterpret_cast<const void*>(blur_nhwc_kernel<T, 0, true>),
                               reinterpret_cast<const void*>(blur_nhwc_kernel<T, 0, false>),
                               reinterpret_cast<const void*>(blur_nhwc_kernel<T, 1, true, false>),
                               reinterpret_cast<const void*>(blur_nhwc_kernel<T, 1, false, false>),
                               reinterpret_cast<const void*>(blur_nhwc_kernel<T, 1, true, true>),
                               reinterpret_cast<const void*>(blur_nhwc_kernel<T, 1, false, true>),
+                              reinterpret_cast<const void*>(blur_nhwc_kernel<T, 3, true, false>),
+                              reinterpret_cast<const void*>(blur_nhwc_kernel<T, 3, false, false>),
+                              reinterpret_cast<const void*>(blur_nhwc_kernel<T, 3, true, true>),
+                              reinterpret_cast<const void*>(blur_nhwc_kernel<T, 3, false, true>),
                               reinterpret_cast<const void*>(blur_nhwc_kernel<T, 2, true>),
                               reinterpret_cast<const void*>(blur_nhwc_kernel<T, 2, false>)};
-    for (int i = 0; i < 8 && e == cudaSuccess; ++i)
+    for (int i = 0; i < 12 && e == cudaSuccess; ++i)
       e = cudaFuncSetAttribute(kernels[i], cudaFuncAttributeMaxDynamicSharedMemorySize, static_cast<int>(smem));
     if (e != cudaSuccess) return cuda_fail(e, "blur_nhwc smem opt-in");
     configured.done();
@@ -873,7 +884,11 @@
   blur_nhwc_kernel<T, M_, S_, F_><<<grid, kT, smem, st>>>(static_cast<T*>(out), static_cast<T*>(out2), tmap, kernel, kernel_h, \
                                                          kernel_w, noise, noise_weight, bias, row_scale, scale2,     \
                                                          static_cast<const T*>(mul), partial, p)
-  if (mode == 1) {
+  if (mode == 1 && out_is_mask) {
+    if (fast) { if (separable) GG_BLUR(3, true, true); else GG_BLUR(3, false, true); }
+    else { if (separable) GG_BLUR(3, true, false); else GG_BLUR(3, false, false); }
+  }
+  else if (mode == 1) {
     if (fast) { if (separable) GG_BLUR(1, true, true); else GG_BLUR(1, false, true); }
     else { if (separable) GG_BLUR(1, true, false); else GG_BLUR(1, false, false); }
   }
@@ -910,8 +925,28 @@
   GG_DISPATCH_T(dtype, "blur_nhwc",
                 return launch_blur<T_>(out, out2, in, kernel, noise, noise_weight, bias, row_scale, scale2, mul, row_dot,
                                        workspace, N, C, in_h, in_w, kernel_h, kernel_w, separable, pad_x0, pad_x1, pad_y0,
-                                       pad_y1, mode, act, alpha, scale, stream, dtype));
+                                       pad_y1, mode, act, alpha, scale, stream, dtype, false));
   return GG_OK;
 }
 
-}
+int gg_blur_nhwc_mask(void* mask, void* out2, const void* in, const float* kernel, const float* noise,
+                      const float* noise_weight, const float* bias, const float* row_scale, const float* scale2, int dtype,
+                      int64_t N, int C, int in_h, int in_w, int kernel_h, int kernel_w, int separable, int pad_x0, int pad_x1,
+                      int pad_y0, int pad_y1, int act, float alpha, float scale, void* stream) {
+  if (N < 0 || C < 0 || in_h < 1 || in_w < 1) return fail(GG_ERR_BAD_ARG, "blur_nhwc_mask: bad shape");
+  if (kernel_h < 1 || kernel_w < 1 || kernel_h > 4 || kernel_w > 4) return fail(GG_ERR_UNSUPPORTED, "blur_nhwc_mask: filter must be <= 4x4");
+  if (act != 1 && act != 3) return fail(GG_ERR_UNSUPPORTED, "blur_nhwc_mask: act must be 1 or 3");
+  if (dtype != GG_F32 && dtype != GG_BF16) return fail(GG_ERR_UNSUPPORTED, "blur_nhwc_mask: dtype %d not supported (fp32 or bf16)", dtype);
+  if (N == 0 || C == 0) return GG_OK;
+  if (!in || !kernel) return fail(GG_ERR_BAD_ARG, "blur_nhwc_mask: null tensor");
+  if (!mask) return fail(GG_ERR_BAD_ARG, "blur_nhwc_mask: null mask");
+  if (out2 && !scale2) return fail(GG_ERR_BAD_ARG, "blur_nhwc_mask: out2 needs scale2");
+  if (N > 65535) return fail(GG_ERR_UNSUPPORTED, "blur_nhwc_mask: batch > 65535");
+  GG_DISPATCH_T(dtype, "blur_nhwc_mask",
+                return launch_blur<T_>(mask, out2, in, kernel, noise, noise_weight, bias, row_scale, scale2, nullptr, nullptr,
+                                       nullptr, N, C, in_h, in_w, kernel_h, kernel_w, separable, pad_x0, pad_x1, pad_y0,
+                                       pad_y1, 1, act, alpha, scale, stream, dtype, true));
+  return GG_OK;
+}
+
+}
diff --git a/gangealing_b200/csrc/styled.cu b/gangealing_b200/csrc/styled.cu
--- a/gangealing_b200/csrc/styled.cu
+++ b/gangealing_b200/csrc/styled.cu
@@ -19,7 +19,7 @@
   int chunk, chunks_per_sample;
 };
 
-template <typename T, bool FAST>
+template <typename T, bool FAST, bool MASK>
 __global__ void __launch_bounds__(kT, 2)
 styled_tail_nhwc_kernel(const TailFwdParams p) {
   constexpr int V = ChanVec<T>::V;
@@ -53,7 +53,8 @@
   const unsigned gmask = 0xffu << (threadIdx.x & 24);
   const int hw = static_cast<int>(p.hw);
   const T* raw = static_cast<const T*>(p.raw) + n * hw * C;
-  T* out = p.out ? static_cast<T*>(p.out) + n * hw * C : nullptr;
+  T* out = (p.out && !MASK) ? static_cast<T*>(p.out) + n * hw * C : nullptr;
+  uint32_t* mask = MASK ? static_cast<uint32_t*>(p.out) + n * hw * (C >> 5) : nullptr;
   T* xs = p.xs ? static_cast<T*>(p.xs) + n * hw * C : nullptr;
   const float* noise_n = p.noise ? p.noise + n * hw : nullptr;
   const int q0 = static_cast<int>(p0), q1 = static_cast<int>(p1);
@@ -124,9 +125,15 @@
             acc[u][2] = fmaf(w2[k], o[k], acc[u][2]);
           }
         }
+        uint32_t word = 0u;
+        if (MASK) word = sign_word<V>(sign_bits<T>(o), l, gmask);
         if (pb + u < q1) {
           const unsigned off = po[u] + static_cast<unsigned>(v * V);
-          if (out) stg_stream16(out + off, ChanVec<T>::pack(o));
+          if (MASK) {
+            if ((l * V & 31) == 0) mask[off >> 5] = word;
+          } else if (out) {
+            stg_stream16(out + off, ChanVec<T>::pack(o));
+          }
           if (xs) stg_stream16(xs + off, ChanVec<T>::pack(o2));
         }
       }
@@ -164,7 +171,7 @@
   int r_ds, r_dd, r_gw, n_red;
 };
 
-template <typename T>
+template <typename T, bool MASK>
 __global__ void __launch_bounds__(kT, 2)
 styled_tail_bwd_nhwc_kernel(const TailBwdParams p) {
   constexpr int V = ChanVec<T>::V;
@@ -181,6 +188,11 @@
   for (int k = 0; k < V; ++k) a_ds[k] = a_dd[k] = a_g0[k] = a_g1[k] = a_g2[k] = 0.f;
   const T* gxs = static_cast<const T*>(p.g_xs);
   const T* outp = static_cast<const T*>(p.out);
+  const uint32_t* maskp = static_cast<const uint32_t*>(p.out) + n * p.hw * (C >> 5);
+  const int mw = C >> 5;
+  auto load_out = [&](int64_t pu, int64_t off) {
+    return MASK ? make_uint4(sign_load<V>(maskp + pu * mw, cq), 0u, 0u, 0u) : ldg_stream16(outp + off);
+  };
   const T* rawp = static_cast<const T*>(p.raw);
   T* graw = static_cast<T*>(p.g_raw);
   if (pl < lanes_p) {
@@ -199,19 +211,22 @@
     auto body = [&](int64_t off, const uint4 gr, const uint4 orw, const uint4 rr, float s0, float s1, float s2) {
       float g[V], o[V], r[V], gt[V];
       ChanVec<T>::unpack(gr, g);
-      ChanVec<T>::unpack(orw, o);
+      if (!MASK) ChanVec<T>::unpack(orw, o);
       ChanVec<T>::unpack(rr, r);
 #pragma unroll
       for (int k = 0; k < V; ++k) {
         float go = g[k] * sv[k];
         if (p.g_rgb) go = fmaf(w2[k], s2, fmaf(w1[k], s1, fmaf(w0[k], s0, go)));
-        const float t = (o[k] > 0.f ? go : go * p.alpha) * p.gain;
-        a_ds[k] = fmaf(g[k], o[k], a_ds[k]);
-        a_dd[k] = fmaf(t, r[k], a_dd[k]);
-        a_g0[k] = fmaf(s0, o[k], a_g0[k]);
-        a_g1[k] = fmaf(s1, o[k], a_g1[k]);
-        a_g2[k] = fmaf(s2, o[k], a_g2[k]);
+        const bool pos = MASK ? ((orw.x >> k) & 1u) != 0u : o[k] > 0.f;
+        const float t = (pos ? go : go * p.alpha) * p.gain;
         gt[k] = t * dv[k];
+        if (!MASK) {
+          a_ds[k] = fmaf(g[k], o[k], a_ds[k]);
+          a_dd[k] = fmaf(t, r[k], a_dd[k]);
+          a_g0[k] = fmaf(s0, o[k], a_g0[k]);
+          a_g1[k] = fmaf(s1, o[k], a_g1[k]);
+          a_g2[k] = fmaf(s2, o[k], a_g2[k]);
+        }
       }
       *reinterpret_cast<uint4*>(graw + off) = ChanVec<T>::pack(gt);
     };
@@ -224,7 +239,7 @@
       for (int u = 0; u < U; ++u) {
         const int64_t pu = pp + u * lanes_p;
         off[u] = ((n * p.hw + pu) * cv + cq) * V;
-        orw[u] = ldg_stream16(outp + off[u]);
+        orw[u] = load_out(pu, off[u]);
         gr[u] = gxs ? ldg_stream16(gxs + off[u]) : zero;
       }
 #pragma unroll
@@ -240,11 +255,11 @@
     }
     for (; pp < p1; pp += lanes_p) {
       const int64_t off = ((n * p.hw + pp) * cv + cq) * V;
-      body(off, gxs ? ldg_stream16(gxs + off) : zero, ldg_stream16(outp + off), rawp ? ldg_stream16(rawp + off) : zero,
+      body(off, gxs ? ldg_stream16(gxs + off) : zero, load_out(pp, off), rawp ? ldg_stream16(rawp + off) : zero,
            g0 ? __ldg(g0 + pp) : 0.f, g0 ? __ldg(g0 + p.hw + pp) : 0.f, g0 ? __ldg(g0 + 2 * p.hw + pp) : 0.f);
     }
   }
-  if (p.partial && p.n_red > 0) {
+  if (!MASK && p.partial && p.n_red > 0) {
     const int R = p.n_red;
     if (pl < lanes_p) {
       float* row = red + static_cast<int64_t>(pl) * R * C + cq * V;
@@ -289,26 +304,25 @@
 
 using namespace gg;
 
-extern "C" {
-
-int gg_styled_tail_nhwc(void* out, void* xs, float* rgb, const void* raw, const float* noise, const float* noise_weight,
-                        const float* bias, const float* demod, const float* s_next, const float* wm, const float* rgb_bias,
-                        const float* skip, int dtype, int act, float alpha, float scale, int64_t N, int C, int64_t HW,
-                        void* stream) {
-  if (N < 0 || C < 0 || HW < 0) return fail(GG_ERR_BAD_ARG, "styled_tail_nhwc: negative size");
-  if (dtype != GG_F32 && dtype != GG_BF16) return fail(GG_ERR_UNSUPPORTED, "styled_tail_nhwc: dtype %d not supported (fp32 or bf16)", dtype);
-  if (act != 1 && act != 3) return fail(GG_ERR_UNSUPPORTED, "styled_tail_nhwc: act must be 1 (linear) or 3 (lrelu)");
+static int launch_tail_fwd(const char* who, void* out, bool out_is_mask, void* xs, float* rgb, const void* raw,
+                           const float* noise, const float* noise_weight, const float* bias, const float* demod,
+                           const float* s_next, const float* wm, const float* rgb_bias, const float* skip, int dtype, int act,
+                           float alpha, float scale, int64_t N, int C, int64_t HW, void* stream) {
+  if (N < 0 || C < 0 || HW < 0) return fail(GG_ERR_BAD_ARG, "%s: negative size", who);
+  if (dtype != GG_F32 && dtype != GG_BF16) return fail(GG_ERR_UNSUPPORTED, "%s: dtype %d not supported (fp32 or bf16)", who, dtype);
+  if (act != 1 && act != 3) return fail(GG_ERR_UNSUPPORTED, "%s: act must be 1 (linear) or 3 (lrelu)", who);
   if (N * HW * C == 0) return GG_OK;
   const int V = dtype == GG_BF16 ? 8 : 4;
-  if (C % (V * kGroup) != 0 || C > 2048) return fail(GG_ERR_UNSUPPORTED, "styled_tail_nhwc: C must be a multiple of %d, <= 2048", V * kGroup);
-  if (!raw || (!out && !xs && !rgb)) return fail(GG_ERR_BAD_ARG, "styled_tail_nhwc: null tensor");
-  if (xs && !s_next) return fail(GG_ERR_BAD_ARG, "styled_tail_nhwc: xs needs s_next");
-  if (rgb && !wm) return fail(GG_ERR_BAD_ARG, "styled_tail_nhwc: rgb needs wm");
+  if (C % (V * kGroup) != 0 || C > 2048) return fail(GG_ERR_UNSUPPORTED, "%s: C must be a multiple of %d, <= 2048", who, V * kGroup);
+  if (!raw || (!out && !xs && !rgb)) return fail(GG_ERR_BAD_ARG, "%s: null tensor", who);
+  if (out_is_mask && !out) return fail(GG_ERR_BAD_ARG, "%s: null mask", who);
+  if (xs && !s_next) return fail(GG_ERR_BAD_ARG, "%s: xs needs s_next", who);
+  if (rgb && !wm) return fail(GG_ERR_BAD_ARG, "%s: rgb needs wm", who);
   const int64_t chunk = fwd_chunk(N, HW);
-  if (chunk > 0x7fffff00LL || HW * C >= 0x7fffffffLL) return fail(GG_ERR_BAD_ARG, "styled_tail_nhwc: plane too large (H*W*C must be < 2^31)");
+  if (chunk > 0x7fffff00LL || HW * C >= 0x7fffffffLL) return fail(GG_ERR_BAD_ARG, "%s: plane too large (H*W*C must be < 2^31)", who);
   const int K = static_cast<int>((HW + chunk - 1) / chunk);
   const int64_t grid = N * K;
-  if (grid > 0x7fffffffLL) return fail(GG_ERR_BAD_ARG, "styled_tail_nhwc: too many CTAs");
+  if (grid > 0x7fffffffLL) return fail(GG_ERR_BAD_ARG, "%s: too many CTAs", who);
   TailFwdParams p;
   p.raw = raw; p.out = out; p.xs = xs; p.rgb = rgb; p.skip = rgb ? skip : nullptr;
   p.noise = noise; p.noise_weight = noise_weight; p.bias = bias; p.demod = demod; p.s_next = s_next;
@@ -318,15 +332,34 @@
   auto st = static_cast<cudaStream_t>(stream);
   const bool fast = p.gain > 0.f && ((p.act == 3 && p.alpha >= 0.f && p.alpha <= 1.f) || p.act == 1);
   const unsigned g = static_cast<unsigned>(grid);
-  if (dtype == GG_F32) {
-    if (fast) styled_tail_nhwc_kernel<float, true><<<g, kT, smem, st>>>(p);
-    else styled_tail_nhwc_kernel<float, false><<<g, kT, smem, st>>>(p);
-  } else {
-    if (fast) styled_tail_nhwc_kernel<__nv_bfloat16, true><<<g, kT, smem, st>>>(p);
-    else styled_tail_nhwc_kernel<__nv_bfloat16, false><<<g, kT, smem, st>>>(p);
-  }
+#define GG_TAIL(T_, F_)                                                                   \
+  do {                                                                                    \
+    if (out_is_mask) styled_tail_nhwc_kernel<T_, F_, true><<<g, kT, smem, st>>>(p);       \
+    else styled_tail_nhwc_kernel<T_, F_, false><<<g, kT, smem, st>>>(p);                  \
+  } while (0)
+  if (dtype == GG_F32) { if (fast) GG_TAIL(float, true); else GG_TAIL(float, false); }
+  else { if (fast) GG_TAIL(__nv_bfloat16, true); else GG_TAIL(__nv_bfloat16, false); }
+#undef GG_TAIL
   GG_CHECK_LAUNCH("styled_tail_nhwc launch");
   return GG_OK;
+}
+
+extern "C" {
+
+int gg_styled_tail_nhwc(void* out, void* xs, float* rgb, const void* raw, const float* noise, const float* noise_weight,
+                        const float* bias, const float* demod, const float* s_next, const float* wm, const float* rgb_bias,
+                        const float* skip, int dtype, int act, float alpha, float scale, int64_t N, int C, int64_t HW,
+                        void* stream) {
+  return launch_tail_fwd("styled_tail_nhwc", out, false, xs, rgb, raw, noise, noise_weight, bias, demod, s_next, wm, rgb_bias,
+                         skip, dtype, act, alpha, scale, N, C, HW, stream);
+}
+
+int gg_styled_tail_mask_nhwc(void* mask, void* xs, float* rgb, const void* raw, const float* noise, const float* noise_weight,
+                             const float* bias, const float* demod, const float* s_next, const float* wm,
+                             const float* rgb_bias, const float* skip, int dtype, int act, float alpha, float scale, int64_t N,
+                             int C, int64_t HW, void* stream) {
+  return launch_tail_fwd("styled_tail_mask_nhwc", mask, true, xs, rgb, raw, noise, noise_weight, bias, demod, s_next, wm,
+                         rgb_bias, skip, dtype, act, alpha, scale, N, C, HW, stream);
 }
 
 int64_t gg_styled_tail_backward_workspace(int dtype, int64_t N, int C, int64_t HW) {
@@ -375,16 +408,16 @@
   if (smem > 48 * 1024) {
     static DeviceOnce configured;
     if (configured.needed()) {
-      cudaError_t e = cudaFuncSetAttribute(styled_tail_bwd_nhwc_kernel<float>, cudaFuncAttributeMaxDynamicSharedMemorySize, 100 * 1024);
+      cudaError_t e = cudaFuncSetAttribute(styled_tail_bwd_nhwc_kernel<float, false>, cudaFuncAttributeMaxDynamicSharedMemorySize, 100 * 1024);
       if (e == cudaSuccess)
-        e = cudaFuncSetAttribute(styled_tail_bwd_nhwc_kernel<__nv_bfloat16>, cudaFuncAttributeMaxDynamicSharedMemorySize, 100 * 1024);
+        e = cudaFuncSetAttribute(styled_tail_bwd_nhwc_kernel<__nv_bfloat16, false>, cudaFuncAttributeMaxDynamicSharedMemorySize, 100 * 1024);
       if (e != cudaSuccess) return cuda_fail(e, "styled_tail_backward_nhwc smem opt-in");
       configured.done();
     }
     if (smem > 100 * 1024) return fail(GG_ERR_UNSUPPORTED, "styled_tail_backward_nhwc: C too large for the reduction stage");
   }
-  if (dtype == GG_F32) styled_tail_bwd_nhwc_kernel<float><<<static_cast<unsigned>(grid), kT, smem, st>>>(p);
-  else styled_tail_bwd_nhwc_kernel<__nv_bfloat16><<<static_cast<unsigned>(grid), kT, smem, st>>>(p);
+  if (dtype == GG_F32) styled_tail_bwd_nhwc_kernel<float, false><<<static_cast<unsigned>(grid), kT, smem, st>>>(p);
+  else styled_tail_bwd_nhwc_kernel<__nv_bfloat16, false><<<static_cast<unsigned>(grid), kT, smem, st>>>(p);
   GG_CHECK_LAUNCH("styled_tail_backward_nhwc launch");
   if (r > 0) {
     float* first = d_s_next ? d_s_next : (d_demod ? d_demod : d_wm);
@@ -410,4 +443,31 @@
   return GG_OK;
 }
 
-}
+int gg_styled_tail_backward_mask_nhwc(void* g_raw, const void* g_xs, const float* g_rgb, const void* mask,
+                                      const float* s_next, const float* demod, const float* wm, int dtype, float alpha,
+                                      float scale, int64_t N, int C, int64_t HW, void* stream) {
+  if (N < 0 || C < 0 || HW < 0) return fail(GG_ERR_BAD_ARG, "styled_tail_backward_mask_nhwc: negative size");
+  if (dtype != GG_F32 && dtype != GG_BF16) return fail(GG_ERR_UNSUPPORTED, "styled_tail_backward_mask_nhwc: dtype %d not supported", dtype);
+  if (N * HW * C == 0) return GG_OK;
+  const int V = dtype == GG_BF16 ? 8 : 4;
+  if (C % 32 != 0 || C / V > kT) return fail(GG_ERR_UNSUPPORTED, "styled_tail_backward_mask_nhwc: C must be a multiple of 32, <= %d", V * kT);
+  if (!g_raw || !mask || (!g_xs && !g_rgb)) return fail(GG_ERR_BAD_ARG, "styled_tail_backward_mask_nhwc: null tensor");
+  if (g_xs && !s_next) return fail(GG_ERR_BAD_ARG, "styled_tail_backward_mask_nhwc: g_xs needs s_next");
+  if (g_rgb && !wm) return fail(GG_ERR_BAD_ARG, "styled_tail_backward_mask_nhwc: g_rgb needs wm");
+  const int64_t chunk64 = bwd_chunk(N, C / V, HW);
+  if (chunk64 > 0x7fffffffLL) return fail(GG_ERR_BAD_ARG, "styled_tail_backward_mask_nhwc: plane too large");
+  const int K = static_cast<int>((HW + chunk64 - 1) / chunk64);
+  const int64_t grid = N * K;
+  if (grid > 0x7fffffffLL) return fail(GG_ERR_BAD_ARG, "styled_tail_backward_mask_nhwc: too many CTAs");
+  TailBwdParams p;
+  p.g_raw = g_raw; p.partial = nullptr; p.g_xs = g_xs; p.out = mask; p.raw = nullptr; p.s_next = s_next; p.demod = demod;
+  p.g_rgb = g_rgb; p.wm = wm; p.alpha = alpha; p.gain = scale; p.C = C; p.hw = HW; p.chunk = static_cast<int>(chunk64);
+  p.chunks_per_sample = K; p.r_ds = p.r_dd = p.r_gw = -1; p.n_red = 0;
+  auto st = static_cast<cudaStream_t>(stream);
+  if (dtype == GG_F32) styled_tail_bwd_nhwc_kernel<float, true><<<static_cast<unsigned>(grid), kT, 0, st>>>(p);
+  else styled_tail_bwd_nhwc_kernel<__nv_bfloat16, true><<<static_cast<unsigned>(grid), kT, 0, st>>>(p);
+  GG_CHECK_LAUNCH("styled_tail_backward_mask_nhwc launch");
+  return GG_OK;
+}
+
+}
diff --git a/gangealing_b200/op/nhwc.py b/gangealing_b200/op/nhwc.py
--- a/gangealing_b200/op/nhwc.py
+++ b/gangealing_b200/op/nhwc.py
@@ -38,8 +38,14 @@
     return noise.float().contiguous()
 
 
+def sign_mask_empty(n, c, h, w, device):
+    if c % 32:
+        raise RuntimeError("sign mask: C = %d is not a multiple of 32" % c)
+    return torch.empty((n, h, w, c // 32), dtype=torch.int32, device=device)
+
+
 def blur(x, kernel, pad, mode=0, noise=None, noise_weight=None, bias=None, row_scale=None, scale2=None, want_out=True,
-         want_out2=False, mul=None, want_dot=False, negative_slope=0.2, gain=1.0, act=3):
+         want_out2=False, mul=None, want_dot=False, negative_slope=0.2, gain=1.0, act=3, want_mask=False):
     n, c, in_h, in_w = x.shape
     taps = kernel.detach()
     if taps.dtype != torch.float32 or not taps.is_contiguous():
@@ -54,7 +60,12 @@
 
     def empty():
         return torch.empty((n, c, out_h, out_w), dtype=x.dtype, device=x.device, memory_format=CL)
-    out = empty() if (want_out or mode != 1) else None
+    if want_mask and mode != 1:
+        raise RuntimeError("blur: the sign mask belongs to the fused tail (mode 1)")
+    if want_mask:
+        out = sign_mask_empty(n, c, out_h, out_w, x.device)
+    else:
+        out = empty() if (want_out or mode != 1) else None
     out2 = empty() if (mode == 1 and want_out2) else None
     nz = noise_plane(noise, n, out_h, out_w) if mode == 1 else None
     dot = ws = None
@@ -71,17 +82,24 @@
         ev0, ev1 = torch.cuda.Event(enable_timing=True), torch.cuda.Event(enable_timing=True)
         ev0.record()
     nw, b, rs, s2 = _f32(noise_weight, 1), _f32(bias, c), _f32(row_scale, n * c), _f32(scale2, n * c)
-    rc = lib.gg_blur_nhwc(_lib.ptr(out), _lib.ptr(out2), x.data_ptr(), taps.data_ptr(), _lib.ptr(nz),
-                          _lib.ptr(nw), _lib.ptr(b), _lib.ptr(rs),
-                          _lib.ptr(s2), _lib.ptr(mul if dot is not None else None), _lib.ptr(dot), _lib.ptr(ws),
-                          code, n, c, in_h, in_w, kh, kw, 1 if _lib.filter_is_separable(kernel) else 0, pad[0], pad[1],
-                          pad[2], pad[3], mode, act, negative_slope, gain, _lib.stream())
-    _lib.check(rc, "gg_blur_nhwc")
+    sep = 1 if _lib.filter_is_separable(kernel) else 0
+    if want_mask:
+        rc = lib.gg_blur_nhwc_mask(out.data_ptr(), _lib.ptr(out2), x.data_ptr(), taps.data_ptr(), _lib.ptr(nz), _lib.ptr(nw),
+                                   _lib.ptr(b), _lib.ptr(rs), _lib.ptr(s2), code, n, c, in_h, in_w, kh, kw, sep, pad[0],
+                                   pad[1], pad[2], pad[3], act, negative_slope, gain, _lib.stream())
+    else:
+        rc = lib.gg_blur_nhwc(_lib.ptr(out), _lib.ptr(out2), x.data_ptr(), taps.data_ptr(), _lib.ptr(nz),
+                              _lib.ptr(nw), _lib.ptr(b), _lib.ptr(rs),
+                              _lib.ptr(s2), _lib.ptr(mul if dot is not None else None), _lib.ptr(dot), _lib.ptr(ws),
+                              code, n, c, in_h, in_w, kh, kw, sep, pad[0], pad[1],
+                              pad[2], pad[3], mode, act, negative_slope, gain, _lib.stream())
+    _lib.check(rc, "gg_blur_nhwc_mask" if want_mask else "gg_blur_nhwc")
     if timed:
         ev1.record()
         es = x.element_size()
-        writes = (out is not None) + (out2 is not None)
+        writes = (out is not None and not want_mask) + (out2 is not None)
         TIMING.append((ev0, ev1, es * n * c * (in_h * in_w + writes * out_h * out_w) + (4 * n * out_h * out_w if nz is not None else 0)
+                       + (out.numel() * 4 if want_mask else 0)
                        + 4 * ((2 + (scale2 is not None)) * c + 1 + kh * kw)))
     return out, out2, dot
 
@@ -126,9 +144,13 @@
     return out, dot
 
 
-def styled_tail(raw, noise, noise_weight, bias, demod, s_next, wm, rgb_bias, skip, want_out, negative_slope, gain, act=3):
+def styled_tail(raw, noise, noise_weight, bias, demod, s_next, wm, rgb_bias, skip, want_out, negative_slope, gain, act=3,
+                want_mask=False):
     n, c, h, w = raw.shape
-    out = torch.empty_like(raw) if want_out else None
+    if want_mask:
+        out = sign_mask_empty(n, c, h, w, raw.device)
+    else:
+        out = torch.empty_like(raw) if want_out else None
     xs = torch.empty_like(raw) if s_next is not None else None
     rgb = torch.empty((n, 3, h, w), dtype=torch.float32, device=raw.device) if wm is not None else None
     sk = None
@@ -140,10 +162,11 @@
             raise RuntimeError("styled_tail: skip must be (N, 3, H, W)")
     consts = [noise_plane(noise, n, h, w), _f32(noise_weight, 1), _f32(bias, c), _f32(demod, n * c), _f32(s_next, n * c),
               _f32(wm, n * 3 * c), _f32(rgb_bias, 3)]
-    rc = _lib.load().gg_styled_tail_nhwc(_lib.ptr(out), _lib.ptr(xs), _lib.ptr(rgb), raw.data_ptr(),
-                                         *[_lib.ptr(t) for t in consts], _lib.ptr(sk),
-                                         _lib.dtype_code(raw), act, negative_slope, gain, n, c, h * w, _lib.stream())
-    _lib.check(rc, "gg_styled_tail_nhwc")
+    lib = _lib.load()
+    entry = lib.gg_styled_tail_mask_nhwc if want_mask else lib.gg_styled_tail_nhwc
+    rc = entry(_lib.ptr(out), _lib.ptr(xs), _lib.ptr(rgb), raw.data_ptr(), *[_lib.ptr(t) for t in consts], _lib.ptr(sk),
+               _lib.dtype_code(raw), act, negative_slope, gain, n, c, h * w, _lib.stream())
+    _lib.check(rc, "gg_styled_tail_mask_nhwc" if want_mask else "gg_styled_tail_nhwc")
     return out, xs, rgb
 
 
@@ -177,3 +200,21 @@
                                           code, negative_slope, gain, n, c, h * w, rows * c, _lib.stream())
     _lib.check(rc, "gg_styled_tail_backward_nhwc")
     return g_raw, d_s, d_d, d_w
+
+
+def styled_tail_backward_mask(g_xs, g_rgb, mask, s_next, demod, wm, negative_slope, gain, dtype):
+    n, h, w, words = mask.shape
+    c = 32 * words
+    g_raw = torch.empty((n, c, h, w), dtype=dtype, device=mask.device, memory_format=CL)
+    if g_xs is not None and (g_xs.shape != g_raw.shape or g_xs.dtype != dtype or not g_xs.is_contiguous(memory_format=CL)
+                             or not _lib.aligned16(g_xs)):
+        raise RuntimeError("styled_tail_backward_mask: g_xs must be a 16-byte-aligned channels-last tensor of the "
+                               "activation's shape and dtype")
+    if g_rgb is not None and (g_rgb.shape != (n, 3, h, w) or g_rgb.dtype != torch.float32 or not g_rgb.is_contiguous()):
+        raise RuntimeError("styled_tail_backward_mask: g_rgb must be a dense fp32 (N, 3, H, W) tensor")
+    consts = [_f32(s_next, n * c), _f32(demod, n * c), _f32(wm, n * 3 * c)]
+    rc = _lib.load().gg_styled_tail_backward_mask_nhwc(g_raw.data_ptr(), _lib.ptr(g_xs), _lib.ptr(g_rgb), mask.data_ptr(),
+                                                       *[_lib.ptr(t) for t in consts], _lib.dtype_code(g_raw),
+                                                       negative_slope, gain, n, c, h * w, _lib.stream())
+    _lib.check(rc, "gg_styled_tail_backward_mask_nhwc")
+    return g_raw
diff --git a/gangealing_b200/op/style_path.py b/gangealing_b200/op/style_path.py
--- a/gangealing_b200/op/style_path.py
+++ b/gangealing_b200/op/style_path.py
@@ -21,7 +21,7 @@
             w = torch.stack([(lin.weight.detach() * lin.scale).t().contiguous() for _, lin, _ in members])
             b = torch.stack([(lin.bias.detach() * lin.lr_mul) for _, lin, _ in members]).unsqueeze(1)
             idx = torch.tensor([li for _, _, li in members], device=w.device)
-            self.groups.append((w, b, idx, [key for key, _, _ in members]))
+            self.groups.append((w, b, idx, [key for key, _, _ in members], [li for _, _, li in members]))
         self.stamp = tuple((lin.weight._version, lin.weight.data_ptr(), lin.bias._version) for _, lin, _ in mods)
 
     def valid(self, convs, rgbs):
@@ -29,17 +29,17 @@
         return self.stamp == tuple((lin.weight._version, lin.weight.data_ptr(), lin.bias._version) for lin in mods)
 
 
-def all_styles(generator, latent, convs, rgbs, conv_idx, rgb_idx):
+def all_styles(generator, latent, convs, rgbs, conv_idx, rgb_idx, row_needs_grad=None):
     plan = getattr(generator, "_gg_style_plan", None)
     if plan is None or not plan.valid(convs, rgbs):
         plan = _Plan(convs, rgbs, conv_idx, rgb_idx)
         generator._gg_style_plan = plan
     out = {}
-    for w, b, idx, keys in plan.groups:
+    for w, b, idx, keys, rows in plan.groups:
         lat = latent.index_select(1, idx).transpose(0, 1)
         s = torch.baddbmm(b, lat, w)
         for j, key in enumerate(keys):
-            out[key] = s[j]
+            out[key] = s[j] if row_needs_grad is None or row_needs_grad[rows[j]] else s[j].detach()
     return [out[("conv", i)] for i in range(len(convs))], [out[("rgb", i)] for i in range(len(rgbs))]
 
 
@@ -67,6 +67,7 @@
                                           I(*[w.shape[1] for w in weights]), I(*[w.shape[2] for w in weights]), float(eps), b,
                                           _lib.stream())
         _lib.check(rc, "gg_modconv_demod_batched")
+        ctx.mark_non_differentiable(*[o for l, o in enumerate(outs) if not ctx.needs_input_grad[1 + l]])
         ctx.save_for_backward(*ss, *outs, *wsqs)
         ctx.cfg = (n, tuple(float(x) for x in scales), tuple(s.dtype for s in styles))
         return tuple(outs)
diff --git a/gangealing_b200/op/styled_fused.py b/gangealing_b200/op/styled_fused.py
--- a/gangealing_b200/op/styled_fused.py
+++ b/gangealing_b200/op/styled_fused.py
@@ -16,19 +16,21 @@
     def forward(ctx, raw, demod, s_next, wm, skip, noise, noise_weight, bias, rgb_bias, kernel, pad, negative_slope, gain):
         _lib.require_cuda(raw, demod, s_next, wm, skip, noise)
         needs = ctx.needs_input_grad
-        save = needs[0] or needs[1] or needs[2] or needs[3]
+        reduces = needs[1] or needs[2] or needs[3]
+        save = needs[0] or reduces
+        masked = needs[0] and not reduces and (kernel is None or s_next is not None)
         if kernel is None:
-            out, xs, rgb = nhwc.styled_tail(raw, noise, noise_weight, bias, demod, s_next, wm, rgb_bias, skip, save,
-                                            negative_slope, gain)
+            out, xs, rgb = nhwc.styled_tail(raw, noise, noise_weight, bias, demod, s_next, wm, rgb_bias, skip,
+                                            save and not masked, negative_slope, gain, want_mask=masked)
         else:
             if wm is not None:
                 raise RuntimeError("fused tail: the blur (up-sampling) layers carry no to-RGB branch")
             pad4 = (pad[0], pad[1], pad[0], pad[1])
             out, xs, _ = nhwc.blur(raw, kernel, pad4, mode=1, noise=noise, noise_weight=noise_weight, bias=bias,
-                                   row_scale=demod, scale2=s_next, want_out=save or s_next is None,
-                                   want_out2=s_next is not None, negative_slope=negative_slope, gain=gain)
+                                   row_scale=demod, scale2=s_next, want_out=(save and not masked) or s_next is None,
+                                   want_out2=s_next is not None, negative_slope=negative_slope, gain=gain, want_mask=masked)
             rgb = None
-        ctx.cfg = (kernel is not None, pad, negative_slope, gain, tuple(raw.shape))
+        ctx.cfg = (kernel is not None, pad, negative_slope, gain, tuple(raw.shape), masked, raw.dtype)
         if save:
             ctx.save_for_backward(raw if (needs[1] and demod is not None) else None, out,
                                   demod.detach() if demod is not None else None,
@@ -42,27 +44,32 @@
     @once_differentiable
     def backward(ctx, g_xs, g_rgb):
         raw, out, demod, s_next, wm, kernel = ctx.saved_tensors
-        is_blur, pad, negative_slope, gain, raw_shape = ctx.cfg
+        is_blur, pad, negative_slope, gain, raw_shape, masked, dtype = ctx.cfg
         need_raw, need_d, need_s, need_w, need_skip = ctx.needs_input_grad[:5]
         if g_xs is not None:
             g_xs = g_xs.contiguous(memory_format=CL)
-            if g_xs.dtype != out.dtype:
-                g_xs = g_xs.to(out.dtype)
+            if g_xs.dtype != dtype:
+                g_xs = g_xs.to(dtype)
         if g_rgb is not None:
             g_rgb = g_rgb.float().contiguous()
         g_raw = d_s = d_d = d_w = None
         if g_xs is None and g_rgb is None:
             return (None,) * 13
-        if not is_blur:
+        if masked and not is_blur:
+            g_raw = nhwc.styled_tail_backward_mask(g_xs, g_rgb, out, s_next, demod, wm, negative_slope, gain, dtype)
+        elif not is_blur:
             g_raw, d_s, d_d, d_w = nhwc.styled_tail_backward(
                 g_xs, g_rgb, out, raw, s_next, demod, wm, need_s, need_d and demod is not None, need_w,
                 negative_slope, gain)
         else:
-            g_t, d_s, _, _ = nhwc.styled_tail_backward(g_xs, None, out, None, s_next, None, None, need_s, False, False,
-                                                       negative_slope, gain)
+            if masked:
+                g_t = nhwc.styled_tail_backward_mask(g_xs, None, out, s_next, None, None, negative_slope, gain, dtype)
+            else:
+                g_t, d_s, _, _ = nhwc.styled_tail_backward(g_xs, None, out, None, s_next, None, None, need_s, False, False,
+                                                           negative_slope, gain)
             kh, kw = kernel.shape
             pad4 = (pad[0], pad[1], pad[0], pad[1])
-            gp = grad_pad(raw_shape[2], raw_shape[3], out.shape[2], out.shape[3], kh, kw, (1, 1), (1, 1), pad4)
+            gp = grad_pad(raw_shape[2], raw_shape[3], g_t.shape[2], g_t.shape[3], kh, kw, (1, 1), (1, 1), pad4)
             want_dot = need_d and demod is not None
             g_raw, _, d_d = nhwc.blur(g_t, _lib.flipped_filter(kernel), gp, mode=2, row_scale=demod, mul=raw if want_dot else None,
                                       want_dot=want_dot)
@@ -94,12 +101,12 @@
     return not any(p.requires_grad for p in generator.parameters())
 
 
-def synthesis(generator, latent, noise, act_dtype=torch.float32):
+def synthesis(generator, latent, noise, act_dtype=torch.float32, row_needs_grad=None):
     layers = [generator.conv1] + list(generator.convs)
     rgbs = [generator.to_rgb1] + list(generator.to_rgbs)
     b = latent.shape[0]
     styles, rgb_styles = style_path.all_styles(generator, latent, layers, rgbs, list(range(len(layers))),
-                                               [2 * r + 1 for r in range(len(rgbs))])
+                                               [2 * r + 1 for r in range(len(rgbs))], row_needs_grad)
     demods = style_path.all_demod([layer.conv.weight for layer in layers], styles, [layer.conv.scale for layer in layers],
                                   layers[0].conv.eps)
     x0 = generator.input(latent).to(act_dtype).contiguous(memory_format=CL)
diff --git a/gangealing_b200/stylegan2/networks.py b/gangealing_b200/stylegan2/networks.py
--- a/gangealing_b200/stylegan2/networks.py
+++ b/gangealing_b200/stylegan2/networks.py
@@ -383,6 +383,7 @@
                 [getattr(self.noises, f"noise_{i}") for i in range(self.num_layers)]
         if truncation < 1:
             styles = [truncation_latent + truncation * (styles[0] - truncation_latent), styles[0]]
+        row_needs_grad = None
         if len(styles) < 2 or inject_index == self.n_latent:
             inject_index = self.n_latent
             latent = styles[0].unsqueeze(1).repeat(1, inject_index, 1) if styles[0].ndim < 3 else styles[0]
@@ -391,11 +392,12 @@
                 inject_index = random.randint(1, self.n_latent - 1)
             latent = torch.cat([styles[0].unsqueeze(1).repeat(1, inject_index, 1),
                                 styles[1].unsqueeze(1).repeat(1, self.n_latent - inject_index, 1)], 1)
+            row_needs_grad = [styles[0].requires_grad] * inject_index + [styles[1].requires_grad] * (self.n_latent - inject_index)
 
         if self.channels_last and self.fuse_synthesis and self.ops_are_native():
             from ..op import styled_fused
             if styled_fused.fusable(self, latent, self.act_dtype):
-                image = styled_fused.synthesis(self, latent, noise, self.act_dtype)
+                image = styled_fused.synthesis(self, latent, noise, self.act_dtype, row_needs_grad)
                 return (image, latent) if return_latents else (image, None)
         x0 = self.input(latent)
         if self.channels_last:
diff --git a/gangealing_b200/training/latent_learner.py b/gangealing_b200/training/latent_learner.py
--- a/gangealing_b200/training/latent_learner.py
+++ b/gangealing_b200/training/latent_learner.py
@@ -86,18 +86,22 @@
         self.coefficients = nn.Parameter(initializer.detach().clone())
         self.n_latent, self.inject_index, self.num_heads = n_latent, inject_index, num_heads
 
-    def forward(self, styled_latent, psi=None, lat_mean=None, pca=None, unfold=False):
+    def forward(self, styled_latent, psi=None, lat_mean=None, pca=None, unfold=False, split=False):
         if pca is not None:
             return self.assign_buffers(pca)
-        return self.interpolate(styled_latent, psi, lat_mean, unfold)
+        return self.interpolate(styled_latent, psi, lat_mean, unfold, split)
 
-    def interpolate(self, styled_latent, psi, lat_mean=None, unfold=False):
+    def interpolate(self, styled_latent, psi, lat_mean=None, unfold=False, split=False):
         assert len(styled_latent) == 1
         w = styled_latent[0]
         n = w.size(0)
         mean = self.lat_mean if lat_mean is None else lat_mean
         target = (mean + self.coefficients @ self.directions).repeat(n, 1)
         w = w.repeat_interleave(self.num_heads, dim=0)
+        if split:
+            if unfold:
+                raise ValueError("DirectionInterpolator: unfold and split are exclusive")
+            return [target.lerp(w, psi), w]
         truncated = target.lerp(w, psi).unsqueeze(1).repeat(1, self.inject_index, 1)
         fixed = w.unsqueeze(1).repeat(1, self.n_latent - self.inject_index, 1)
         out = torch.cat([truncated, fixed], dim=1)
diff --git a/gangealing_b200/training/losses.py b/gangealing_b200/training/losses.py
--- a/gangealing_b200/training/losses.py
+++ b/gangealing_b200/training/losses.py
@@ -12,8 +12,9 @@
         if z is None:
             z = torch.randn(batch, dim_latent, device=device)
         unaligned_in, w_noise = generator([z], noise=None, return_latents=True)
-        w_aligned = ll([w_noise[:, 0, :]], psi=psi)
-        aligned_target, _ = generator(w_aligned, input_is_latent=True, noise=None)
+        w_aligned = ll([w_noise[:, 0, :]], psi=psi, split=True)
+        inject = getattr(ll, "module", ll).inject_index
+        aligned_target, _ = generator(w_aligned, input_is_latent=True, inject_index=inject, noise=None)
         aligned_target = resize_fake2stn(aligned_target)
     return unaligned_in, aligned_target
 
diff --git a/include/gg_b200.h b/include/gg_b200.h
--- a/include/gg_b200.h
+++ b/include/gg_b200.h
@@ -121,6 +121,11 @@
                         const void* mul, float* row_dot, void* workspace, int dtype, int64_t N, int C, int in_h,
                         int in_w, int kernel_h, int kernel_w, int separable, int pad_x0, int pad_x1, int pad_y0,
                         int pad_y1, int mode, int act, float alpha, float scale, void* stream);
+GG_API int gg_blur_nhwc_mask(void* mask, void* out2, const void* in, const float* kernel, const float* noise,
+                             const float* noise_weight, const float* bias, const float* row_scale, const float* scale2,
+                             int dtype, int64_t N, int C, int in_h, int in_w, int kernel_h, int kernel_w, int separable,
+                             int pad_x0, int pad_x1, int pad_y0, int pad_y1, int act, float alpha, float scale,
+                             void* stream);
 
 GG_API int gg_styled_tail_nhwc(void* out, void* xs, float* rgb, const void* raw, const float* noise,
                                const float* noise_weight, const float* bias, const float* demod, const float* s_next,
@@ -132,6 +137,14 @@
                                         const float* s_next, const float* demod, const float* wm, int dtype,
                                         float alpha, float scale, int64_t N, int C, int64_t HW, int64_t reduce_pitch,
                                         void* stream);
+GG_API int gg_styled_tail_mask_nhwc(void* mask, void* xs, float* rgb, const void* raw, const float* noise,
+                                    const float* noise_weight, const float* bias, const float* demod,
+                                    const float* s_next, const float* wm, const float* rgb_bias, const float* skip,
+                                    int dtype, int act, float alpha, float scale, int64_t N, int C, int64_t HW,
+                                    void* stream);
+GG_API int gg_styled_tail_backward_mask_nhwc(void* g_raw, const void* g_xs, const float* g_rgb, const void* mask,
+                                             const float* s_next, const float* demod, const float* wm, int dtype,
+                                             float alpha, float scale, int64_t N, int C, int64_t HW, void* stream);
 
 GG_API int64_t gg_to_rgb_nhwc_workspace(int64_t N, int C, int64_t HW);
 GG_API int gg_to_rgb_nhwc_forward(float* out, const float* x, const float* wm, const float* bias, const float* skip,
```
